# qope/starky-bn254

Measured on AMD Instinct MI355X. Metric: G1 scalar-mult proofs/sec at trace height 2^16, higher is better.
Workload: dtype u64

## Files before the change

### starky_bn254_amd/csrc/kernels.cuh

```cuda
#pragma once
#include "poseidon.cuh"
#include "air.cuh"

#include "kernels_ntt.cuh"

__global__ void pow_table_kernel(u64* out, size_t n, u64 base) {
  size_t i = (size_t)blockIdx.x * blockDim.x + threadIdx.x;
  if (i < n) out[i] = f_pow(F(base), i).v;
}
__global__ void shift_odd_table_kernel(u64* out, size_t n, const u64* __restrict__ shift, const u64* __restrict__ tw, u32 log_s) {
  size_t i = (size_t)blockIdx.x * blockDim.x + threadIdx.x;
  if (i < n) out[i] = (F(shift[i]) * F(tw[(i >> log_s) << log_s])).v;
}
__global__ void scale_pow_kernel(u64* v, size_t n, u64 base) {
  size_t i = (size_t)blockIdx.x * blockDim.x + threadIdx.x;
  if (i < n) v[i] = (F(v[i]) * f_pow(F(base), i)).v;
}

__global__ __launch_bounds__(256) __attribute__((amdgpu_waves_per_eu(4))) void leaf_hash_kernel(const u64* __restrict__ lde, size_t m, u32 lde_log, u32 ncols,
                                                        u64* __restrict__ digests) {
  size_t row = (size_t)blockIdx.x * blockDim.x + threadIdx.x;
  if (row >= m) return;
  F s[12];
#pragma unroll
  for (int i = 0; i < 12; i++) s[i] = F(0);
  size_t leaf = bitrev32((u32)row, lde_log);
  if (ncols <= 4) {
    for (u32 c = 0; c < 4; c++) digests[leaf * 4 + c] = c < ncols ? lde[(size_t)c * m + row] : 0;
    return;
  }
  for (u32 c = 0; c < ncols; c += 8) {
#pragma unroll
    for (u32 i = 0; i < 8; i++)
      if (c + i < ncols) s[i] = F(lde[(size_t)(c + i) * m + row]);
    poseidon_permute_keep(s, c + 8 >= ncols ? P_KEEP_DIGEST : (c + 16 <= ncols ? P_KEEP_CAPACITY : P_KEEP_ALL));
  }
#pragma unroll
  for (int i = 0; i < 4; i++) digests[leaf * 4 + i] = s[i].v;
}

__global__ __launch_bounds__(256) void merkle_level_kernel(const u64* __restrict__ child, u64* __restrict__ parent, size_t nparent) {
  size_t i = (size_t)blockIdx.x * blockDim.x + threadIdx.x;
  if (i >= nparent) return;
  F s[12];
#pragma unroll
  for (int k = 0; k < 8; k++) s[k] = F(child[i * 8 + k]);
#pragma unroll
  for (int k = 8; k < 12; k++) s[k] = F(0);
  poseidon_permute_keep(s, P_KEEP_DIGEST);
#pragma unroll
  for (int k = 0; k < 4; k++) parent[i * 4 + k] = s[k].v;
}

__global__ __launch_bounds__(256) __attribute__((amdgpu_waves_per_eu(4))) void leaf_absorb_kernel(const u64* __restrict__ lde_chunk, size_t m, u32 lde_log, u32 ncols_chunk,
                                                          u64* __restrict__ state, int first, int last, u64* __restrict__ digests, int next_full) {
  size_t row = (size_t)blockIdx.x * blockDim.x + threadIdx.x;
  if (row >= m) return;
  F s[12];
#pragma unroll
  for (int i = 0; i < 12; i++) s[i] = F(0);
  if (!first) {
#pragma unroll
    for (int i = 8; i < 12; i++) s[i] = F(state[(size_t)i * m + row]);
    if (ncols_chunk < 8) {
#pragma unroll
      for (int i = 0; i < 8; i++) s[i] = F(state[(size_t)i * m + row]);
    }
  }
  for (u32 c = 0; c < ncols_chunk; c += 8) {
#pragma unroll
    for (u32 i = 0; i < 8; i++)
      if (c + i < ncols_chunk) s[i] = F(lde_chunk[(size_t)(c + i) * m + row]);
    const bool end = c + 8 >= ncols_chunk;
    const int keep = end ? (last ? P_KEEP_DIGEST : (next_full ? P_KEEP_CAPACITY : P_KEEP_ALL)) : (c + 16 <= ncols_chunk ? P_KEEP_CAPACITY : P_KEEP_ALL);
    poseidon_permute_keep(s, keep);
  }
  u32 tid = threadIdx.x;
  asm volatile("" : "+v"(tid));
  const size_t row2 = (size_t)blockIdx.x * blockDim.x + tid;
  if (last) {
    size_t leaf = bitrev32((u32)row2, lde_log);
#pragma unroll
    for (int i = 0; i < 4; i++) digests[leaf * 4 + i] = s[i].v;
  } else {
#pragma unroll
    for (int i = 8; i < 12; i++) state[(size_t)i * m + row2] = s[i].v;
    if (!next_full) {
#pragma unroll
      for (int i = 0; i < 8; i++) state[(size_t)i * m + row2] = s[i].v;
    }
  }
}

static constexpr u32 MERKLE_SUBTREE_THREADS = 256;
__global__ __launch_bounds__(MERKLE_SUBTREE_THREADS) void merkle_subtree_kernel(u64* __restrict__ tree, size_t nleaf, u32 l0, u32 nlev, u32 nchild) {
  __shared__ u64 buf[2 * 256 * 4];
  const u32 tid = threadIdx.x, nt = blockDim.x;
  const u64* child = tree + (2 * nleaf - ((2 * nleaf) >> l0)) * 4;
  size_t base = (size_t)blockIdx.x * nchild;
  for (u32 e = tid; e < nchild * 4; e += nt) buf[e] = child[base * 4 + e];
  __syncthreads();
  u32 active = nchild / 2;
  const u32 groups = nt / 16, grp = tid / 16, lane = tid & 15;
  for (u32 lv = 1; lv <= nlev; lv++) {
    u64* out = tree + (2 * nleaf - ((2 * nleaf) >> (l0 + lv))) * 4;
    const size_t idx0 = ((size_t)blockIdx.x * nchild) >> lv;
    if (active > 4 * groups) {
      F s[12];
      if (tid < active) {
#pragma unroll
        for (int k = 0; k < 8; k++) s[k] = F(buf[tid * 8 + k]);
#pragma unroll
        for (int k = 8; k < 12; k++) s[k] = F(0);
        poseidon_permute_keep(s, P_KEEP_DIGEST);
      }
      __syncthreads();
      if (tid < active) {
#pragma unroll
        for (int k = 0; k < 4; k++) { buf[tid * 4 + k] = s[k].v; out[(idx0 + tid) * 4 + k] = s[k].v; }
      }
      __syncthreads();
    } else {
      u64 res[4];
      u32 nit = (active + groups - 1) / groups;
      for (u32 it = 0; it < nit; it++) {
        u32 parent = it * groups + grp;
        if (it * groups + (tid / 64) * 4 >= active) break;
        const u32 e = lane < 12 ? lane : lane - 12;
        u64 v = (parent < active && e < 8) ? buf[parent * 8 + e] : 0;
        res[it] = poseidon_permute_coop16(v, lane);
      }
      __syncthreads();
      for (u32 it = 0; it < nit; it++) {
        u32 parent = it * groups + grp;
        if (parent < active && lane < 4) { buf[parent * 4 + lane] = res[it]; out[(idx0 + parent) * 4 + lane] = res[it]; }
      }
      __syncthreads();
    }
    active >>= 1;
  }
}

__global__ __launch_bounds__(256) void merkle_level_thread_kernel(u64* __restrict__ tree, size_t nleaf, u32 l) {
  const size_t parents = nleaf >> (l + 1);
  const size_t i = (size_t)blockIdx.x * blockDim.x + threadIdx.x;
  if (i >= parents) return;
  const u64* child = tree + (2 * nleaf - ((2 * nleaf) >> l)) * 4;
  u64* out = tree + (2 * nleaf - ((2 * nleaf) >> (l + 1))) * 4;
  F s[12];
#pragma unroll
  for (int k = 0; k < 8; k++) s[k] = F(child[i * 8 + k]);
#pragma unroll
  for (int k = 8; k < 12; k++) s[k] = F(0);
  poseidon_permute_keep(s, P_KEEP_DIGEST);
#pragma unroll
  for (int k = 0; k < 4; k++) out[i * 4 + k] = s[k].v;
}
__global__ __launch_bounds__(256) void merkle_level_coop_kernel(u64* __restrict__ tree, size_t nleaf, u32 l) {
  const size_t parents = nleaf >> (l + 1);
  const size_t parent = ((size_t)blockIdx.x * blockDim.x + threadIdx.x) >> 4;
  const u32 lane = threadIdx.x & 15, e = lane < 12 ? lane : lane - 12;
  const u64* child = tree + (2 * nleaf - ((2 * nleaf) >> l)) * 4;
  u64* out = tree + (2 * nleaf - ((2 * nleaf) >> (l + 1))) * 4;
  const u64 v = (parent < parents && e < 8) ? child[parent * 8 + e] : 0;
  const u64 r = poseidon_permute_coop16(v, lane);
  if (parent < parents && lane < 4) out[parent * 4 + lane] = r;
}

__global__ __launch_bounds__(256) void fri_leaf_hash_kernel(const u64* __restrict__ va, const u64* __restrict__ vb, u32 log_m, u32 arity_bits,
                                                            u64* __restrict__ digests) {
  size_t leaf = (size_t)blockIdx.x * blockDim.x + threadIdx.x;
  size_t nleaf = (size_t)1 << (log_m - arity_bits);
  if (leaf >= nleaf) return;
  if (arity_bits == 1) {
    const u32 n0 = bitrev32((u32)(leaf * 2), log_m), n1 = bitrev32((u32)(leaf * 2 + 1), log_m);
    digests[leaf * 4 + 0] = va[n0]; digests[leaf * 4 + 1] = vb[n0]; digests[leaf * 4 + 2] = va[n1]; digests[leaf * 4 + 3] = vb[n1];
    return;
  }
  F s[12];
#pragma unroll
  for (int i = 0; i < 12; i++) s[i] = F(0);
  u32 arity = 1u << arity_bits;
  for (u32 t = 0; t < arity; t += 4) {
#pragma unroll
    for (u32 u = 0; u < 4; u++) {
      u32 nat = bitrev32((u32)(leaf * arity + t + u), log_m);
      s[2 * u] = F(va[nat]); s[2 * u + 1] = F(vb[nat]);
    }
    poseidon_permute_keep(s, t + 4 >= arity ? P_KEEP_DIGEST : P_KEEP_CAPACITY);
  }
#pragma unroll
  for (int i = 0; i < 4; i++) digests[leaf * 4 + i] = s[i].v;
}

__global__ __launch_bounds__(256) void fri_leaf_hash_coop_kernel(const u64* __restrict__ va, const u64* __restrict__ vb, u32 log_m, u32 arity_bits,
                                                                 u64* __restrict__ digests) {
  const size_t leaf = ((size_t)blockIdx.x * blockDim.x + threadIdx.x) >> 4;
  const size_t nleaf = (size_t)1 << (log_m - arity_bits);
  const u32 lane = threadIdx.x & 15, e = lane < 12 ? lane : lane - 12;
  const u32 arity = 1u << arity_bits;
  if (arity_bits == 1) {
    if (leaf < nleaf && lane < 4) {
      const u32 nat = bitrev32((u32)(leaf * 2 + (lane >> 1)), log_m);
      digests[leaf * 4 + lane] = (lane & 1) ? vb[nat] : va[nat];
    }
    return;
  }
  u64 st = 0;
  for (u32 t = 0; t < arity; t += 4) {
    if (leaf < nleaf && e < 8) {
      const u32 nat = bitrev32((u32)(leaf * arity + t + (e >> 1)), log_m);
      st = (e & 1) ? vb[nat] : va[nat];
    }
    st = poseidon_permute_coop16(st, lane);
  }
  if (leaf < nleaf && lane < 4) digests[leaf * 4 + lane] = st;
}

__global__ void field_mul_batch_kernel(const u64* a, const u64* b, u64* out, size_t count, int mode) {
  size_t i = (size_t)blockIdx.x * blockDim.x + threadIdx.x;
  if (i >= count) return;
#if defined(__HIP_DEVICE_COMPILE__)
  out[i] = mode ? nw::canon(nw::canon(nw::mul(a[i], b[i]))) : (F(a[i]) * F(b[i])).v;
#endif
}
__global__ void poseidon_batch_kernel(u64* states, size_t count) {
  size_t i = (size_t)blockIdx.x * blockDim.x + threadIdx.x;
  if (i >= count) return;
  F s[12];
  for (int k = 0; k < 12; k++) s[k] = F(states[i * 12 + k]);
  poseidon_permute(s);
  for (int k = 0; k < 12; k++) states[i * 12 + k] = s[k].v;
}

struct PairCols { int lhs, rhs; };

__device__ __forceinline__ F wave_scan_mul(F x, int lane) {
#pragma unroll
  for (int d = 1; d < 64; d <<= 1) {
    u64 o = __shfl_up((unsigned long long)x.v, d, 64);
    if (lane >= d) x = x * F(o);
  }
  return x;
}

template <int PZ_E>
__global__ __launch_bounds__(256) void permutation_z_kernel(const u64* __restrict__ trace, size_t n, const PairCols* __restrict__ pairs,
                                                            u64 gamma0, u64 gamma1, u64* __restrict__ zout) {
  __shared__ u64 wtot[4];
  __shared__ u64 carry_s;
  const int z = blockIdx.x;
  const u64* lhs = trace + (size_t)pairs[z].lhs * n;
  const u64* rhs = trace + (size_t)pairs[z].rhs * n;
  u64* zc = zout + (size_t)z * n;
  const int tid = threadIdx.x, lane = tid & 63, wv = tid >> 6;
  const F g0(gamma0), g1(gamma1);
  F carry(1), dprod(1);
  for (size_t base = 0; base < n; base += 256 * PZ_E) {
    const size_t i0 = base + (size_t)tid * PZ_E;
    u64 lv[PZ_E], rv[PZ_E];
#pragma unroll
    for (int e = 0; e < PZ_E; e++) { lv[e] = lhs[i0 + e]; rv[e] = rhs[i0 + e]; }
    F pr[PZ_E];
#pragma unroll
    for (int e = 0; e < PZ_E; e++) {
      const F l(lv[e]), r(rv[e]);
      const F num = (l + g0) * (l + g1);
      pr[e] = e ? pr[e - 1] * num : num;
      dprod = dprod * ((r + g0) * (r + g1));
    }
    F inc = wave_scan_mul(pr[PZ_E - 1], lane);
    if (lane == 63) wtot[wv] = inc.v;
    __syncthreads();
    F pre = carry;
    for (int w = 0; w < wv; w++) pre = pre * F(wtot[w]);
    const u64 prev = __shfl_up((unsigned long long)inc.v, 1, 64);
    const F excl = lane == 0 ? pre : pre * F(prev);
    zc[i0] = excl.v;
#pragma unroll
    for (int e = 1; e < PZ_E; e++) zc[i0 + e] = (excl * pr[e - 1]).v;
    carry = carry * F(wtot[0]) * F(wtot[1]) * F(wtot[2]) * F(wtot[3]);
    __syncthreads();
  }
  {
    F w = dprod;
#pragma unroll
    for (int d = 32; d >= 1; d >>= 1) w = w * F(__shfl_xor((unsigned long long)w.v, d, 64));
    if (lane == 0) wtot[wv] = w.v;
    __syncthreads();
    if (tid == 0) carry_s = f_inv(F(wtot[0]) * F(wtot[1]) * F(wtot[2]) * F(wtot[3])).v;
    __syncthreads();
  }
  carry = F(carry_s);
  __syncthreads();
  for (size_t base = n; base > 0; base -= 256 * PZ_E) {
    const size_t i0 = base - 1 - (size_t)tid * PZ_E;
    u64 rv[PZ_E], zv[PZ_E];
#pragma unroll
    for (int e = 0; e < PZ_E; e++) { rv[e] = rhs[i0 - e]; zv[e] = zc[i0 - e]; }
    F pr[PZ_E];
#pragma unroll
    for (int e = 0; e < PZ_E; e++) {
      const F r(rv[e]);
      const F den = (r + g0) * (r + g1);
      pr[e] = e ? pr[e - 1] * den : den;
    }
    F inc = wave_scan_mul(pr[PZ_E - 1], lane);
    if (lane == 63) wtot[wv] = inc.v;
    __syncthreads();
    F pre = carry;
    for (int w = 0; w < wv; w++) pre = pre * F(wtot[w]);
    const u64 prev = __shfl_up((unsigned long long)inc.v, 1, 64);
    const F excl = lane == 0 ? pre : pre * F(prev);
#pragma unroll
    for (int e = 0; e < PZ_E; e++) zc[i0 - e] = (F(zv[e]) * (excl * pr[e])).v;
    carry = carry * F(wtot[0]) * F(wtot[1]) * F(wtot[2]) * F(wtot[3]);
    __syncthreads();
  }
}

#include "kernels_quotient.cuh"
__global__ __launch_bounds__(256) void quotient_combine_kernel(QuotientParams p) {
  size_t i = (size_t)blockIdx.x * blockDim.x + threadIdx.x;
  if (i >= p.m) return;
  F dinv(p.zh_inv[((i << p.row_shift) | p.row_rho) & 1]);
#pragma unroll
  for (int j = 0; j < SBN_NCH; j++) {
    F acc(p.part[((size_t)(QSEG - 1) * SBN_NCH + j) * p.m + i]);
#pragma unroll
    for (u32 sgm = 0; sgm + 1 < QSEG; sgm++) acc += F(p.part[((size_t)sgm * SBN_NCH + j) * p.m + i]) * F(p.seg_shift[sgm][j]);
    p.qout[(size_t)j * p.m + i] = (acc * dinv).v;
  }
}

__global__ void domain_tables_kernel(u64* xs, u64* lag_first, u64* lag_last, size_t m, u32 lde_log, u32 degree_bits) {
  size_t i = (size_t)blockIdx.x * blockDim.x + threadIdx.x;
  if (i >= m) return;
  F w = f_root_of_unity(lde_log);
  F x = F(GL_GEN) * f_pow(w, i);
  F g = f_root_of_unity(degree_bits);
  F nn = F((u64)1 << degree_bits);
  F zx = f_exp_pow2(x, degree_bits) - F(1);
  xs[i] = x.v;
  lag_first[i] = (zx * f_inv(nn * (x - F(1)))).v;
  lag_last[i] = (zx * f_inv(nn * (g * x - F(1)))).v;
}

__device__ __forceinline__ F wave_scan_mul_rev(F x, int lane) {
#pragma unroll
  for (int d = 1; d < 64; d <<= 1) {
    u64 o = __shfl_down((unsigned long long)x.v, d, 64);
    if (lane + d < 64) x = x * F(o);
  }
  return x;
}
template <int PZ_E>
__global__ __launch_bounds__(256) void permz_chunk_products_kernel(const u64* __restrict__ trace, size_t n, const PairCols* __restrict__ pairs, u64 gamma0, u64 gamma1,
                                                                   u64* __restrict__ tot) {
  __shared__ u64 wn[4], wd[4];
  const int z = blockIdx.y;
  const size_t c = blockIdx.x, chunks = gridDim.x;
  const int tid = threadIdx.x, lane = tid & 63, wv = tid >> 6;
  const size_t i0 = c * 256 * PZ_E + (size_t)tid * PZ_E;
  const u64* lhs = trace + (size_t)pairs[z].lhs * n + i0;
  const u64* rhs = trace + (size_t)pairs[z].rhs * n + i0;
  const F g0(gamma0), g1(gamma1);
  u64 lv[PZ_E], rv[PZ_E];
#pragma unroll
  for (int e = 0; e < PZ_E; e++) { lv[e] = lhs[e]; rv[e] = rhs[e]; }
  F pn(1), pd(1);
#pragma unroll
  for (int e = 0; e < PZ_E; e++) { const F l(lv[e]), r(rv[e]); pn = pn * ((l + g0) * (l + g1)); pd = pd * ((r + g0) * (r + g1)); }
#pragma unroll
  for (int d = 32; d >= 1; d >>= 1) { pn = pn * F(__shfl_xor((unsigned long long)pn.v, d, 64)); pd = pd * F(__shfl_xor((unsigned long long)pd.v, d, 64)); }
  if (lane == 0) { wn[wv] = pn.v; wd[wv] = pd.v; }
  __syncthreads();
  if (tid == 0) {
    tot[((size_t)z * chunks + c) * 2] = (F(wn[0]) * F(wn[1]) * F(wn[2]) * F(wn[3])).v;
    tot[((size_t)z * chunks + c) * 2 + 1] = (F(wd[0]) * F(wd[1]) * F(wd[2]) * F(wd[3])).v;
  }
}
__global__ __launch_bounds__(64) void permz_chunk_scan_kernel(const u64* __restrict__ tot, u32 chunks, u64* __restrict__ pq) {
  const int z = blockIdx.x, lane = threadIdx.x;
  const u64* t = tot + (size_t)z * chunks * 2;
  u64* o = pq + (size_t)z * chunks * 2;
  F carry(1), all(1);
  for (u32 b = 0; b < chunks; b += 64) {
    const u32 idx = b + lane;
    const bool on = idx < chunks;
    const F inc = wave_scan_mul(on ? F(t[2 * idx]) : F(1), lane);
    const u64 pv = __shfl_up((unsigned long long)inc.v, 1, 64);
    if (on) o[2 * idx] = (lane == 0 ? carry : carry * F(pv)).v;
    carry = carry * F(__shfl((unsigned long long)inc.v, 63, 64));
    F d = on ? F(t[2 * idx + 1]) : F(1);
#pragma unroll
    for (int k = 32; k >= 1; k >>= 1) d = d * F(__shfl_xor((unsigned long long)d.v, k, 64));
    all = all * d;
  }
  F carry_s = f_inv(all);
  for (u32 b = ((chunks - 1) / 64) * 64;; b -= 64) {
    const u32 idx = b + lane;
    const bool on = idx < chunks;
    const F inc = wave_scan_mul_rev(on ? F(t[2 * idx + 1]) : F(1), lane);
    const u64 sv = __shfl_down((unsigned long long)inc.v, 1, 64);
    if (on) o[2 * idx + 1] = (lane == 63 ? carry_s : carry_s * F(sv)).v;
    carry_s = carry_s * F(__shfl((unsigned long long)inc.v, 0, 64));
    if (b == 0) break;
  }
}
template <int PZ_E>
__global__ __launch_bounds__(256) void permz_chunk_write_kernel(const u64* __restrict__ trace, size_t n, const PairCols* __restrict__ pairs, u64 gamma0, u64 gamma1,
                                                                const u64* __restrict__ pq, u64* __restrict__ zout) {
  __shared__ u64 wn[4], wd[4];
  const int z = blockIdx.y;
  const size_t c = blockIdx.x, chunks = gridDim.x;
  const int tid = threadIdx.x, lane = tid & 63, wv = tid >> 6;
  const size_t i0 = c * 256 * PZ_E + (size_t)tid * PZ_E;
  const u64* lhs = trace + (size_t)pairs[z].lhs * n + i0;
  const u64* rhs = trace + (size_t)pairs[z].rhs * n + i0;
  u64* zc = zout + (size_t)z * n + i0;
  const F g0(gamma0), g1(gamma1);
  u64 lv[PZ_E], rv[PZ_E];
#pragma unroll
  for (int e = 0; e < PZ_E; e++) { lv[e] = lhs[e]; rv[e] = rhs[e]; }
  F pn[PZ_E], sd[PZ_E];
#pragma unroll
  for (int e = 0; e < PZ_E; e++) { const F l(lv[e]); const F num = (l + g0) * (l + g1); pn[e] = e ? pn[e - 1] * num : num; }
#pragma unroll
  for (int e = PZ_E - 1; e >= 0; e--) { const F r(rv[e]); const F den = (r + g0) * (r + g1); sd[e] = e < PZ_E - 1 ? sd[e + 1] * den : den; }
  const F incn = wave_scan_mul(pn[PZ_E - 1], lane), incd = wave_scan_mul_rev(sd[0], lane);
  if (lane == 63) wn[wv] = incn.v;
  if (lane == 0) wd[wv] = incd.v;
  __syncthreads();
  F pre(pq[((size_t)z * chunks + c) * 2]), suf(pq[((size_t)z * chunks + c) * 2 + 1]);
  for (int w = 0; w < wv; w++) pre = pre * F(wn[w]);
  for (int w = 3; w > wv; w--) suf = suf * F(wd[w]);
  const u64 pv = __shfl_up((unsigned long long)incn.v, 1, 64), sv = __shfl_down((unsigned long long)incd.v, 1, 64);
  const F exn = lane == 0 ? pre : pre * F(pv);
  const F exd = lane == 63 ? suf : suf * F(sv);
  const F both = exn * exd;
  zc[0] = (both * sd[0]).v;
#pragma unroll
  for (int e = 1; e < PZ_E; e++) zc[e] = (both * pn[e - 1] * sd[e]).v;
}

__global__ void ext_pow_table_kernel(u64* pa, u64* pb, size_t n, u64 z0, u64 z1) {
  size_t i = (size_t)blockIdx.x * blockDim.x + threadIdx.x;
  if (i >= n) return;
  E2 r = e2_pow(E2(F(z0), F(z1)), i);
  pa[i] = r.a.v; pb[i] = r.b.v;
}
__device__ __forceinline__ F block_sum(F v, u64* sh) {
  const int lane = threadIdx.x & 63, wv = threadIdx.x >> 6;
#pragma unroll
  for (int d = 32; d >= 1; d >>= 1) v = v + F(__shfl_xor((unsigned long long)v.v, d, 64));
  __syncthreads();
  if (lane == 0) sh[wv] = v.v;
  __syncthreads();
  F t(0);
  for (unsigned w = 0; w < blockDim.x / 64; w++) t = t + F(sh[w]);
  return t;
}
template <u32 OPEN_UNROLL>
__global__ __launch_bounds__(256) void openings_kernel(const u64* __restrict__ coeffs, size_t n, const u64* __restrict__ pa0, const u64* __restrict__ pb0,
                                                       const u64* __restrict__ pa1, const u64* __restrict__ pb1, u64* __restrict__ out) {
  __shared__ u64 sh[4];
  const u64* c = coeffs + (size_t)blockIdx.x * n;
  Acc<F> s0, r0, s1, r1;
  s0.clear(); r0.clear(); s1.clear(); r1.clear();
  for (size_t i = threadIdx.x; i < n; i += 256 * OPEN_UNROLL) {
    u64 cv[OPEN_UNROLL], t0[OPEN_UNROLL], t1[OPEN_UNROLL], t2[OPEN_UNROLL], t3[OPEN_UNROLL];
#pragma unroll
    for (u32 k = 0; k < OPEN_UNROLL; k++) {
      const size_t ik = i + 256 * k;
      cv[k] = c[ik]; t0[k] = pa0[ik]; t1[k] = pb0[ik]; t2[k] = pa1[ik]; t3[k] = pb1[ik];
    }
    __builtin_amdgcn_sched_barrier(0);
#pragma unroll
    for (u32 k = 0; k < OPEN_UNROLL; k++) {
      const F v{cv[k]};
      s0.macv(v, F(t0[k])); r0.macv(v, F(t1[k]));
      s1.macv(v, F(t2[k])); r1.macv(v, F(t3[k]));
    }
  }
  const F a0 = block_sum(s0.value(), sh), b0 = block_sum(r0.value(), sh), a1 = block_sum(s1.value(), sh), b1 = block_sum(r1.value(), sh);
  if (threadIdx.x == 0) {
    u64* o = out + (size_t)blockIdx.x * 4;
    o[0] = a0.v; o[1] = b0.v; o[2] = a1.v; o[3] = b1.v;
  }
}

template <u32 OPEN_UNROLL>
__global__ __launch_bounds__(256) void openings1_kernel(const u64* __restrict__ coeffs, size_t n, const u64* __restrict__ pa, const u64* __restrict__ pb,
                                                        u64* __restrict__ out, u32 off) {
  __shared__ u64 sh[4];
  const u64* c = coeffs + (size_t)blockIdx.x * n;
  Acc<F> s0, r0;
  s0.clear(); r0.clear();
  for (size_t i = threadIdx.x; i < n; i += 256 * OPEN_UNROLL) {
    u64 cv[OPEN_UNROLL], t0[OPEN_UNROLL], t1[OPEN_UNROLL];
#pragma unroll
    for (u32 k = 0; k < OPEN_UNROLL; k++) {
      const size_t ik = i + 256 * k;
      cv[k] = c[ik]; t0[k] = pa[ik]; t1[k] = pb[ik];
    }
    __builtin_amdgcn_sched_barrier(0);
#pragma unroll
    for (u32 k = 0; k < OPEN_UNROLL; k++) {
      const F v{cv[k]};
      s0.macv(v, F(t0[k])); r0.macv(v, F(t1[k]));
    }
  }
  const F a0 = block_sum(s0.value(), sh), b0 = block_sum(r0.value(), sh);
  if (threadIdx.x == 0) {
    u64* o = out + (size_t)blockIdx.x * 4 + off;
    o[0] = a0.v; o[1] = b0.v;
  }
}

__global__ __launch_bounds__(256) void fri_combine_partial_kernel(const u64* __restrict__ coeffs, size_t n, u32 npoly, u32 group_size,
                                                                  const u64* __restrict__ pa, const u64* __restrict__ pb, u64* __restrict__ part_a,
                                                                  u64* __restrict__ part_b) {
  size_t i = (size_t)blockIdx.x * blockDim.x + threadIdx.x;
  if (i >= n) return;
  const u32 g = blockIdx.y;
  const u32 j0 = g * group_size, cnt = j0 + group_size < npoly ? group_size : npoly - j0;
  const u64* c = coeffs + (size_t)j0 * n + i;
  Acc<F> a, b;
  a.clear(); b.clear();
  u32 k = 0;
  for (; k + 8 <= cnt; k += 8) {
    u64 f[8];
#pragma unroll
    for (u32 u = 0; u < 8; u++) f[u] = c[(size_t)(k + u) * n];
#pragma unroll
    for (u32 u = 0; u < 8; u++) { const F v(f[u]); a.mac(v, F(pa[k + u])); b.mac(v, F(pb[k + u])); }
  }
  for (; k < cnt; k++) { const F v(c[(size_t)k * n]); a.mac(v, F(pa[k])); b.mac(v, F(pb[k])); }
  part_a[(size_t)g * n + i] = a.value().v; part_b[(size_t)g * n + i] = b.value().v;
}
__global__ void fri_combine_reduce_kernel(const u64* part_a, const u64* part_b, size_t n, u32 ngroups, const u64* w, u64* out_a, u64* out_b, int accumulate) {
  size_t i = (size_t)blockIdx.x * blockDim.x + threadIdx.x;
  if (i >= n) return;
  E2 acc = accumulate ? E2(F(out_a[i]), F(out_b[i])) : E2(F(0), F(0));
  for (u32 g = 0; g < ngroups; g++) acc += E2(F(part_a[(size_t)g * n + i]), F(part_b[(size_t)g * n + i])) * E2(F(w[2 * g]), F(w[2 * g + 1]));
  out_a[i] = acc.a.v; out_b[i] = acc.b.v;
}

static constexpr u32 DBL_CHUNK = 16;
__global__ __launch_bounds__(256) void divide_by_linear_pass1(const u64* __restrict__ ca, const u64* __restrict__ cb, size_t nchunks, u64 z0, u64 z1,
                                                              u64* __restrict__ ha, u64* __restrict__ hb) {
  const size_t t = (size_t)blockIdx.x * blockDim.x + threadIdx.x;
  if (t >= nchunks) return;
  const E2 z{F(z0), F(z1)};
  const size_t s = t * DBL_CHUNK;
  E2 h{F(0), F(0)};
  for (u32 k = DBL_CHUNK; k-- > 0;) h = h * z + E2(F(ca[s + k]), F(cb[s + k]));
  ha[t] = h.a.v; hb[t] = h.b.v;
}
template <u32 U> __device__ __forceinline__ void dbl_fold(const u64* ha, const u64* hb, size_t base, size_t per, const E2 zl, E2& g) {
  for (size_t j0 = per; j0 > 0; j0 -= U) {
    u64 va[U], vb[U];
#pragma unroll
    for (u32 k = 0; k < U; k++) { va[k] = ha[base + j0 - 1 - k]; vb[k] = hb[base + j0 - 1 - k]; }
#pragma unroll
    for (u32 k = 0; k < U; k++) g = E2(F(va[k]), F(vb[k])) + zl * g;
  }
}
template <u32 U> __device__ __forceinline__ void dbl_replay(u64* ha, u64* hb, size_t base, size_t per, const E2 zl, E2 carry) {
  for (size_t j0 = per; j0 > 0; j0 -= U) {
    u64 va[U], vb[U];
#pragma unroll
    for (u32 k = 0; k < U; k++) { va[k] = ha[base + j0 - 1 - k]; vb[k] = hb[base + j0 - 1 - k]; }
#pragma unroll
    for (u32 k = 0; k < U; k++) {
      ha[base + j0 - 1 - k] = carry.a.v; hb[base + j0 - 1 - k] = carry.b.v;
      carry = E2(F(va[k]), F(vb[k])) + zl * carry;
    }
  }
}
__global__ __launch_bounds__(256) void divide_by_linear_pass2(u64* __restrict__ ha, u64* __restrict__ hb, size_t nchunks, u64 z0, u64 z1) {
  __shared__ u64 sa[2][256], sb[2][256];
  const int tid = threadIdx.x;
  const int lanes = nchunks < 256 ? (int)nchunks : 256;
  const size_t per = nchunks / lanes, base = (size_t)tid * per;
  const bool live = tid < lanes;
  const E2 zl = e2_pow(E2{F(z0), F(z1)}, DBL_CHUNK);
  E2 g{F(0), F(0)};
  if (live) { if (per % 8 == 0) dbl_fold<8>(ha, hb, base, per, zl, g); else dbl_fold<1>(ha, hb, base, per, zl, g); }
  E2 m = e2_pow(zl, per);
  int cur = 0;
  sa[0][tid] = g.a.v; sb[0][tid] = g.b.v;
  __syncthreads();
  for (int d = 1; d < lanes; d <<= 1) {
    E2 v{F(sa[cur][tid]), F(sb[cur][tid])};
    if (tid + d < lanes) v = v + m * E2(F(sa[cur][tid + d]), F(sb[cur][tid + d]));
    sa[cur ^ 1][tid] = v.a.v; sb[cur ^ 1][tid] = v.b.v;
    m = m * m;
    cur ^= 1;
    __syncthreads();
  }
  E2 carry{F(0), F(0)};
  if (tid + 1 < lanes) carry = E2(F(sa[cur][tid + 1]), F(sb[cur][tid + 1]));
  if (live) { if (per % 8 == 0) dbl_replay<8>(ha, hb, base, per, zl, carry); else dbl_replay<1>(ha, hb, base, per, zl, carry); }
}
__global__ __launch_bounds__(256) void divide_by_linear_pass3(const u64* __restrict__ ca, const u64* __restrict__ cb, size_t nchunks, u64 z0, u64 z1,
                                                              const u64* __restrict__ ha, const u64* __restrict__ hb, u64 mul0, u64 mul1,
                                                              u64* __restrict__ oa, u64* __restrict__ ob, int accumulate, u32 times_x) {
  const size_t t = (size_t)blockIdx.x * blockDim.x + threadIdx.x;
  if (t >= nchunks) return;
  const E2 z{F(z0), F(z1)}, mul{F(mul0), F(mul1)};
  const size_t s = t * DBL_CHUNK, n = nchunks * DBL_CHUNK;
  E2 b{F(ha[t]), F(hb[t])};
  for (u32 k = DBL_CHUNK; k-- > 0;) {
    const size_t i = s + k;
    const E2 q = b;
    b = b * z + E2(F(ca[i]), F(cb[i]));
    const size_t j = i + times_x;
    if (j >= n) continue;
    const E2 o = accumulate ? E2(F(oa[j]), F(ob[j])) * mul + q : q;
    oa[j] = o.a.v; ob[j] = o.b.v;
  }
}

__global__ void fri_fold_kernel(const u64* ca, const u64* cb, size_t nout, u32 arity, u64 b0, u64 b1, u64* oa, u64* ob) {
  size_t i = (size_t)blockIdx.x * blockDim.x + threadIdx.x;
  if (i >= nout) return;
  E2 beta{F(b0), F(b1)}, acc(F(0), F(0));
  for (u32 t = arity; t-- > 0;) acc = acc * beta + E2(F(ca[i * arity + t]), F(cb[i * arity + t]));
  oa[i] = acc.a.v; ob[i] = acc.b.v;
}

struct PowParams { u64 state[12]; u32 wpos; u32 min_lz; u64 base; u64 count; u64* result; };
__global__ __launch_bounds__(256) void pow_kernel(PowParams p) {
  u64 gid = (u64)blockIdx.x * blockDim.x + threadIdx.x;
  if (gid >= p.count) return;
  F s[12];
#pragma unroll
  for (int i = 0; i < 12; i++) s[i] = F(p.state[i]);
  s[p.wpos] = F(p.base + gid);
  poseidon_permute(s);
  u64 resp = s[P_RATE - 1].v;
  u32 lz = resp ? (u32)__clzll((long long)resp) : 64;
  if (lz >= p.min_lz) atomicMin((unsigned long long*)p.result, (unsigned long long)(p.base + gid));
}

__global__ __launch_bounds__(256) void split_pack_kernel(const u64* __restrict__ lde, size_t m, u32 nc, u32 ob, u32 log_r, u32 me,
                                                         u64* __restrict__ send_l, u64* __restrict__ send_n, u64* __restrict__ self_l, u64* __restrict__ self_n) {
  const size_t i = (size_t)blockIdx.x * blockDim.x + threadIdx.x;
  const u32 c = blockIdx.y;
  if (i >= m || c >= nc) return;
  const u64 v = lde[(size_t)c * m + i];
  const size_t ml = m >> log_r, rmask = ((size_t)1 << log_r) - 1;
  const u32 s = bitrev32((u32)(i & rmask), log_r);
  if (s == me) self_l[(size_t)c * ml + (i >> log_r)] = v;
  else send_l[((size_t)s * ob + c) * ml + (i >> log_r)] = v;
  if (send_n) {
    const size_t p = (i + m - 2) & (m - 1);
    const u32 s2 = bitrev32((u32)(p & rmask), log_r);
    if (s2 == me) self_n[(size_t)c * ml + (p >> log_r)] = v;
    else send_n[((size_t)s2 * ob + c) * ml + (p >> log_r)] = v;
  }
}
__global__ void split_unpack_rows_kernel(const u64* __restrict__ in, size_t m, u32 nplanes, u32 log_r, u64* __restrict__ out) {
  const size_t i = (size_t)blockIdx.x * blockDim.x + threadIdx.x;
  if (i >= m) return;
  const size_t ml = m >> log_r;
  const u32 s = bitrev32((u32)(i & (((size_t)1 << log_r) - 1)), log_r);
  for (u32 p = 0; p < nplanes; p++) out[(size_t)p * m + i] = in[((size_t)s * nplanes + p) * ml + (i >> log_r)];
}
__global__ void split_modadd_kernel(const u64* __restrict__ in, size_t len, u32 nranks, u64* __restrict__ out) {
  const size_t k = (size_t)blockIdx.x * blockDim.x + threadIdx.x;
  if (k >= len) return;
  F acc(in[k]);
  for (u32 r = 1; r < nranks; r++) acc += F(in[(size_t)r * len + k]);
  out[k] = acc.v;
}

__global__ void gather_rows_kernel(const u64* mat, size_t m, u32 lde_log, u32 ncols, const u32* idx, u64* out, size_t qstride, size_t off) {
  u32 c = blockIdx.x * blockDim.x + threadIdx.x;
  u32 q = blockIdx.y;
  if (c >= ncols) return;
  size_t row = bitrev32(idx[q], lde_log);
  out[(size_t)q * qstride + off + c] = mat[(size_t)c * m + row];
}
__global__ void gather_siblings_kernel(const u64* tree, size_t nleaf, u32 nlevels, const u32* idx, u32 shift, u64* out, size_t qstride, size_t off) {
  u32 q = blockIdx.x;
  u32 e = threadIdx.x;
  if (e >= nlevels * 4) return;
  u32 l = e >> 2, k = e & 3;
  size_t x = idx[q] >> shift;
  size_t level_off = 2 * nleaf - ((2 * nleaf) >> l);
  size_t sib = (x >> l) ^ 1;
  out[(size_t)q * qstride + off + e] = tree[(level_off + sib) * 4 + k];
}
__global__ void gather_fri_leaf_kernel(const u64* va, const u64* vb, u32 log_m, u32 arity_bits, const u32* idx, u32 shift, u64* out, size_t qstride, size_t off) {
  u32 q = blockIdx.x;
  u32 e = threadIdx.x;
  u32 arity = 1u << arity_bits;
  if (e >= 2 * arity) return;
  size_t leaf = idx[q] >> shift;
  u32 nat = bitrev32((u32)(leaf * arity + (e >> 1)), log_m);
  out[(size_t)q * qstride + off + e] = (e & 1) ? vb[nat] : va[nat];
}

typedef unsigned long long u64x2_t __attribute__((ext_vector_type(2)));
__global__ __launch_bounds__(256) void first_non_canonical_kernel(const u64* __restrict__ w, size_t count, u64 base, unsigned long long* first_bad) {
  const size_t head = (((size_t)w & 8) && count) ? 1 : 0;
  const u64x2_t* __restrict__ v = reinterpret_cast<const u64x2_t*>(w + head);
  const size_t nvec = (count - head) >> 1;
  const size_t tid = (size_t)blockIdx.x * blockDim.x + threadIdx.x, stride = (size_t)gridDim.x * blockDim.x;
  u64 bad = ~(u64)0;
#pragma unroll 4
  for (size_t i = tid; i < nvec; i += stride) {
    const u64x2_t x = v[i];
    const bool b0 = x.x >= GLP, b1 = x.y >= GLP;
    if (b0 | b1) { const u64 j = head + 2 * i + (b0 ? 0 : 1); bad = bad < j ? bad : j; }
  }
  if (tid == 0) {
    const size_t last = head + 2 * nvec;
    if (last < count && w[last] >= GLP) bad = bad < last ? bad : last;
    if (head && w[0] >= GLP) bad = 0;
  }
  if (!__any(bad != ~(u64)0)) return;
  for (int d = 32; d >= 1; d >>= 1) { const u64 o = __shfl_xor((unsigned long long)bad, d, 64); bad = o < bad ? o : bad; }
  if ((threadIdx.x & 63) == 0) atomicMin(first_bad, (unsigned long long)(base + bad));
}
```

### starky_bn254_amd/csrc/kernels_ntt.cuh

```cuda
#pragma once
#include "gl.cuh"

struct NttPassParams {
  const u64* in; u64* out;
  size_t in_col_stride, out_col_stride;
  u32 log_r;
  u32 log_t;
  u32 log_n;
  size_t in_sr, in_st, out_sr, out_st;
  size_t n_in;
  u32 r_fast_load;
  u32 twiddle;
  const u64* tw;
  u32 tw_log;
  const u64* pre;
  const u64* post;
  u64 scale;
  const u64* pre2;
  u32 split;
  u32 xcd_order;
};

GL_HD F tw_lookup(const u64* tw, u32 tw_log, u64 e_of_order, u32 order_log) {
  u64 idx = (e_of_order << (tw_log - order_log)) & ((1ULL << tw_log) - 1);
  u64 half = 1ULL << (tw_log - 1);
  if (idx >= half) return -F(tw[idx - half]);
  return F(tw[idx]);
}

__device__ __forceinline__ u64 tw_full(const u64* __restrict__ tw, u32 tw_log, u32 e_of_order, u32 order_log) {
  return tw[(e_of_order << (tw_log - order_log)) & ((1u << tw_log) - 1u)];
}

static constexpr int NTT_THREADS = 256;

#ifdef SBN_NTT_KERNELS_HERE
__global__ __launch_bounds__(NTT_THREADS) void ntt_pass_kernel(NttPassParams p) {
  extern __shared__ u64 lds[];
  const u32 R = 1u << p.log_r, T = 1u << p.log_t;
  const u32 LDT = T + 1;
  const size_t col = blockIdx.y;
  const size_t t0 = (size_t)blockIdx.x << p.log_t;
  const u64* in = p.in + col * p.in_col_stride;
  u64* out = p.out + col * p.out_col_stride;
  const u32 total = R << p.log_t;
  for (u32 e = threadIdx.x; e < total; e += NTT_THREADS) {
    u32 r, t;
    if (p.r_fast_load) { r = e & (R - 1); t = e >> p.log_r; } else { t = e & (T - 1); r = e >> p.log_t; }
    size_t gi = (size_t)r * p.in_sr + (t0 + t) * p.in_st;
    u64 v = 0;
    if (gi < p.n_in) {
      v = in[gi];
      if (p.pre) v = (F(v) * F(p.pre[gi])).v;
    }
    lds[r * LDT + t] = v;
  }
  __syncthreads();
  for (u32 s = 0; s < p.log_r; s++) {
    u32 half = R >> (s + 1);
    u32 nb = total >> 1;
    for (u32 e = threadIdx.x; e < nb; e += NTT_THREADS) {
      u32 t = e & (T - 1), b = e >> p.log_t;
      u32 j = b & (half - 1), blk = b / half;
      u32 i0 = blk * 2 * half + j, i1 = i0 + half;
      F u{lds[i0 * LDT + t]}, v(lds[i1 * LDT + t]);
      F w = tw_lookup(p.tw, p.tw_log, (u64)j << s, p.log_r);
      lds[i0 * LDT + t] = (u + v).v;
      lds[i1 * LDT + t] = ((u - v) * w).v;
    }
    __syncthreads();
  }
  for (u32 e = threadIdx.x; e < total; e += NTT_THREADS) {
    u32 t = e & (T - 1), k = e >> p.log_t;
    u32 q = bitrev32(k, p.log_r);
    F v{lds[q * LDT + t]};
    if (p.twiddle) v = v * tw_lookup(p.tw, p.tw_log, (u64)k * (t0 + t), p.log_n);
    if (p.scale != 1) v = v * F(p.scale);
    size_t go = (size_t)k * p.out_sr + (t0 + t) * p.out_st;
    if (p.post) v = v * F(p.post[go]);
    out[go] = v.v;
  }
}
#else
__global__ void ntt_pass_kernel(NttPassParams p);
#endif

namespace nw {
#if !defined(SBN_NTT_CXX_ARITH)
using namespace gp;
__device__ __forceinline__ u64 repay_carry(u64 s, u64 k) { u64 k2, k3; u64 t = madm1(sel01(k), s, k2); return madm1(sel01(k2), t, k3); }
__device__ __forceinline__ u64 add(u64 a, u64 b) {
  u64 k1, k2; u32 lo = addco(lo32(a), lo32(b), k1); u32 hi = addc(hi32(a), hi32(b), k1, k2);
  return repay_carry(pack(lo, hi), k2);
}
__device__ __forceinline__ u64 sub(u64 a, u64 b) {
  u64 k1, k2, k3, k4, k5, k6;
  u32 lo = subco(lo32(a), lo32(b), k1); u32 hi = subb(hi32(a), hi32(b), k1, k2);
  u32 l2 = subco(lo, selm1(k2), k3); u32 h2 = subb0(hi, k3, k4);
  u32 l3 = subco(l2, selm1(k4), k5); u32 h3 = subb0(h2, k5, k6);
  return pack(l3, h3);
}
__device__ __forceinline__ u64 red32(u64 lo, u32 hi) { u64 k; u64 t = madm1(hi, lo, k); u64 k2; return madm1(sel01(k), t, k2); }
__device__ __forceinline__ u64 red(u64 lo, u64 hi) {
  u64 k1, k2, k3, k4, k5, k6;
  const u32 l = subco(lo32(lo), hi32(hi), k1), h = subb0(hi32(lo), k1, k2);
  const u32 t = subb0(lo32(hi), k2, k3);
  const u64 r = madm1(t, pack(l, h), k4);
  const u32 rl = addc(lo32(r), selm1(k4), k3, k5), rh = addc(hi32(r), 0u, k5, k6);
  return pack(rl, rh);
}
template <int E> __device__ __forceinline__ u64 mul_pow2(u64 x) {
  if constexpr (E == 0) return x;
  else if constexpr (E < 32) return red32(x << E, hi32(x) >> (32 - E));
  else if constexpr (E == 32) return red32(pack(0, lo32(x)), hi32(x));
  else if constexpr (E < 64) return red(pack(0, lo32(x) << (E - 32)), x >> (64 - E));
  else return mul_pow2<E - 48>(mul_pow2<48>(x));
}
__device__ __forceinline__ u64 mul(u64 a, u64 b) { return gl_mul_weak(a, b); }
__device__ __forceinline__ u64 canon(u64 x) { return gp::canon(x); }
#else
__device__ __forceinline__ u64 add(u64 a, u64 b) {
  u64 s = a + b;
  u64 c = s < a ? GLEPS : 0;
  s += c;
  if (s < c) s += GLEPS;
  return s;
}
__device__ __forceinline__ u64 sub(u64 a, u64 b) {
  u64 d = a - b;
  u64 c = a < b ? GLEPS : 0;
  u64 r = d - c;
  if (d < c) r -= GLEPS;
  return r;
}
__device__ __forceinline__ u64 red(u64 lo, u64 hi) {
  u32 hi_hi = (u32)(hi >> 32), hi_lo = (u32)hi;
  u64 t0 = lo - hi_hi;
  if (lo < hi_hi) t0 -= GLEPS;
  u64 t1 = ((u64)hi_lo << 32) - hi_lo;
  u64 r = t0 + t1;
  if (r < t1) r += GLEPS;
  return r;
}
template <int E> __device__ __forceinline__ u64 mul_pow2(u64 x) {
  if constexpr (E == 0) return x;
  else if constexpr (E < 64) return red(x << E, x >> (64 - E));
  else return mul_pow2<E - 48>(mul_pow2<48>(x));
}
__device__ __forceinline__ u64 mul(u64 a, u64 b) { return red(a * b, __umul64hi(a, b)); }
__device__ __forceinline__ u64 canon(u64 x) { return x >= GLP ? x - GLP : x; }
#endif

#define NW_BF(i, j, E) { u64 a_ = x[i], b_ = x[j]; x[i] = add(a_, b_); x[j] = mul_pow2<E>(sub(a_, b_)); }
__device__ __forceinline__ void dft16_rho(u64* x) {
  NW_BF(0, 8, 0) NW_BF(1, 9, 12) NW_BF(2, 10, 24) NW_BF(3, 11, 36) NW_BF(4, 12, 48) NW_BF(5, 13, 60) NW_BF(6, 14, 72) NW_BF(7, 15, 84)
  NW_BF(0, 4, 0) NW_BF(1, 5, 24) NW_BF(2, 6, 48) NW_BF(3, 7, 72) NW_BF(8, 12, 0) NW_BF(9, 13, 24) NW_BF(10, 14, 48) NW_BF(11, 15, 72)
  NW_BF(0, 2, 0) NW_BF(1, 3, 48) NW_BF(4, 6, 0) NW_BF(5, 7, 48) NW_BF(8, 10, 0) NW_BF(9, 11, 48) NW_BF(12, 14, 0) NW_BF(13, 15, 48)
  NW_BF(0, 1, 0) NW_BF(2, 3, 0) NW_BF(4, 5, 0) NW_BF(6, 7, 0) NW_BF(8, 9, 0) NW_BF(10, 11, 0) NW_BF(12, 13, 0) NW_BF(14, 15, 0)
}
#undef NW_BF
}

#ifdef SBN_NTT_KERNELS_HERE
template <int LOG_B>
__global__ __launch_bounds__(256) void ntt_fast_pass_kernel(NttPassParams p, u32 kperm) {
  extern __shared__ u64 lds[];
  constexpr u32 NB = 1u << LOG_B;
  constexpr u32 R = 256u << LOG_B;
  const size_t col = p.xcd_order ? blockIdx.x : blockIdx.y;
  const size_t t0 = (size_t)(p.xcd_order ? blockIdx.y : blockIdx.x) << 4;
  const u32 half = p.split ? blockIdx.z : 0u;
  const u64* __restrict__ pre = half ? p.pre2 : p.pre;
  const u64* in = p.in + col * p.in_col_stride;
  u64* out = p.out + col * p.out_col_stride;
  u32 g, t;
  if (p.r_fast_load) { g = threadIdx.x & 15; t = threadIdx.x >> 4; } else { t = threadIdx.x & 15; g = threadIdx.x >> 4; }
  const size_t tg = t0 + t;
  const u32 S1 = p.r_fast_load ? 257u : 272u;
  const u32 lane_off = p.r_fast_load ? (t * 16) : t;
  const u32 g_mul = p.r_fast_load ? 1u : 16u;
  u64 x[NB][16];
#pragma unroll
  for (u32 b = 0; b < NB; b++)
#pragma unroll
    for (u32 q = 0; q < 16; q++) {
      u32 r = g + 16 * q + 256 * b;
      size_t gi = (size_t)r * p.in_sr + tg * p.in_st;
      u64 v = 0;
      if (gi < p.n_in) {
        v = in[gi];
        if (pre) v = nw::mul(v, pre[gi]);
      }
      x[b][q] = v;
    }
  if (LOG_B == 1) {
    const bool upper_zero = p.in_st == 1 && (size_t)256 * p.in_sr >= p.n_in;
#pragma unroll
    for (u32 q = 0; q < 16; q++) {
      u32 r = g + 16 * q;
      u64 a = x[0][q], bb = x[NB - 1][q];
      u64 w = tw_full(p.tw, p.tw_log, r, 9);
      if (upper_zero) { x[NB - 1][q] = nw::mul(a, w); }
      else { x[0][q] = nw::add(a, bb); x[NB - 1][q] = nw::mul(nw::sub(a, bb), w); }
    }
  }
#pragma unroll
  for (u32 b = 0; b < NB; b++) {
    nw::dft16_rho(x[b]);
#pragma unroll
    for (u32 pidx = 0; pidx < 16; pidx++) {
      u32 m = __brev(pidx) >> 28;
      u32 k1 = (kperm * m) & 15;
      u64 v = x[b][pidx];
      if (g && k1) v = nw::mul(v, tw_full(p.tw, p.tw_log, (u32)(g * k1), 8));
      lds[(b * 16 + k1) * S1 + lane_off + g * g_mul] = v;
    }
  }
  __syncthreads();
  const u32 k1 = g;
#pragma unroll
  for (u32 b = 0; b < NB; b++) {
#pragma unroll
    for (u32 gp = 0; gp < 16; gp++) x[b][gp] = lds[(b * 16 + k1) * S1 + lane_off + gp * g_mul];
    nw::dft16_rho(x[b]);
#pragma unroll
    for (u32 pidx = 0; pidx < 16; pidx++) {
      u32 m = __brev(pidx) >> 28;
      u32 k2 = (kperm * m) & 15;
      u32 k256 = k1 + 16 * k2;
      u32 k = LOG_B == 0 ? k256 : (k256 * NB + b);
      if (LOG_B == 1) k = (k << p.split) + half;
      u64 v = x[b][pidx];
      if (p.twiddle) v = nw::mul(v, tw_full(p.tw, p.tw_log, (u32)(k * tg), p.log_n));
      if (p.scale != 1) v = nw::mul(v, p.scale);
      size_t go = (size_t)k * p.out_sr + tg * p.out_st;
      if (p.post) v = nw::mul(v, p.post[go]);
      out[go] = nw::canon(v);
    }
  }
  (void)R;
}
#else
template <int LOG_B> __global__ void ntt_fast_pass_kernel(NttPassParams p, u32 kperm);
#endif

struct NttFusedParams {
  const u64* in; size_t in_col_stride;
  u64* coef; size_t coef_col_stride;
  u64* out; size_t out_col_stride;
  size_t n1;
  u32 log_n;
  const u64* tw_i; const u64* tw_f; u32 tw_log;
  const u64* pre;
  u64 scale;
  const u64* pre2;
};
#ifdef SBN_NTT_KERNELS_HERE
__global__ __launch_bounds__(256) __attribute__((amdgpu_waves_per_eu(4))) void ntt_fused_inv_b_lde_a_kernel(NttFusedParams p) {
  extern __shared__ u64 lds[];
  const size_t col = blockIdx.x;
  const size_t t0 = (size_t)blockIdx.y << 4;
  const u64* in = p.in + col * p.in_col_stride;
  u64* coef = p.coef + col * p.coef_col_stride;
  u64* out = p.out + col * p.out_col_stride;
  const u32 g = threadIdx.x & 15, t = threadIdx.x >> 4;
  const size_t tg = t0 + t;
  u64 x[2][16];
#pragma unroll
  for (u32 q = 0; q < 16; q++) x[0][q] = in[(size_t)(g + 16 * q) + tg * 256];
  nw::dft16_rho(x[0]);
#pragma unroll
  for (u32 pidx = 0; pidx < 16; pidx++) {
    const u32 m = __brev(pidx) >> 28, k1 = (11u * m) & 15;
    u64 v = x[0][pidx];
    if (g && k1) v = nw::mul(v, tw_full(p.tw_i, p.tw_log, (u32)(g * k1), 8));
    lds[k1 * 257 + t * 16 + g] = v;
  }
  __syncthreads();
#pragma unroll
  for (u32 gp = 0; gp < 16; gp++) x[0][gp] = lds[g * 257 + t * 16 + gp];
  nw::dft16_rho(x[0]);
  u64 a[16];
#pragma unroll
  for (u32 pidx = 0; pidx < 16; pidx++) {
    const u32 m = __brev(pidx) >> 28, k2 = (11u * m) & 15;
    const u32 k = g + 16 * k2;
    const u64 v = nw::mul(x[0][pidx], p.scale);
    coef[(size_t)k * p.n1 + tg] = nw::canon(v);
    a[k2] = v;
  }
  __syncthreads();
#pragma unroll
  for (u32 q = 0; q < 16; q++) {
    const u32 r = g + 16 * q;
    const u64 v = nw::mul(a[q], p.pre[(size_t)r * p.n1 + tg]);
    x[0][q] = v;
    x[1][q] = nw::mul(v, tw_full(p.tw_f, p.tw_log, r, 9));
  }
#pragma unroll
  for (u32 b = 0; b < 2; b++) {
    nw::dft16_rho(x[b]);
#pragma unroll
    for (u32 pidx = 0; pidx < 16; pidx++) {
      const u32 m = __brev(pidx) >> 28, k1 = (5u * m) & 15;
      u64 v = x[b][pidx];
      if (g && k1) v = nw::mul(v, tw_full(p.tw_f, p.tw_log, (u32)(g * k1), 8));
      lds[(b * 16 + k1) * 272 + g * 17 + t] = v;
    }
  }
  __syncthreads();
  const u32 t2 = threadIdx.x & 15, k1o = threadIdx.x >> 4;
  const size_t tg2 = t0 + t2;
#pragma unroll
  for (u32 b = 0; b < 2; b++) {
#pragma unroll
    for (u32 gp = 0; gp < 16; gp++) x[b][gp] = lds[(b * 16 + k1o) * 272 + gp * 17 + t2];
    nw::dft16_rho(x[b]);
#pragma unroll
    for (u32 pidx = 0; pidx < 16; pidx++) {
      const u32 m = __brev(pidx) >> 28, k2 = (5u * m) & 15;
      const u32 k = (k1o + 16 * k2) * 2 + b;
      const u64 v = nw::mul(x[b][pidx], tw_full(p.tw_f, p.tw_log, (u32)(k * tg2), p.log_n + 1));
      out[(size_t)k * p.n1 + tg2] = nw::canon(v);
    }
  }
}
#else
__global__ void ntt_fused_inv_b_lde_a_kernel(NttFusedParams p);
#endif

#ifdef SBN_NTT_KERNELS_HERE
__global__ __launch_bounds__(256) __attribute__((amdgpu_waves_per_eu(4))) void ntt_fused512_inv_b_lde_a_kernel(NttFusedParams p) {
  extern __shared__ u64 lds[];
  const size_t col = blockIdx.x;
  const size_t t0 = (size_t)blockIdx.y << 4;
  const u64* in = p.in + col * p.in_col_stride;
  u64* coef = p.coef + col * p.coef_col_stride;
  u64* out = p.out + col * p.out_col_stride;
  const u32 g = threadIdx.x & 15, t = threadIdx.x >> 4;
  const size_t tg = t0 + t;
  u64 x[2][16];
#pragma unroll
  for (u32 q0 = 0; q0 < 16; q0 += 8) {
#pragma unroll
    for (u32 q = q0; q < q0 + 8; q++) {
      const u64 lo = in[(size_t)(g + 16 * q) + tg * 512], hi = in[(size_t)(g + 16 * q + 256) + tg * 512];
      x[0][q] = nw::add(lo, hi);
      x[1][q] = nw::mul(nw::sub(lo, hi), tw_full(p.tw_i, p.tw_log, g + 16 * q, 9));
    }
    asm volatile("" ::: "memory");
  }
#pragma unroll
  for (u32 b = 0; b < 2; b++) {
    nw::dft16_rho(x[b]);
#pragma unroll
    for (u32 pidx = 0; pidx < 16; pidx++) {
      const u32 m = __brev(pidx) >> 28, k1 = (11u * m) & 15;
      u64 v = x[b][pidx];
      if (g && k1) v = nw::mul(v, tw_full(p.tw_i, p.tw_log, (u32)(g * k1), 8));
      lds[(b * 16 + k1) * 257 + t * 16 + g] = v;
    }
  }
  __syncthreads();
#pragma unroll
  for (u32 b = 0; b < 2; b++) {
    u64 z[16];
#pragma unroll
    for (u32 gp = 0; gp < 16; gp++) z[gp] = lds[(b * 16 + g) * 257 + t * 16 + gp];
    nw::dft16_rho(z);
#pragma unroll
    for (u32 pidx = 0; pidx < 16; pidx++) {
      const u32 m = __brev(pidx) >> 28, k2 = (11u * m) & 15;
      const u64 v = nw::mul(z[pidx], p.scale);
      coef[(size_t)((g + 16 * k2) * 2 + b) * 512 + tg] = nw::canon(v);
      x[b][k2] = v;
    }
    asm volatile("" ::: "memory");
  }
  __syncthreads();
#pragma unroll 1
  for (u32 h = 0; h < 2; h++) {
    u32 t2 = threadIdx.x & 15, k1o = threadIdx.x >> 4;
    u32 gl = g, tl = t;
    asm volatile("" : "+v"(t2), "+v"(k1o), "+v"(gl), "+v"(tl));
    const size_t tg2 = t0 + t2, tgl = t0 + tl;
    const u64* __restrict__ pre = h ? p.pre2 : p.pre;
#pragma unroll
    for (u32 b = 0; b < 2; b++)
#pragma unroll
      for (u32 q0 = 0; q0 < 16; q0 += 8) {
#pragma unroll
        for (u32 q = q0; q < q0 + 8; q++) {
          const size_t ci = (size_t)(2 * (gl + 16 * q) + b) * 512 + tgl;
          u64 c = x[b][q];
          if (h) c = coef[ci];
          x[b][q] = nw::mul(c, pre[ci]);
        }
        asm volatile("" ::: "memory");
      }
#pragma unroll
    for (u32 b = 0; b < 2; b++) {
      nw::dft16_rho(x[b]);
#pragma unroll
      for (u32 pidx = 0; pidx < 16; pidx++) {
        const u32 m = __brev(pidx) >> 28, k1 = (5u * m) & 15;
        u64 v = x[b][pidx];
        if (gl && k1) v = nw::mul(v, tw_full(p.tw_f, p.tw_log, (u32)(gl * k1), 8));
        lds[(b * 16 + k1) * 272 + gl * 17 + tl] = v;
      }
    }
    __syncthreads();
#pragma unroll
    for (u32 b = 0; b < 2; b++) {
#pragma unroll
      for (u32 gp = 0; gp < 16; gp++) x[b][gp] = lds[(b * 16 + k1o) * 272 + gp * 17 + t2];
      nw::dft16_rho(x[b]);
    }
#pragma unroll
    for (u32 pidx = 0; pidx < 16; pidx++) {
      const u32 m = __brev(pidx) >> 28, k2 = (5u * m) & 15;
      const u32 j = k1o + 16 * k2;
      const u64 e = x[0][pidx], o = nw::mul(x[1][pidx], tw_full(p.tw_f, p.tw_log, j, 9));
      const u32 ka = 2 * j + h, kb = 2 * (j + 256) + h;
      out[(size_t)ka * 512 + tg2] = nw::canon(nw::mul(nw::add(e, o), tw_full(p.tw_f, p.tw_log, (u32)(ka * tg2), 19)));
      out[(size_t)kb * 512 + tg2] = nw::canon(nw::mul(nw::sub(e, o), tw_full(p.tw_f, p.tw_log, (u32)(kb * tg2), 19)));
    }
    __syncthreads();
  }
}
#else
__global__ void ntt_fused512_inv_b_lde_a_kernel(NttFusedParams p);
#endif
```

### starky_bn254_amd/csrc/ntt.hip

```cpp
#define SBN_NTT_KERNELS_HERE
#include "kernels_ntt.cuh"
template __global__ void ntt_fast_pass_kernel<0>(NttPassParams p, u32 kperm);
template __global__ void ntt_fast_pass_kernel<1>(NttPassParams p, u32 kperm);
```

### starky_bn254_amd/csrc/prover.hip

```cpp
#include "prover_ctx.hpp"
#include "kernels.cuh"
#include <algorithm>
#include <cstring>
#include <cstdlib>
#include <thread>
#include <atomic>
#include <chrono>
#include <functional>

namespace sbn { thread_local std::string g_last_error; }

static std::atomic<int> g_default_device{0};
static thread_local int t_device = -1;
static inline int cur_device() { return t_device >= 0 ? t_device : g_default_device.load(); }
#define g_device (cur_device())
namespace sbn {
int current_device() { return cur_device(); }
int use_current_device(const char* why) {
  int ndev = 0;
  if (hipGetDeviceCount(&ndev) != hipSuccess || ndev == 0) return fail(SBN_ERR_NO_DEVICE, "no HIP device available: %s", why);
  HIPC(hipSetDevice(g_device));
  return 0;
}
}

static const char* STAGE_NAMES[ST_COUNT + EX_COUNT] = {
  "trace_commit", "perm_z", "z_commit", "quotient_eval", "quotient_commit",
  "openings", "fri_combine", "fri_layers", "pow", "queries",
  "trace_absorb_kernels_ms", "trace_absorb_launches", "z_absorb_kernels_ms", "z_absorb_launches", "device_tracegen_ms",
  "split_exchange_ms"};

static int dmalloc(u64** p, size_t words, size_t* bytes = nullptr) {
  HIPC(hipMalloc((void**)p, words * sizeof(u64)));
  if (bytes) *bytes += words * sizeof(u64);
  return 0;
}

static u32 pick_log_t(u32 log_r, u32 log_s) {
  u32 lt = 4;
  while (lt > 0 && ((size_t)(1u << log_r) * ((1u << lt) + 1) * 8) > 48 * 1024) lt--;
  return std::min(lt, log_s);
}
static int ntt_columns(sbn_prover* P, const u64* in, size_t in_cs, u64* out, size_t out_cs, u64* tmp, size_t tmp_cs, size_t ncols,
                       u32 log_n, bool inverse, size_t n_in, const u64* pre, const u64* post, u64 scale, hipStream_t st = nullptr, int which = 3) {
  if (ncols == 0) return 0;
  if (!st) st = P->stream;
  u32 log_n1 = (log_n + 1) / 2, log_n2 = log_n - log_n1;
  size_t n1 = (size_t)1 << log_n1, n2 = (size_t)1 << log_n2;
  NttPassParams a{};
  a.in = in; a.out = tmp; a.in_col_stride = in_cs; a.out_col_stride = tmp_cs;
  a.log_r = log_n1; a.log_t = pick_log_t(log_n1, log_n2); a.log_n = log_n;
  a.in_sr = n2; a.in_st = 1; a.out_sr = n2; a.out_st = 1; a.n_in = n_in;
  a.r_fast_load = 0; a.twiddle = 1; a.tw = inverse ? P->d_tw_i : P->d_tw_f; a.tw_log = P->lde_log;
  a.pre = pre; a.post = nullptr; a.scale = 1;
  NttPassParams b{};
  b.in = tmp; b.out = out; b.in_col_stride = tmp_cs; b.out_col_stride = out_cs;
  b.log_r = log_n2; b.log_t = pick_log_t(log_n2, log_n1); b.log_n = log_n;
  b.in_sr = 1; b.in_st = n2; b.out_sr = n1; b.out_st = 1; b.n_in = (size_t)1 << log_n;
  b.r_fast_load = 1; b.twiddle = 0; b.tw = a.tw; b.tw_log = P->lde_log;
  b.pre = nullptr; b.post = post; b.scale = scale;
  for (size_t c0 = 0; c0 < ncols; c0 += 32768) {
    size_t nc = std::min<size_t>(32768, ncols - c0);
    NttPassParams pa = a, pb = b;
    pa.in = a.in + c0 * in_cs; pa.out = a.out + c0 * tmp_cs;
    pb.in = b.in + c0 * tmp_cs; pb.out = b.out + c0 * out_cs;
    dim3 ga((unsigned)(n2 >> pa.log_t), (unsigned)nc), gb((unsigned)(n1 >> pb.log_t), (unsigned)nc);
    size_t la = ((size_t)1 << pa.log_r) * ((1u << pa.log_t) + 1) * 8, lb = ((size_t)1 << pb.log_r) * ((1u << pb.log_t) + 1) * 8;
    const u32 kperm = inverse ? 11u : 5u;
    auto launch = [&](NttPassParams q, dim3 grid, size_t lds_bytes) {
      const bool fast = q.log_t == 4 && (q.log_r == 8 || q.log_r == 9);
      if (fast) { q.xcd_order = 1; std::swap(grid.x, grid.y); }
      if (fast && q.log_r == 8) hipLaunchKernelGGL(ntt_fast_pass_kernel<0>, grid, dim3(256), 16 * 272 * 8, st, q, kperm);
      else if (fast) hipLaunchKernelGGL(ntt_fast_pass_kernel<1>, grid, dim3(256), 32 * 272 * 8, st, q, kperm);
      else hipLaunchKernelGGL(ntt_pass_kernel, grid, dim3(NTT_THREADS), lds_bytes, st, q);
    };
    if (pa.log_r == 9 && log_n2 >= 4) pa.log_t = 4;
    if (pb.log_r == 9 && log_n1 >= 4) pb.log_t = 4;
    const bool split_a = !inverse && pa.log_r == 10 && log_n2 >= 4 && pa.in_st == 1 && n_in <= (size_t)512 * pa.in_sr && pre == P->d_shift && P->d_shift_odd;
    if (split_a) { pa.log_r = 9; pa.log_t = 4; pa.split = 1; pa.pre2 = P->d_shift_odd; }
    ga = dim3((unsigned)(n2 >> pa.log_t), (unsigned)nc, split_a ? 2u : 1u); gb = dim3((unsigned)(n1 >> pb.log_t), (unsigned)nc);
    la = ((size_t)1 << pa.log_r) * ((1u << pa.log_t) + 1) * 8; lb = ((size_t)1 << pb.log_r) * ((1u << pb.log_t) + 1) * 8;
    if (which & 1) launch(pa, ga, la);
    if (which & 2) launch(pb, gb, lb);
  }
  HIPC(hipGetLastError());
  return 0;
}

static u64 host_inv_pow2(u32 k) { return f_inv(F((u64)1 << k)).v; }
static int ntt_fast_setup() {
  static std::atomic<bool> done[SBN_MAX_DEVICES];
  const int d = g_device >= 0 && g_device < SBN_MAX_DEVICES ? g_device : 0;
  if (!done[d].load()) {
    HIPC(hipFuncSetAttribute((const void*)ntt_fast_pass_kernel<1>, hipFuncAttributeMaxDynamicSharedMemorySize, 32 * 272 * 8));
    HIPC(hipFuncSetAttribute((const void*)ntt_fused_inv_b_lde_a_kernel, hipFuncAttributeMaxDynamicSharedMemorySize, 32 * 272 * 8));
    HIPC(hipFuncSetAttribute((const void*)ntt_fused512_inv_b_lde_a_kernel, hipFuncAttributeMaxDynamicSharedMemorySize, 32 * 272 * 8));
    done[d].store(true);
  }
  return 0;
}
static void ntt_plan(sbn_prover* P) {
  P->ntt_fused = P->degree_bits == 16 || P->degree_bits == 17;
  P->ntt_fused512 = P->degree_bits == 18 && P->lde_log == 19;
}

static int intt_values(sbn_prover* P, const u64* vals, u64* coef, size_t ncols) {
  for (size_t c0 = 0; c0 < ncols; c0 += P->ntt_chunk) {
    size_t nc = std::min(P->ntt_chunk, ncols - c0);
    int rc = ntt_columns(P, vals + c0 * P->n, P->n, coef + c0 * P->n, P->n, P->d_tmp, P->m, nc, P->degree_bits, true, P->n, nullptr, nullptr,
                         host_inv_pow2(P->degree_bits));
    if (rc) return rc;
  }
  return 0;
}
static int lde_coeffs(sbn_prover* P, const u64* coef, u64* lde, size_t ncols) {
  for (size_t c0 = 0; c0 < ncols; c0 += P->ntt_chunk) {
    size_t nc = std::min(P->ntt_chunk, ncols - c0);
    int rc = ntt_columns(P, coef + c0 * P->n, P->n, lde + c0 * P->m, P->m, P->d_tmp, P->m, nc, P->lde_log, false, P->n, P->d_shift, nullptr, 1);
    if (rc) return rc;
  }
  return 0;
}
static int intt_then_lde(sbn_prover* P, const u64* vals, u64* coef, u64* lde, size_t ncols) {
  for (size_t c0 = 0; c0 < ncols; c0 += P->ntt_chunk) {
    size_t nc = std::min(P->ntt_chunk, ncols - c0);
    int rc = ntt_columns(P, vals + c0 * P->n, P->n, coef + c0 * P->n, P->n, P->d_tmp, P->m, nc, P->degree_bits, true, P->n, nullptr, nullptr,
                         host_inv_pow2(P->degree_bits));
    if (rc) return rc;
    rc = ntt_columns(P, coef + c0 * P->n, P->n, lde + c0 * P->m, P->m, P->d_tmp, P->m, nc, P->lde_log, false, P->n, P->d_shift, nullptr, 1);
    if (rc) return rc;
  }
  return 0;
}

static int intt_lde_cols_fused(sbn_prover* P, const u64* v, u64* cf, u64* lde_out, size_t nc, u64* tmp2, hipStream_t lde_stream, hipEvent_t handoff) {
  int rc = ntt_columns(P, v, P->n, cf, P->n, P->d_tmp, P->m, nc, P->degree_bits, true, P->n, nullptr, nullptr, host_inv_pow2(P->degree_bits), nullptr, 1);
  if (rc) return rc;
  NttFusedParams f{};
  const u32 log_n1 = (P->degree_bits + 1) / 2;
  f.in = P->d_tmp; f.in_col_stride = P->m; f.coef = cf; f.coef_col_stride = P->n; f.out = tmp2; f.out_col_stride = P->m;
  f.n1 = (size_t)1 << log_n1; f.log_n = P->degree_bits; f.tw_i = P->d_tw_i; f.tw_f = P->d_tw_f; f.tw_log = P->lde_log; f.pre = P->d_shift; f.pre2 = P->d_shift_odd;
  f.scale = host_inv_pow2(P->degree_bits);
  if (P->ntt_fused512) hipLaunchKernelGGL(ntt_fused512_inv_b_lde_a_kernel, dim3((unsigned)nc, 32u), dim3(256), 32 * 272 * 8, P->stream, f);
  else hipLaunchKernelGGL(ntt_fused_inv_b_lde_a_kernel, dim3((unsigned)nc, (unsigned)(f.n1 >> 4)), dim3(256), 32 * 272 * 8, P->stream, f);
  if (lde_stream != P->stream) {
    HIPC(hipEventRecord(handoff, P->stream));
    HIPC(hipStreamWaitEvent(lde_stream, handoff, 0));
  }
  return ntt_columns(P, cf, P->n, lde_out, P->m, tmp2, P->m, nc, P->lde_log, false, P->n, P->d_shift, nullptr, 1, lde_stream, 2);
}
static int intt_lde_cols(sbn_prover* P, const u64* v, u64* cf, u64* lde_out, size_t nc) {
  if ((P->ntt_fused || P->ntt_fused512) && P->d_tmp2) return intt_lde_cols_fused(P, v, cf, lde_out, nc, P->d_tmp2, P->stream, nullptr);
  int rc = ntt_columns(P, v, P->n, cf, P->n, P->d_tmp, P->m, nc, P->degree_bits, true, P->n, nullptr, nullptr, host_inv_pow2(P->degree_bits));
  if (rc) return rc;
  return ntt_columns(P, cf, P->n, lde_out, P->m, P->d_tmp, P->m, nc, P->lde_log, false, P->n, P->d_shift, nullptr, 1);
}

static int tree_alloc(DevTree& t, size_t nleaf, u32 cap_height, size_t* bytes = nullptr) {
  t.nleaf = nleaf;
  u32 lg = 0; while (((size_t)1 << lg) < nleaf) lg++;
  t.nlevels = lg - cap_height;
  return dmalloc(&t.d, 2 * nleaf * 4, bytes);
}
static int tree_build_inner(sbn_prover* P, DevTree& t, hipStream_t st) {
  u32 l0 = 0;
  while (l0 < t.nlevels) {
    const size_t parents = t.nleaf >> (l0 + 1);
    if (parents <= 8192 && parents >= 16 && ((t.nleaf >> l0) % 32) == 0) {
      const u32 nlev = std::min<u32>(t.nlevels - l0, 5);
      hipLaunchKernelGGL(merkle_subtree_kernel, dim3((unsigned)((t.nleaf >> l0) / 32)), dim3(MERKLE_SUBTREE_THREADS), 0, st, t.d, t.nleaf, l0, nlev, 32u);
      l0 += nlev;
      continue;
    }
    if (parents >= 16384) {
      hipLaunchKernelGGL(merkle_level_thread_kernel, dim3((unsigned)((parents + 255) / 256)), dim3(256), 0, st, t.d, t.nleaf, l0);
      l0++;
    } else if (parents > 16) {
      hipLaunchKernelGGL(merkle_level_coop_kernel, dim3((unsigned)((parents * 16 + 255) / 256)), dim3(256), 0, st, t.d, t.nleaf, l0);
      l0++;
    } else {
      const size_t nodes = t.nleaf >> l0;
      u32 nchild = (u32)std::min<size_t>(512, nodes);
      u32 lg = 0; while ((2u << lg) < nchild) lg++;
      u32 nlev = std::min(t.nlevels - l0, lg + 1);
      hipLaunchKernelGGL(merkle_subtree_kernel, dim3((unsigned)(nodes / nchild)), dim3(MERKLE_SUBTREE_THREADS), 0, st, t.d, t.nleaf, l0, nlev, nchild);
      l0 += nlev;
    }
  }
  HIPC(hipGetLastError());
  return 0;
}
static int tree_from_matrix(sbn_prover* P, DevTree& t, const u64* lde, size_t ncols) {
  hipLaunchKernelGGL(leaf_hash_kernel, dim3((unsigned)((P->m + 255) / 256)), dim3(256), 0, P->stream, lde, P->m, P->lde_log, (u32)ncols, t.d);
  return tree_build_inner(P, t, P->stream);
}
struct HostUpload { const u64* src; hipEvent_t* done; };
static int upload_setup(sbn_prover* P) {
  if (!P->ustream) HIPC(hipStreamCreate(&P->ustream));
  for (auto& e : P->upload_done) if (!e) HIPC(hipEventCreateWithFlags(&e, hipEventDisableTiming));
  for (auto& e : P->slot_copied) if (!e) HIPC(hipEventCreateWithFlags(&e, hipEventDisableTiming));
  if (!P->h_ring) HIPC(hipHostMalloc((void**)&P->h_ring, UPLOAD_SLOTS * UPLOAD_SLOT_WORDS * sizeof(u64), hipHostMallocDefault));
  if (!P->h_first_bad) HIPC(hipHostMalloc((void**)&P->h_first_bad, sizeof(unsigned long long), hipHostMallocDefault));
  if (!P->d_first_bad) { HIPC(hipMalloc((void**)&P->d_first_bad, sizeof(unsigned long long))); P->dev_bytes += sizeof(unsigned long long); }
  return 0;
}
static void launch_first_non_canonical(const u64* d_words, size_t count, u64 base, unsigned long long* d_first_bad, hipStream_t st) {
  const size_t blocks = std::min<size_t>(std::max<size_t>((count / 2 + 255) / 256, 1), 2048);
  hipLaunchKernelGGL(first_non_canonical_kernel, dim3((unsigned)blocks), dim3(256), 0, st, d_words, count, base, d_first_bad);
}
static int upload_chunk(sbn_prover* P, const HostUpload& up, size_t k, size_t c0, size_t nc) {
  const size_t w0 = c0 * P->n, w1 = w0 + nc * P->n;
  const size_t threads = std::min<size_t>(tracegen_host_threads(), 16);
  for (size_t a = w0; a < w1; a += UPLOAD_SLOT_WORDS) {
    const size_t len = std::min(UPLOAD_SLOT_WORDS, w1 - a);
    const unsigned s = P->slot_next; P->slot_next = (s + 1) % UPLOAD_SLOTS;
    if (P->slot_used[s]) HIPC(hipEventSynchronize(P->slot_copied[s]));
    u64* slot = P->h_ring + (size_t)s * UPLOAD_SLOT_WORDS;
    const u64* from = up.src + a;
    const size_t parts = std::max<size_t>(1, std::min(threads, len >> 15)), per = (len + parts - 1) / parts;
    host_parallel_for(parts, [&](size_t t) { const size_t b0 = t * per, b1 = std::min(len, b0 + per); if (b0 < b1) memcpy(slot + b0, from + b0, (b1 - b0) * sizeof(u64)); });
    HIPC(hipMemcpyAsync(P->d_trace + a, slot, len * sizeof(u64), hipMemcpyHostToDevice, P->ustream));
    HIPC(hipEventRecord(P->slot_copied[s], P->ustream));
    P->slot_used[s] = true;
  }
  launch_first_non_canonical(P->d_trace + w0, w1 - w0, (u64)w0, P->d_first_bad, P->ustream);
  HIPC(hipGetLastError());
  HIPC(hipEventRecord(up.done[k], P->ustream));
  return 0;
}

static int commit_pipeline(sbn_prover* P, const u64* vals, u64* coef, u64* lde, size_t ncols, DevTree& t, int ex_ms, int ex_launches, const HostUpload* up = nullptr) {
  size_t ch = P->ntt_chunk;
  size_t nchunks = (ncols + ch - 1) / ch;
  if (nchunks > (size_t)MAX_CHUNKS) return fail(SBN_ERR_UNSUPPORTED, "too many column chunks");
  if (ncols <= 4) {
    if (up) {
      int rc = upload_chunk(P, *up, 0, 0, ncols);
      if (rc) return rc;
      HIPC(hipStreamWaitEvent(P->stream, up->done[0], 0));
    }
    int rc = intt_then_lde(P, vals, coef, lde, ncols);
    if (rc) return rc;
    P->stage_ms[ST_COUNT + ex_launches] = 0;
    return tree_from_matrix(P, t, lde, ncols);
  }
  for (size_t k = 0; k < nchunks; k++) {
    size_t c0 = k * ch, nc = std::min(ch, ncols - c0);
    int rc;
    if (up) {
      if ((rc = upload_chunk(P, *up, k, c0, nc))) return rc;
      HIPC(hipStreamWaitEvent(P->stream, up->done[k], 0));
    }
    if (P->ntt_two_streams && (P->ntt_fused || P->ntt_fused512) && P->d_tmp3) {
      if (k >= 2) HIPC(hipStreamWaitEvent(P->stream, P->chunk_ready[k - 2], 0));
      rc = intt_lde_cols_fused(P, vals + c0 * P->n, coef + c0 * P->n, lde + c0 * P->m, nc, (k & 1) ? P->d_tmp3 : P->d_tmp2, P->nstream, P->intt_done[k]);
      if (rc) return rc;
      HIPC(hipEventRecord(P->chunk_ready[k], P->nstream));
    } else if (P->ntt_two_streams && !P->ntt_fused && !P->ntt_fused512) {
      rc = ntt_columns(P, vals + c0 * P->n, P->n, coef + c0 * P->n, P->n, P->d_tmp, P->m, nc, P->degree_bits, true, P->n, nullptr, nullptr, host_inv_pow2(P->degree_bits));
      if (rc) return rc;
      HIPC(hipEventRecord(P->intt_done[k], P->stream));
      HIPC(hipStreamWaitEvent(P->nstream, P->intt_done[k], 0));
      rc = ntt_columns(P, coef + c0 * P->n, P->n, lde + c0 * P->m, P->m, P->d_tmp2, P->m, nc, P->lde_log, false, P->n, P->d_shift, nullptr, 1, P->nstream);
      if (rc) return rc;
      HIPC(hipEventRecord(P->chunk_ready[k], P->nstream));
    } else {
      rc = intt_lde_cols(P, vals + c0 * P->n, coef + c0 * P->n, lde + c0 * P->m, nc);
      if (rc) return rc;
      HIPC(hipEventRecord(P->chunk_ready[k], P->stream));
    }
    HIPC(hipStreamWaitEvent(P->hstream, P->chunk_ready[k], 0));
    HIPC(hipEventRecord(P->abs_ev[2 * k], P->hstream));
    hipLaunchKernelGGL(leaf_absorb_kernel, dim3((unsigned)((P->m + 255) / 256)), dim3(256), 0, P->hstream, lde + c0 * P->m, P->m, P->lde_log, (u32)nc,
                       P->d_sponge, k == 0 ? 1 : 0, k + 1 == nchunks ? 1 : 0, t.d,
                       (k + 1 < nchunks && std::min(ch, ncols - (c0 + nc)) >= 8) ? 1 : 0);
    HIPC(hipEventRecord(P->abs_ev[2 * k + 1], P->hstream));
  }
  int rc = tree_build_inner(P, t, P->hstream);
  if (rc) return rc;
  HIPC(hipEventRecord(P->hash_done, P->hstream));
  HIPC(hipStreamWaitEvent(P->stream, P->hash_done, 0));
  P->stage_ms[ST_COUNT + ex_launches] = (float)nchunks;
  (void)ex_ms;
  return 0;
}
static thread_local double t_wait_deadline_s = 0;
static inline void poll_backoff(unsigned spins) {
  if (spins < 2000) std::this_thread::yield();
  else std::this_thread::sleep_for(std::chrono::microseconds(spins < 20000 ? 20 : 200));
}
static inline hipError_t stream_wait(hipStream_t st) {
  if (t_wait_deadline_s <= 0) return hipStreamSynchronize(st);
  const auto t0 = std::chrono::steady_clock::now();
  unsigned spins = 0;
  for (;;) {
    const hipError_t e = hipStreamQuery(st);
    if (e != hipErrorNotReady) return e;
    if (std::chrono::duration<double>(std::chrono::steady_clock::now() - t0).count() > t_wait_deadline_s) return hipErrorNotReady;
    poll_backoff(++spins);
  }
}
static inline hipError_t event_wait(hipEvent_t ev) {
  if (t_wait_deadline_s <= 0) return hipEventSynchronize(ev);
  const auto t0 = std::chrono::steady_clock::now();
  unsigned spins = 0;
  for (;;) {
    const hipError_t e = hipEventQuery(ev);
    if (e != hipErrorNotReady) return e;
    if (std::chrono::duration<double>(std::chrono::steady_clock::now() - t0).count() > t_wait_deadline_s) return hipErrorNotReady;
    poll_backoff(++spins);
  }
}
static int split_exchange(sbn_prover* P, hipStream_t st, const std::vector<uint64_t>& so, const std::vector<uint64_t>& sl, const std::vector<uint64_t>& ro,
                          const std::vector<uint64_t>& rl) {
  SplitCtx* S = P->sp;
  bool any = false;
  for (u32 r = 0; r < S->comm.world; r++) any = any || sl[r] || rl[r];
  if (!any) return 0;
  const bool timed = S->tev_used + 2 <= S->tev.size();
  if (timed) HIPC(hipEventRecord(S->tev[S->tev_used], st));
  const int rc = S->comm.all_to_all(S->comm.ctx, (void*)st, so.data(), sl.data(), ro.data(), rl.data());
  if (rc) return fail(SBN_ERR_HIP, "sbn_comm.all_to_all failed (%d)", rc);
  if (timed) { HIPC(hipEventRecord(S->tev[S->tev_used + 1], st)); S->tev_used += 2; }
  return 0;
}
static int split_all_gather_host(sbn_prover* P, const void* send, void* recv, size_t bytes) {
  SplitCtx* S = P->sp;
  const int rc = S->comm.all_gather_host(S->comm.ctx, send, recv, bytes);
  if (rc) return fail(SBN_ERR_HIP, "sbn_comm.all_gather_host failed (%d)", rc);
  return 0;
}
static int split_all_gather_device(sbn_prover* P, size_t words) {
  SplitCtx* S = P->sp;
  const u32 R = S->comm.world;
  if (words * R > S->scratch_words || words * sizeof(u64) > S->comm.send_bytes) return fail(SBN_ERR_HIP, "internal: split scratch too small");
  const uint64_t base = (uint64_t)((const char*)S->scratch - (const char*)S->comm.recv_buf);
  std::vector<uint64_t> so(R, 0), sl(R, words * sizeof(u64)), ro(R), rl(R, words * sizeof(u64));
  for (u32 r = 0; r < R; r++) ro[r] = base + (uint64_t)r * words * sizeof(u64);
  return split_exchange(P, P->stream, so, sl, ro, rl);
}
static int commit_split(sbn_prover* P, const ColShare& sh, const u64* vals, bool vals_global, u64* coef_own, u64* plane_l, u64* plane_n, DevTree& t) {
  SplitCtx* S = P->sp;
  const u32 R = S->comm.world, me = S->comm.rank;
  const size_t n = P->n, m = P->m, ml = S->ml, ob = sh.ob;
  const size_t steps = sh.steps();
  if (steps > (size_t)MAX_CHUNKS) return fail(SBN_ERR_UNSUPPORTED, "too many column blocks");
  const char* rbase = (const char*)S->comm.recv_buf;
  const char* sbase = (const char*)S->comm.send_buf;
  const u32 row_log = P->lde_log - S->log_r;
  for (size_t k = 0; k < steps; k++) {
    const size_t b = k * R + me, nc = sh.block_cols(b);
    hipStream_t tstream = P->stream;
    u64* const slot = (u64*)S->comm.send_buf + (k & 1) * S->slot_words;
    u64* const slot_n = S->planes == 2 ? slot + (size_t)R * ob * ml : nullptr;
    if (nc) {
      const u64* v = vals + (vals_global ? b : k) * ob * n;
      u64* cf = coef_own + k * ob * n;
      u64* lde_out = R == 1 ? plane_l + b * ob * m : S->d_ldechunk;
      const bool fused = P->ntt_fused || P->ntt_fused512;
      const bool two = P->ntt_two_streams && P->d_tmp2 && (!fused || P->d_tmp3);
      tstream = two ? P->nstream : P->stream;
      int rc;
      if (two && fused) {
        if (k >= 2) HIPC(hipStreamWaitEvent(P->stream, P->chunk_ready[k - 2], 0));
        rc = intt_lde_cols_fused(P, v, cf, lde_out, nc, (k & 1) ? P->d_tmp3 : P->d_tmp2, P->nstream, P->intt_done[k]);
      } else if (two) {
        rc = ntt_columns(P, v, n, cf, n, P->d_tmp, m, nc, P->degree_bits, true, n, nullptr, nullptr, host_inv_pow2(P->degree_bits));
        if (rc) return rc;
        HIPC(hipEventRecord(P->intt_done[k], P->stream));
        HIPC(hipStreamWaitEvent(P->nstream, P->intt_done[k], 0));
        rc = ntt_columns(P, cf, n, lde_out, m, P->d_tmp2, m, nc, P->lde_log, false, n, P->d_shift, nullptr, 1, P->nstream);
      } else rc = intt_lde_cols(P, v, cf, lde_out, nc);
      if (rc) return rc;
      if (R > 1 && k >= 2) HIPC(hipStreamWaitEvent(tstream, S->xchg_done[k - 2], 0));
      if (R > 1)
        hipLaunchKernelGGL(split_pack_kernel, dim3((unsigned)((m + 255) / 256), (unsigned)nc), dim3(256), 0, tstream, S->d_ldechunk, m, (u32)nc, (u32)ob, S->log_r, me,
                           slot, slot_n, plane_l + b * ob * ml, plane_n ? plane_n + b * ob * ml : nullptr);
      HIPC(hipGetLastError());
    }
    HIPC(hipEventRecord(P->chunk_ready[k], tstream));
    hipEvent_t arrived = P->chunk_ready[k];
    if (R > 1) {
      HIPC(hipStreamWaitEvent(S->cstream, P->chunk_ready[k], 0));
      for (u32 pl = 0; pl < S->planes; pl++) {
        const u64* dst = pl ? plane_n : plane_l;
        std::vector<uint64_t> so(R, 0), sl(R, 0), ro(R, 0), rl(R, 0);
        for (u32 r = 0; r < R; r++) {
          if (r == me) continue;
          so[r] = (uint64_t)((const char*)(slot + ((size_t)pl * R + r) * ob * ml) - sbase);
          sl[r] = (uint64_t)(nc * ml * sizeof(u64));
          const size_t br = k * R + r;
          ro[r] = (uint64_t)((const char*)(dst + br * ob * ml) - rbase);
          rl[r] = (uint64_t)(sh.block_cols(br) * ml * sizeof(u64));
        }
        int rc = split_exchange(P, S->cstream, so, sl, ro, rl);
        if (rc) return rc;
      }
      HIPC(hipEventRecord(S->xchg_done[k], S->cstream));
      arrived = S->xchg_done[k];
    }
    HIPC(hipStreamWaitEvent(P->hstream, arrived, 0));
    const size_t c_begin = k * R * ob, c_end = std::min(sh.total, (k + 1) * R * ob);
    for (size_t c0 = c_begin; c0 < c_end; c0 += ob) {
      const size_t ncs = std::min(ob, c_end - c0);
      hipLaunchKernelGGL(leaf_absorb_kernel, dim3((unsigned)((ml + 255) / 256)), dim3(256), 0, P->hstream, plane_l + c0 * ml, ml, row_log, (u32)ncs,
                         P->d_sponge, c0 == 0 ? 1 : 0, c0 + ncs == sh.total ? 1 : 0, t.d,
                         (c0 + ncs < sh.total && sh.total - (c0 + ncs) >= 8) ? 1 : 0);
    }
    HIPC(hipGetLastError());
  }
  int rc = tree_build_inner(P, t, P->hstream);
  if (rc) return rc;
  HIPC(hipEventRecord(P->hash_done, P->hstream));
  HIPC(hipStreamWaitEvent(P->stream, P->hash_done, 0));
  return 0;
}
static int split_cap_to_host(sbn_prover* P, const DevTree& t, std::vector<u64>& cap) {
  SplitCtx* S = P->sp;
  const size_t capn = (size_t)1 << P->cfg.cap_height, own = capn >> S->log_r;
  std::vector<u64> mine(own * 4);
  HIPC(hipMemcpyAsync(mine.data(), t.level(t.nlevels), own * 4 * sizeof(u64), hipMemcpyDeviceToHost, P->stream));
  HIPC(stream_wait(P->stream));
  cap.resize(capn * 4);
  return split_all_gather_host(P, mine.data(), cap.data(), own * 4 * sizeof(u64));
}
static int absorb_times(sbn_prover* P, size_t ncols, int ex_ms) {
  size_t nchunks = (ncols + P->ntt_chunk - 1) / P->ntt_chunk;
  float tot = 0;
  for (size_t k = 0; k < nchunks; k++) { float ms = 0; HIPC(hipEventElapsedTime(&ms, P->abs_ev[2 * k], P->abs_ev[2 * k + 1])); tot += ms; }
  P->stage_ms[ST_COUNT + ex_ms] = tot;
  return 0;
}
static int tree_cap_to_host(sbn_prover* P, const DevTree& t, std::vector<u64>& cap, bool first_bad = false) {
  size_t capn = (size_t)1 << P->cfg.cap_height;
  cap.resize(capn * 4);
  HIPC(hipMemcpyAsync(cap.data(), t.level(t.nlevels), capn * 4 * sizeof(u64), hipMemcpyDeviceToHost, P->stream));
  if (first_bad) HIPC(hipMemcpyAsync(P->h_first_bad, P->d_first_bad, sizeof(unsigned long long), hipMemcpyDeviceToHost, P->stream));
  HIPC(stream_wait(P->stream));
  return 0;
}

static constexpr size_t SPLIT_BLOCK = 64;
static int split_sizes(const AirShape& as, u32 degree_bits, u32 rate_bits, u32 world, size_t ob, uint64_t* send_bytes, uint64_t* recv_bytes, size_t* scratch_words,
                       size_t* slot_words) {
  const size_t n = (size_t)1 << degree_bits, m = n << rate_bits;
  const u32 planes = world >= 4 ? 2 : 1;
  const size_t sw = std::max<size_t>(2 * m, 2 * n * world);
  const size_t slot = world > 1 ? (size_t)planes * ob * m : 0;
  *send_bytes = (uint64_t)(std::max(std::max(2 * slot, 2 * (m / world)), 2 * n) * sizeof(u64));
  *recv_bytes = (uint64_t)(((as.ncols + as.nzs) * (m / world) * planes + sw) * sizeof(u64));
  *scratch_words = sw;
  if (slot_words) *slot_words = slot;
  return 0;
}
static int create_ctx(const sbn_air_desc* air, const sbn_config* cfg, uint32_t degree_bits, const sbn_comm* comm, sbn_prover** out);
extern "C" int sbn_prover_create(const sbn_air_desc* air, const sbn_config* cfg, uint32_t degree_bits, sbn_prover** out) {
  return create_ctx(air, cfg, degree_bits, nullptr, out);
}
static int create_ctx(const sbn_air_desc* air, const sbn_config* cfg, uint32_t degree_bits, const sbn_comm* comm, sbn_prover** out) {
  if (!air || !cfg || !out) return fail(SBN_ERR_BAD_ARG, "null argument");
  *out = nullptr;
  if (!config_supported(cfg)) return fail(SBN_ERR_UNSUPPORTED, "unsupported StarkConfig (need num_challenges=2, rate_bits=1)");
  AirShape as;
  if (!air_shape(air, cfg, as)) return fail(SBN_ERR_BAD_ARG, "unknown air kind / num_io");
  if (degree_bits < 9 || degree_bits > 22) return fail(SBN_ERR_UNSUPPORTED, "degree_bits out of range");
  if (as.kind == SBN_AIR_FLAGS && (512 * (size_t)as.num_io) != ((size_t)1 << degree_bits)) return fail(SBN_ERR_BAD_ARG, "FlagStark needs 512*num_io rows");
  if (as.kind == SBN_AIR_FLAGS_U64 && (128 * (size_t)as.num_io) != ((size_t)1 << degree_bits)) return fail(SBN_ERR_BAD_ARG, "the u64 FlagStark needs 128*num_io rows");
  if (is_exp_air(as.kind)) {
    if ((exp_rows_per_instance(as.kind) * as.num_io) != ((size_t)1 << degree_bits)) return fail(SBN_ERR_BAD_ARG, "the Exp tables need 512*num_io rows (FQ12_EXP_U64: 128*num_io)");
    if (as.kind != SBN_AIR_FQ12_EXP && as.kind != SBN_AIR_FQ12_EXP_U64 && degree_bits < 16)
      return fail(SBN_ERR_UNSUPPORTED, "G1_EXP / G2_EXP / FQ_EXP need >= 2^16 rows (u16 range check, range_check.rs:26)");
  }
  if (int rc = use_current_device("the prover path has no CPU fallback")) return rc;
  sbn_prover* P = new sbn_prover();
  P->air = as; P->cfg = *cfg; P->degree_bits = degree_bits; P->lde_log = degree_bits + cfg->rate_bits;
  P->n = (size_t)1 << degree_bits; P->m = (size_t)1 << P->lde_log;
  P->fri = fri_shape(*cfg, degree_bits);
  P->device = g_device;
  int rc = 0;
  auto acc = [&](int r) { if (!rc) rc = r; };
  auto hipc = [&](hipError_t e, const char* what) { if (e != hipSuccess && !rc) rc = fail(SBN_ERR_HIP, "%s failed: %s", what, hipGetErrorString(e)); };
  if (P->fri.total_arity() > degree_bits + cfg->rate_bits - cfg->cap_height) { sbn_prover_destroy(P); return fail(SBN_ERR_UNSUPPORTED, "FRI total reduction arity is too large"); }
  P->ntt_chunk = P->lde_log >= 18 ? 48 : 64;
  {
    std::string serr;
    if (!P->set.load(serr)) { sbn_prover_destroy(P); return fail(SBN_ERR_BAD_ARG, "%s", serr.c_str()); }
  }
  const Settings& set = P->set;
  if (set.ntt_chunk) P->ntt_chunk = (size_t)set.ntt_chunk;
  ntt_plan(P);
  if (P->ntt_fused512 && !set.ntt_chunk) P->ntt_chunk = 40;
  P->chain_mode = set.device_chain >= 0 ? set.device_chain : ((tracegen_host_chains_vectorized() || tracegen_host_threads() >= 8) ? 0 : 2);
  acc(ntt_fast_setup());
  hipc(hipStreamCreate(&P->stream), "hipStreamCreate");
  hipc(hipStreamCreate(&P->hstream), "hipStreamCreate");
  P->ntt_two_streams = P->lde_log >= 19;
  if (P->ntt_two_streams) {
    hipc(hipStreamCreate(&P->nstream), "hipStreamCreate");
    for (auto& e : P->intt_done) hipc(hipEventCreateWithFlags(&e, hipEventDisableTiming), "hipEventCreate");
  }
  for (auto& e : P->ev) hipc(hipEventCreate(&e), "hipEventCreate");
  for (auto& e : P->abs_ev) hipc(hipEventCreate(&e), "hipEventCreate");
  for (auto& e : P->chunk_ready) hipc(hipEventCreateWithFlags(&e, hipEventDisableTiming), "hipEventCreate");
  hipc(hipEventCreateWithFlags(&P->hash_done, hipEventDisableTiming), "hipEventCreate");
  for (auto& v : P->stage_ms) v = 0;
  if (rc) { sbn_prover_destroy(P); return rc; }
  const size_t n = P->n, m = P->m, C = as.ncols, Z = as.nzs;
  if (comm && (C <= 4 || Z == 0)) { sbn_prover_destroy(P); return fail(SBN_ERR_UNSUPPORTED, "the split prover covers the wide tables (this one has %zu columns and %zu permutation Zs)", C, Z); }
  if (comm) {
    const u32 R = comm->world;
    u32 lr = 0; while ((1u << lr) < R) lr++;
    uint64_t sb = 0, rb = 0; size_t sw = 0, slotw = 0;
    if (comm->struct_size != sizeof(sbn_comm)) { sbn_prover_destroy(P); return fail(SBN_ERR_BAD_ARG, "sbn_comm.struct_size does not match this library (ABI %d)", SBN_ABI_VERSION); }
    if (!set.ntt_chunk) P->ntt_chunk = SPLIT_BLOCK;
    if (P->ntt_chunk != SPLIT_BLOCK) { sbn_prover_destroy(P); return fail(SBN_ERR_UNSUPPORTED, "the split prover deals columns in blocks of %zu: unset SBN_NTT_CHUNK", SPLIT_BLOCK); }
    split_sizes(as, degree_bits, cfg->rate_bits, R, SPLIT_BLOCK, &sb, &rb, &sw, &slotw);
    if ((1u << lr) != R || lr > cfg->cap_height || comm->rank >= R || !comm->all_to_all || !comm->all_gather_host || !comm->send_buf || !comm->recv_buf ||
        comm->send_bytes < sb || comm->recv_bytes < rb) {
      sbn_prover_destroy(P);
      return fail(SBN_ERR_BAD_ARG, "bad sbn_comm (world must be a power of two <= 2^cap_height; staging buffers of sbn_split_exchange_bytes)");
    }
    for (const void* buf : {(const void*)comm->send_buf, (const void*)comm->recv_buf}) {
      hipPointerAttribute_t pa{};
      if (hipPointerGetAttributes(&pa, buf) != hipSuccess || pa.device != P->device) {
        (void)hipGetLastError();
        sbn_prover_destroy(P);
        return fail(SBN_ERR_BAD_ARG, "sbn_comm staging buffers do not live on this prover's device %d (call sbn_set_device before creating the transport)", g_device);
      }
    }
    SplitCtx* S = P->sp = new SplitCtx();
    for (auto& e : S->xchg_done) e = nullptr;
    S->comm = *comm; S->log_r = lr; S->rho = bitrev32(comm->rank, lr); S->ml = m >> lr; S->planes = R >= 4 ? 2 : 1;
    S->slot_words = slotw;
    S->cs.total = C; S->cs.ob = SPLIT_BLOCK; S->cs.R = R; S->cs.rank = comm->rank;
    S->zs = S->cs; S->zs.total = Z;
    S->cr = S->cs.own(); S->zr = S->zs.own();
    hipc(hipStreamCreate(&S->cstream), "hipStreamCreate");
    for (auto& e : S->xchg_done) hipc(hipEventCreateWithFlags(&e, hipEventDisableTiming), "hipEventCreate");
    S->tev.assign(2 * (2 * (S->cs.steps() + S->zs.steps()) + 8), nullptr);
    for (auto& e : S->tev) hipc(hipEventCreate(&e), "hipEventCreate");
    u64* rbuf = (u64*)comm->recv_buf;
    S->lde_l = rbuf; rbuf += C * S->ml;
    if (S->planes == 2) { S->lde_n = rbuf; rbuf += C * S->ml; }
    S->zlde_l = rbuf; rbuf += Z * S->ml;
    if (S->planes == 2) { S->zlde_n = rbuf; rbuf += Z * S->ml; }
    S->scratch = rbuf; S->scratch_words = sw;
    P->lde_scratch_words = (size_t)(rb / sizeof(u64));
    acc(dmalloc(&P->d_trace, C * n, &P->dev_bytes)); acc(dmalloc(&P->d_coef, std::max<size_t>(S->cr, 1) * n, &P->dev_bytes));
    acc(dmalloc(&P->d_zval, std::max<size_t>(S->zr, 1) * n, &P->dev_bytes)); acc(dmalloc(&P->d_zcoef, std::max<size_t>(S->zr, 1) * n, &P->dev_bytes));
    acc(dmalloc(&S->d_ldechunk, P->ntt_chunk * m, &P->dev_bytes));
    hipc(hipMalloc((void**)&S->d_idx_local, cfg->num_query_rounds * sizeof(u32)), "hipMalloc"); P->dev_bytes += cfg->num_query_rounds * sizeof(u32);
    acc(tree_alloc(P->tree_t, S->ml, cfg->cap_height - lr, &P->dev_bytes)); acc(tree_alloc(P->tree_z, S->ml, cfg->cap_height - lr, &P->dev_bytes));
  } else {
    P->lde_scratch_words = C * m;
    acc(dmalloc(&P->d_trace, C * n, &P->dev_bytes)); acc(dmalloc(&P->d_coef, C * n, &P->dev_bytes)); acc(dmalloc(&P->d_lde, C * m, &P->dev_bytes));
    acc(dmalloc(&P->d_zval, std::max<size_t>(Z, 1) * n, &P->dev_bytes)); acc(dmalloc(&P->d_zcoef, std::max<size_t>(Z, 1) * n, &P->dev_bytes)); acc(dmalloc(&P->d_zlde, std::max<size_t>(Z, 1) * m, &P->dev_bytes));
    acc(tree_alloc(P->tree_t, m, cfg->cap_height, &P->dev_bytes)); acc(tree_alloc(P->tree_z, m, cfg->cap_height, &P->dev_bytes));
  }
  acc(dmalloc(&P->d_tmp, std::max(P->ntt_chunk, (size_t)4) * m, &P->dev_bytes));
  if (P->ntt_fused || P->ntt_fused512 || P->ntt_two_streams) acc(dmalloc(&P->d_tmp2, std::max(P->ntt_chunk, (size_t)4) * m, &P->dev_bytes));
  if ((P->ntt_fused || P->ntt_fused512) && P->ntt_two_streams) acc(dmalloc(&P->d_tmp3, std::max(P->ntt_chunk, (size_t)4) * m, &P->dev_bytes));
  acc(dmalloc(&P->d_q, 2 * m, &P->dev_bytes)); acc(dmalloc(&P->d_qlde, 4 * m, &P->dev_bytes));
  acc(tree_alloc(P->tree_q, m, cfg->cap_height, &P->dev_bytes));
  acc(dmalloc(&P->d_tw_f, m, &P->dev_bytes)); acc(dmalloc(&P->d_tw_i, m, &P->dev_bytes)); acc(dmalloc(&P->d_shift, m, &P->dev_bytes)); acc(dmalloc(&P->d_shift_inv, m, &P->dev_bytes));
  if (P->ntt_fused512) acc(dmalloc(&P->d_shift_odd, n, &P->dev_bytes));
  acc(dmalloc(&P->d_xs, m, &P->dev_bytes)); acc(dmalloc(&P->d_lag_first, m, &P->dev_bytes)); acc(dmalloc(&P->d_lag_last, m, &P->dev_bytes));
  P->apow_n = apow_len(as.nconstraints, as.nzs);
  acc(dmalloc(&P->d_apow, (size_t)SBN_NCH * P->apow_n, &P->dev_bytes));
  acc(dmalloc(&P->d_zpow, 4 * n, &P->dev_bytes)); acc(dmalloc(&P->d_open, (C + Z + 4) * 4, &P->dev_bytes));
  hipc(hipHostMalloc((void**)&P->h_open, (C + Z + 4) * 4 * sizeof(u64), hipHostMallocDefault), "hipHostMalloc");
  hipc(hipHostMalloc((void**)&P->h_open2, (C + Z) * 4 * sizeof(u64), hipHostMallocDefault), "hipHostMalloc");
  acc(dmalloc(&P->d_part, 2 * 32 * n, &P->dev_bytes)); acc(dmalloc(&P->d_w, 4096, &P->dev_bytes)); acc(dmalloc(&P->d_sponge, 12 * m, &P->dev_bytes));
  acc(dmalloc(&P->d_fa, 4 * n, &P->dev_bytes)); acc(dmalloc(&P->d_fcoef, 2 * m, &P->dev_bytes)); acc(dmalloc(&P->d_fcoef2, 2 * m, &P->dev_bytes));
  acc(dmalloc(&P->d_pow, 1, &P->dev_bytes));
  if (rc) { sbn_prover_destroy(P); return rc; }
  P->d_fb = P->d_fa + 2 * n;
  hipc(hipMalloc((void**)&P->d_pic, sizeof(ExpPiConsts<F>)), "hipMalloc"); P->dev_bytes += sizeof(ExpPiConsts<F>);
  hipc(hipMalloc((void**)&P->d_idx, cfg->num_query_rounds * sizeof(u32)), "hipMalloc"); P->dev_bytes += cfg->num_query_rounds * sizeof(u32);
  {
    u32 bits = P->lde_log;
    for (u32 ab : P->fri.arity_bits) {
      u64* v = nullptr; acc(dmalloc(&v, 2 * ((size_t)1 << bits), &P->dev_bytes)); P->fri_vals.push_back(v);
      DevTree t; acc(tree_alloc(t, (size_t)1 << (bits - ab), cfg->cap_height, &P->dev_bytes)); P->fri_trees.push_back(t);
      bits -= ab;
    }
    if (rc) { sbn_prover_destroy(P); return rc; }
  }
  {
    size_t sib = (size_t)(P->lde_log - cfg->cap_height) * 4;
    size_t s = C + sib + (Z ? Z + sib : 0) + 4 + sib;
    u32 bits = P->lde_log;
    for (u32 ab : P->fri.arity_bits) { bits -= ab; s += 2 * ((size_t)1 << ab) + (size_t)(bits - cfg->cap_height) * 4; }
    P->qstride = s;
    acc(dmalloc(&P->d_qbuf, s * cfg->num_query_rounds, &P->dev_bytes));
    if (rc) { sbn_prover_destroy(P); return rc; }
  }
  auto blocks = [](size_t k) { return dim3((unsigned)((k + 255) / 256)); };
  F w = f_root_of_unity(P->lde_log);
  hipLaunchKernelGGL(pow_table_kernel, blocks(m), dim3(256), 0, P->stream, P->d_tw_f, m, w.v);
  hipLaunchKernelGGL(pow_table_kernel, blocks(m), dim3(256), 0, P->stream, P->d_tw_i, m, f_inv(w).v);
  hipLaunchKernelGGL(pow_table_kernel, blocks(m), dim3(256), 0, P->stream, P->d_shift, m, (u64)GL_GEN);
  hipLaunchKernelGGL(pow_table_kernel, blocks(m), dim3(256), 0, P->stream, P->d_shift_inv, m, f_inv(F(GL_GEN)).v);
  hipLaunchKernelGGL(domain_tables_kernel, blocks(m), dim3(256), 0, P->stream, P->d_xs, P->d_lag_first, P->d_lag_last, m, P->lde_log, degree_bits);
  if (P->d_shift_odd) hipLaunchKernelGGL(shift_odd_table_kernel, blocks(n), dim3(256), 0, P->stream, P->d_shift_odd, n, P->d_shift, P->d_tw_f, 9u);
  {
    std::vector<PairCols> pairs(Z);
    for (size_t z = 0; z < Z; z++) {
      int l, r;
      if (as.kind == SBN_AIR_G1_OP) G1OpShape::pair((int)z, l, r);
      else if (as.kind == SBN_AIR_LOOKUP) LookupShape().pair((int)z, l, r);
      else if (is_op_air(as.kind)) OpShape(as.kind).pair((int)z, l, r);
      else exp_shape(as).pair((int)z, l, r);
      pairs[z].lhs = l; pairs[z].rhs = r;
    }
    hipc(hipMalloc((void**)&P->d_pairs, std::max<size_t>(Z, 1) * sizeof(PairCols)), "hipMalloc"); P->dev_bytes += std::max<size_t>(Z, 1) * sizeof(PairCols);
    if (!rc && Z) hipc(hipMemcpy(P->d_pairs, pairs.data(), Z * sizeof(PairCols), hipMemcpyHostToDevice), "hipMemcpy");
    if (P->sp && P->sp->zr) {
      SplitCtx* S = P->sp;
      std::vector<PairCols> own(S->zr);
      for (size_t l = 0; l < S->zr; l++) own[l] = pairs[S->zs.global_col(S->zs.rank, l)];
      hipc(hipMalloc((void**)&S->d_pairs_own, S->zr * sizeof(PairCols)), "hipMalloc"); P->dev_bytes += S->zr * sizeof(PairCols);
      if (!rc) hipc(hipMemcpy(S->d_pairs_own, own.data(), S->zr * sizeof(PairCols), hipMemcpyHostToDevice), "hipMemcpy");
    }
  }
  hipc(hipStreamSynchronize(P->stream), "hipStreamSynchronize");
  hipc(hipGetLastError(), "table kernels");
  if (rc) { sbn_prover_destroy(P); return rc; }
  *out = P;
  return SBN_OK;
}

namespace sbn { size_t prover_device_bytes(const sbn_prover* P) { return P ? P->dev_bytes : 0; } }
extern "C" void sbn_prover_destroy(sbn_prover* P) {
  if (!P) return;
  (void)hipSetDevice(P->device);
  u64* bufs[] = {P->d_trace, P->d_coef, P->d_lde, P->d_tmp, P->d_tmp2, P->d_tmp3, P->d_zval, P->d_zcoef, P->d_zlde, P->d_q, P->d_qlde, P->tree_t.d, P->tree_z.d,
                 P->tree_q.d, P->d_tw_f, P->d_tw_i, P->d_shift, P->d_shift_inv, P->d_xs, P->d_lag_first, P->d_lag_last, P->d_apow, P->d_zpow,
                 P->d_open, P->d_part, P->d_w, P->d_fa, P->d_fcoef, P->d_fcoef2, P->d_pow, P->d_qbuf, P->d_shift_odd};
  for (u64* b : bufs) if (b) (void)hipFree(b);
  for (u64* b : P->fri_vals) if (b) (void)hipFree(b);
  for (auto& t : P->fri_trees) if (t.d) (void)hipFree(t.d);
  if (P->sp) {
    if (P->sp->d_ldechunk) (void)hipFree(P->sp->d_ldechunk);
    if (P->sp->d_idx_local) (void)hipFree(P->sp->d_idx_local);
    if (P->sp->d_pairs_own) (void)hipFree(P->sp->d_pairs_own);
    for (auto& e : P->sp->xchg_done) if (e) (void)hipEventDestroy(e);
    for (auto& e : P->sp->tev) if (e) (void)hipEventDestroy(e);
    if (P->sp->cstream) (void)hipStreamDestroy(P->sp->cstream);
    delete P->sp;
  }
  if (P->d_pic) (void)hipFree(P->d_pic);
  if (P->d_idx) (void)hipFree(P->d_idx);
  if (P->d_pairs) (void)hipFree(P->d_pairs);
  for (auto& e : P->ev) if (e) (void)hipEventDestroy(e);
  for (auto& e : P->abs_ev) if (e) (void)hipEventDestroy(e);
  for (auto& e : P->chunk_ready) if (e) (void)hipEventDestroy(e);
  if (P->hash_done) (void)hipEventDestroy(P->hash_done);
  if (P->d_sponge) (void)hipFree(P->d_sponge);
  if (P->h_chain) (void)hipHostFree(P->h_chain);
  if (P->h_io) (void)hipHostFree(P->h_io);
  if (P->h_open) (void)hipHostFree(P->h_open);
  if (P->h_open2) (void)hipHostFree(P->h_open2);
  if (P->ustream) (void)hipStreamSynchronize(P->ustream);
  for (auto& e : P->upload_done) if (e) (void)hipEventDestroy(e);
  for (auto& e : P->slot_copied) if (e) (void)hipEventDestroy(e);
  if (P->h_ring) (void)hipHostFree(P->h_ring);
  if (P->h_first_bad) (void)hipHostFree(P->h_first_bad);
  if (P->d_first_bad) (void)hipFree(P->d_first_bad);
  if (P->ustream) (void)hipStreamDestroy(P->ustream);
  if (P->hstream) (void)hipStreamDestroy(P->hstream);
  if (P->nstream) { (void)hipStreamDestroy(P->nstream); for (auto& e : P->intt_done) if (e) (void)hipEventDestroy(e); }
  if (P->stream) (void)hipStreamDestroy(P->stream);
  delete P;
}

static int check_pi(sbn_prover* P, const uint64_t* pi, size_t n_pi) {
  if (n_pi != P->air.npi) return fail(SBN_ERR_BAD_ARG, "expected %zu public inputs, got %zu", P->air.npi, n_pi);
  if (n_pi && !pi) return fail(SBN_ERR_BAD_ARG, "null public inputs");
  for (size_t i = 0; i < n_pi; i++) if (pi[i] >= GLP) return fail(SBN_ERR_NON_CANONICAL, "public input %zu is not canonical", i);
  P->pi.assign(pi, pi + n_pi);
  return 0;
}
extern "C" int sbn_prover_load_trace(sbn_prover* P, const uint64_t* trace, const uint64_t* pi, size_t n_pi) {
  if (!P || !trace) return fail(SBN_ERR_BAD_ARG, "null argument");
  int rc = check_pi(P, pi, n_pi); if (rc) return rc;
  size_t words = P->air.ncols * P->n;
  {
    unsigned nt = tracegen_host_threads(); if (nt == 0) nt = 1; if (nt > 16) nt = 16;
    std::atomic<size_t> bad(words);
    std::vector<std::thread> th;
    size_t per = (words + nt - 1) / nt;
    for (unsigned t = 0; t < nt; t++)
      th.emplace_back([&, t] {
        size_t a = t * per, b = std::min(words, a + per);
        for (size_t i = a; i < b; i++) if (trace[i] >= GLP) { size_t cur = bad.load(); while (i < cur && !bad.compare_exchange_weak(cur, i)) {} break; }
      });
    for (auto& x : th) x.join();
    if (bad.load() < words) return fail(SBN_ERR_NON_CANONICAL, "trace word %zu is not canonical", bad.load());
  }
  HIPC(hipSetDevice(P->device));
  HIPC(hipMemcpy(P->d_trace, trace, words * sizeof(u64), hipMemcpyHostToDevice));
  P->loaded = true;
  return SBN_OK;
}
extern "C" int sbn_prover_load_trace_device(sbn_prover* P, const uint64_t* d_trace, const uint64_t* pi, size_t n_pi) {
  if (!P || !d_trace) return fail(SBN_ERR_BAD_ARG, "null argument");
  int rc = check_pi(P, pi, n_pi); if (rc) return rc;
  HIPC(hipSetDevice(P->device));
  if (d_trace != P->d_trace) HIPC(hipMemcpy(P->d_trace, d_trace, P->air.ncols * P->n * sizeof(u64), hipMemcpyDeviceToDevice));
  P->loaded = true;
  return SBN_OK;
}

extern "C" int sbn_prover_read_trace(sbn_prover* P, uint64_t* out) {
  if (!P || !out) return fail(SBN_ERR_BAD_ARG, "null argument");
  if (!P->loaded) return fail(SBN_ERR_BAD_ARG, "no trace loaded");
  HIPC(hipSetDevice(P->device));
  HIPC(hipMemcpy(out, P->d_trace, P->air.ncols * P->n * sizeof(u64), hipMemcpyDeviceToHost));
  return SBN_OK;
}
extern "C" uint64_t* sbn_prover_trace_device_ptr(sbn_prover* P) {
  if (!P) return nullptr;
  (void)hipSetDevice(P->device);
  return P->d_trace;
}

extern "C" int sbn_prover_stage_times(const sbn_prover* P, float* ms, int cap) {
  if (!P || !ms) return 0;
  int k = std::min(cap, (int)(ST_COUNT + EX_COUNT));
  for (int i = 0; i < k; i++) ms[i] = P->stage_ms[i];
  return k;
}
extern "C" const char* sbn_prover_stage_name(int i) { return (i >= 0 && i < ST_COUNT + EX_COUNT) ? STAGE_NAMES[i] : ""; }

template <int KIND>
static void launch_quotient_kind(sbn_prover* P, const QuotientParams& qp, size_t qblocks) {
  const dim3 g1((unsigned)qblocks, 1), g2((unsigned)qblocks, 2);
  if (qp.seg_mask & 12u) hipLaunchKernelGGL((quotient_kernel<KIND, 2>), g2, dim3(256), 0, P->hstream, qp, qp.apow[0], qp.apow[1], qp.pic);
  if (qp.seg_mask & 1u) hipLaunchKernelGGL((quotient_kernel<KIND, 0>), g1, dim3(256), 0, P->stream, qp, qp.apow[0], qp.apow[1], qp.pic);
  if (qp.seg_mask & 2u) hipLaunchKernelGGL((quotient_kernel<KIND, 1>), g1, dim3(256), 0, P->stream, qp, qp.apow[0], qp.apow[1], qp.pic);
}
static int launch_quotient_parts(sbn_prover* P, const QuotientParams& qp, size_t qblocks) {
  switch (P->air.kind) {
    case SBN_AIR_G1_OP: launch_quotient_kind<1>(P, qp, qblocks); break;
    case SBN_AIR_G1_EXP: launch_quotient_kind<2>(P, qp, qblocks); break;
    case SBN_AIR_G2_EXP: launch_quotient_kind<3>(P, qp, qblocks); break;
    case SBN_AIR_FQ_EXP: launch_quotient_kind<5>(P, qp, qblocks); break;
    case SBN_AIR_FQ12_EXP_U64: launch_quotient_kind<6>(P, qp, qblocks); break;
    case SBN_AIR_MODULAR: launch_quotient_kind<7>(P, qp, qblocks); break;
    case SBN_AIR_FQ12_MUL: launch_quotient_kind<8>(P, qp, qblocks); break;
    case SBN_AIR_LOOKUP: launch_quotient_kind<9>(P, qp, qblocks); break;
    case SBN_AIR_FLAGS: launch_quotient_kind<10>(P, qp, qblocks); break;
    case SBN_AIR_FLAGS_U64: launch_quotient_kind<11>(P, qp, qblocks); break;
    default: launch_quotient_kind<4>(P, qp, qblocks); break;
  }
  HIPC(hipGetLastError());
  return 0;
}

static int prove_impl(sbn_prover* P, sbn_proof** out, const HostUpload* up) {
  if (!P || !out) return fail(SBN_ERR_BAD_ARG, "null argument");
  *out = nullptr;
  if (!up && !P->loaded && !(P->sp && P->sp->comm.world > 1)) return fail(SBN_ERR_BAD_ARG, "no trace loaded");
  HIPC(hipSetDevice(P->device));
  hipStream_t st = P->stream;
  const size_t n = P->n, m = P->m, C = P->air.ncols, Z = P->air.nzs;
  const sbn_config& cfg = P->cfg;
  const size_t capw = ((size_t)1 << cfg.cap_height) * 4;
  auto blocks = [](size_t k) { return dim3((unsigned)((k + 255) / 256)); };
  int rc;
  Challenger ch;
  std::vector<u64> trace_cap, z_cap, q_cap;

  HIPC(hipEventRecord(P->ev[ST_TRACE_COMMIT], st));
  SplitCtx* const S = P->sp;
  struct DeadlineScope { ~DeadlineScope() { t_wait_deadline_s = 0; } } deadline_scope;
  if (S && S->comm.world > 1) {
    t_wait_deadline_s = P->set.comm_timeout_s;
    std::vector<uint32_t> st_all(S->comm.world, 0);
    const uint32_t mine = P->loaded ? 1u : 0u;
    if ((rc = split_all_gather_host(P, &mine, st_all.data(), sizeof(uint32_t)))) return rc;
    for (u32 r = 0; r < S->comm.world; r++) if (!st_all[r]) return fail(SBN_ERR_BAD_ARG, "split proof abandoned: rank %u has no trace loaded", r);
  }
  if (!up && !P->loaded) return fail(SBN_ERR_BAD_ARG, "no trace loaded");
  if (up) HIPC(hipMemsetAsync(P->d_first_bad, 0xff, sizeof(unsigned long long), P->ustream));
  if (S) {
    S->tev_used = 0;
    if ((rc = commit_split(P, S->cs, P->d_trace, true, P->d_coef, S->lde_l, S->lde_n, P->tree_t))) return rc;
  } else if ((rc = commit_pipeline(P, P->d_trace, P->d_coef, P->d_lde, C, P->tree_t, EX_TRACE_ABSORB_MS, EX_TRACE_ABSORB_LAUNCHES, up))) return rc;
  HIPC(hipEventRecord(P->ev[ST_PERM_Z], st));
  if ((rc = S ? split_cap_to_host(P, P->tree_t, trace_cap) : tree_cap_to_host(P, P->tree_t, trace_cap, up != nullptr))) return rc;
  if (up && *P->h_first_bad != ~0ull) return fail(SBN_ERR_NON_CANONICAL, "trace word %zu is not canonical", (size_t)*P->h_first_bad);
  ch.observe_words(trace_cap.data(), capw);

  F gam[2][2] = {};
  if (Z) for (int s = 0; s < 2; s++) for (int c = 0; c < (int)cfg.num_challenges; c++) { (void)ch.challenge(); gam[s][c] = ch.challenge(); }
  const F gamma0 = gam[0][0], gamma1 = gam[1][1];
  {
    const size_t zn = S ? S->zr : Z;
    const PairCols* pairs = S ? S->d_pairs_own : P->d_pairs;
    auto launch_z = [&](size_t z0, size_t cnt, hipStream_t s) {
      if (cnt == 0) return;
      const PairCols* pp = pairs + z0; u64* out = P->d_zval + z0 * n;
      const size_t chunks = n / 2048;
      if (n >= 8192 && n % 2048 == 0 && cnt <= 65535 && cnt * chunks * 4 <= 2 * 32 * n) {
        u64* tot = P->d_part; u64* pq = P->d_part + cnt * chunks * 2;
        hipLaunchKernelGGL(permz_chunk_products_kernel<8>, dim3((unsigned)chunks, (unsigned)cnt), dim3(256), 0, s, P->d_trace, n, pp, gamma0.v, gamma1.v, tot);
        hipLaunchKernelGGL(permz_chunk_scan_kernel, dim3((unsigned)cnt), dim3(64), 0, s, tot, (u32)chunks, pq);
        hipLaunchKernelGGL(permz_chunk_write_kernel<8>, dim3((unsigned)chunks, (unsigned)cnt), dim3(256), 0, s, P->d_trace, n, pp, gamma0.v, gamma1.v, pq, out);
        return;
      }
      if (n % 2048 == 0) hipLaunchKernelGGL(permutation_z_kernel<8>, dim3((unsigned)cnt), dim3(256), 0, s, P->d_trace, n, pp, gamma0.v, gamma1.v, out);
      else if (n % 1024 == 0) hipLaunchKernelGGL(permutation_z_kernel<4>, dim3((unsigned)cnt), dim3(256), 0, s, P->d_trace, n, pp, gamma0.v, gamma1.v, out);
      else hipLaunchKernelGGL(permutation_z_kernel<2>, dim3((unsigned)cnt), dim3(256), 0, s, P->d_trace, n, pp, gamma0.v, gamma1.v, out);
    };
    launch_z(0, zn, st);
  }
  HIPC(hipGetLastError());
  HIPC(hipEventRecord(P->ev[ST_Z_COMMIT], st));
  if (S) {
    if ((rc = commit_split(P, S->zs, P->d_zval, false, P->d_zcoef, S->zlde_l, S->zlde_n, P->tree_z))) return rc;
  } else {
    if (C > 4) if ((rc = absorb_times(P, C, EX_TRACE_ABSORB_MS))) return rc;
    if (Z) if ((rc = commit_pipeline(P, P->d_zval, P->d_zcoef, P->d_zlde, Z, P->tree_z, EX_Z_ABSORB_MS, EX_Z_ABSORB_LAUNCHES))) return rc;
  }
  HIPC(hipEventRecord(P->ev[ST_QUOTIENT_EVAL], st));
  if (Z) {
    if ((rc = S ? split_cap_to_host(P, P->tree_z, z_cap) : tree_cap_to_host(P, P->tree_z, z_cap))) return rc;
    ch.observe_words(z_cap.data(), capw);
  }

  F alphas[SBN_NCH];
  for (int j = 0; j < SBN_NCH; j++) alphas[j] = ch.challenge();
  {
    const size_t APN = P->apow_n;
    std::vector<u64> apow((size_t)SBN_NCH * APN);
    std::vector<F> ap[SBN_NCH];
    for (int j = 0; j < SBN_NCH; j++) {
      ap[j].resize(APN);
      F a(1);
      for (size_t k = 0; k < APN; k++) { ap[j][k] = a; apow[(size_t)j * APN + k] = a.v; a = a * alphas[j]; }
    }
    HIPC(hipMemcpyAsync(P->d_apow, apow.data(), apow.size() * sizeof(u64), hipMemcpyHostToDevice, st));
    if (is_exp_air(P->air.kind)) {
      static thread_local ExpPiConsts<F> pic;
      const F* app[SBN_NCH] = {ap[0].data(), ap[1].data()};
      std::vector<F> pif(P->pi.size());
      for (size_t i = 0; i < pif.size(); i++) pif[i] = F(P->pi[i]);
      exp_pi_consts<F>(exp_shape(P->air), app, pif.data(), pic);
      HIPC(hipMemcpyAsync(P->d_pic, &pic, sizeof(pic), hipMemcpyHostToDevice, st));
    }
    HIPC(stream_wait(st));
  }
  {
    QuotientParams qp{};
    qp.lde = P->d_lde; qp.zlde = P->d_zlde; qp.m = m; qp.next_step = 2;
    qp.lde_next = qp.lde; qp.zlde_next = qp.zlde; qp.row_shift = 0; qp.row_rho = 0;
    if (S) {
      qp.lde = S->lde_l; qp.zlde = S->zlde_l; qp.m = S->ml; qp.row_shift = S->log_r; qp.row_rho = S->rho;
      qp.lde_next = S->planes == 2 ? S->lde_n : S->lde_l; qp.zlde_next = S->planes == 2 ? S->zlde_n : S->zlde_l;
      qp.next_step = S->comm.world == 1 ? 2 : (S->comm.world == 2 ? 1 : 0);
    }
    qp.xs = P->d_xs; qp.lag_first = P->d_lag_first; qp.lag_last = P->d_lag_last;
    F gn = f_exp_pow2(F(GL_GEN), P->degree_bits);
    qp.zh_inv[0] = f_inv(gn - F(1)).v; qp.zh_inv[1] = f_inv(-gn - F(1)).v;
    qp.last = f_inv(f_root_of_unity(P->degree_bits)).v;
    for (int j = 0; j < SBN_NCH; j++) { qp.alpha[j] = alphas[j].v; qp.apow[j] = P->d_apow + (size_t)j * P->apow_n; }
    qp.gamma0 = gamma0.v; qp.gamma1 = gamma1.v; qp.num_zs = (int)Z; qp.num_io = (int)P->air.num_io; qp.pic = P->d_pic; qp.qout = P->d_q;
    if (S) qp.qout = (u64*)S->comm.send_buf;
    qp.part = P->d_part;
    {
      qp.zsplit = (int)(Z / 2);
      qp.lookups_in_perm = P->set.quotient_lookups == 1;
      const u64 n_tail = is_exp_air(P->air.kind) ? (u64)ExpShape(exp_e(P->air.kind), (int)P->air.num_io).num_tail_constraints() : 0;
      const u64 after[4] = {n_tail + 2 * (u64)Z, 2 * (u64)Z, 0, 0};
      qp.seg_count[0] = (int)(P->air.nconstraints - n_tail); qp.seg_count[1] = (int)n_tail;
      qp.seg_count[2] = qp.seg_count[3] = 2 * (int)Z;
      for (int sgm = 0; sgm < 4; sgm++) for (int j = 0; j < SBN_NCH; j++) qp.seg_shift[sgm][j] = f_pow(alphas[j], after[sgm]).v;
    }
    const size_t qblocks = (qp.m + 255) / 256;
    qp.seg_mask = 0xfu;
#ifdef SBN_DIAG
    { const char* e = std::getenv("SBN_DIAG_QUOTIENT_SEGMASK"); if (e) qp.seg_mask = (u32)atoi(e) & 0xfu; }
    if (qp.seg_mask != 0xfu) HIPC(hipMemsetAsync(qp.part, 0, (size_t)QSEG * SBN_NCH * qp.m * sizeof(u64), st));
#endif
    HIPC(hipEventRecord(P->chunk_ready[3], st));
    HIPC(hipStreamWaitEvent(P->hstream, P->chunk_ready[3], 0));
    if ((rc = launch_quotient_parts(P, qp, qblocks))) return rc;
    HIPC(hipEventRecord(P->hash_done, P->hstream));
    HIPC(hipStreamWaitEvent(st, P->hash_done, 0));
    hipLaunchKernelGGL(quotient_combine_kernel, blocks(qp.m), dim3(256), 0, st, qp);
    HIPC(hipGetLastError());
    if (S) {
      if ((rc = split_all_gather_device(P, 2 * S->ml))) return rc;
      hipLaunchKernelGGL(split_unpack_rows_kernel, blocks(m), dim3(256), 0, st, S->scratch, m, 2u, S->log_r, P->d_q);
      HIPC(hipGetLastError());
    } else if (Z > 4) { if ((rc = absorb_times(P, Z, EX_Z_ABSORB_MS))) return rc; }
  }
  HIPC(hipEventRecord(P->ev[ST_QUOTIENT_COMMIT], st));
  if ((rc = ntt_columns(P, P->d_q, m, P->d_q, m, P->d_tmp, m, 2, P->lde_log, true, m, nullptr, P->d_shift_inv, host_inv_pow2(P->lde_log)))) return rc;
  if ((rc = lde_coeffs(P, P->d_q, P->d_qlde, 4))) return rc;
  if ((rc = tree_from_matrix(P, P->tree_q, P->d_qlde, 4))) return rc;
  HIPC(hipEventRecord(P->ev[ST_OPENINGS], st));
  if ((rc = tree_cap_to_host(P, P->tree_q, q_cap))) return rc;
  ch.observe_words(q_cap.data(), capw);

  E2 zeta = ch.ext_challenge();
  F g = f_root_of_unity(P->degree_bits);
  if (e2_exp_pow2(zeta, P->degree_bits) == E2(F(1), F(0))) return fail(SBN_ERR_HIP, "opening point is in the subgroup");
  E2 zeta_next = zeta * g;
  hipLaunchKernelGGL(ext_pow_table_kernel, blocks(n), dim3(256), 0, st, P->d_zpow, P->d_zpow + n, n, zeta.a.v, zeta.b.v);
  hipLaunchKernelGGL(ext_pow_table_kernel, blocks(n), dim3(256), 0, st, P->d_zpow + 2 * n, P->d_zpow + 3 * n, n, zeta_next.a.v, zeta_next.b.v);
  const u64* open = P->h_open;
  const u64* open2 = P->h_open2;
  if (S && S->comm.world > 1) {
    const u64 *zp0 = P->d_zpow, *zp1 = P->d_zpow + n, *zp2 = P->d_zpow + 2 * n, *zp3 = P->d_zpow + 3 * n;
    auto open_k = n % 1024 == 0 ? openings_kernel<4> : openings_kernel<1>;
    if (S->cr) hipLaunchKernelGGL(open_k, dim3((unsigned)S->cr), dim3(256), 0, st, P->d_coef, n, zp0, zp1, zp2, zp3, P->d_open);
    if (S->zr) hipLaunchKernelGGL(open_k, dim3((unsigned)S->zr), dim3(256), 0, st, P->d_zcoef, n, zp0, zp1, zp2, zp3, P->d_open + C * 4);
    hipLaunchKernelGGL(open_k, dim3(4), dim3(256), 0, st, P->d_q, n, zp0, zp1, zp2, zp3, P->d_open + (C + Z) * 4);
    HIPC(hipGetLastError());
    HIPC(hipMemcpyAsync(P->h_open, P->d_open, (C + Z + 4) * 4 * sizeof(u64), hipMemcpyDeviceToHost, st));
    HIPC(hipEventRecord(P->ev[ST_FRI_COMBINE], st));
    HIPC(stream_wait(st));
    const u32 R = S->comm.world;
    const size_t cmax = S->cs.max_own(), zmax = S->zs.max_own(), per = (cmax + zmax) * 4;
    std::vector<u64> mine(per, 0), all((size_t)R * per);
    memcpy(mine.data(), P->h_open, S->cr * 4 * sizeof(u64));
    memcpy(mine.data() + cmax * 4, P->h_open + C * 4, S->zr * 4 * sizeof(u64));
    if ((rc = split_all_gather_host(P, mine.data(), all.data(), per * sizeof(u64)))) return rc;
    for (u32 r = 0; r < R; r++) {
      const u64* src = all.data() + (size_t)r * per;
      for (size_t l = 0, cnt = S->cs.own_cols(r); l < cnt; l++) memcpy(P->h_open + S->cs.global_col(r, l) * 4, src + l * 4, 4 * sizeof(u64));
      for (size_t l = 0, cnt = S->zs.own_cols(r); l < cnt; l++) memcpy(P->h_open + (C + S->zs.global_col(r, l)) * 4, src + (cmax + l) * 4, 4 * sizeof(u64));
    }
    open2 = open;
    for (size_t p = 0; p < C + Z + 4; p++) { ch.observe(F(open[4 * p])); ch.observe(F(open[4 * p + 1])); }
    for (size_t p = 0; p < C + Z; p++) { ch.observe(F(open[4 * p + 2])); ch.observe(F(open[4 * p + 3])); }
  } else {
    const bool u4 = n % 1024 == 0;
    auto open1_k = u4 ? openings1_kernel<4> : openings1_kernel<1>;
    const u64 *zp0 = P->d_zpow, *zp1 = P->d_zpow + n, *zp2 = P->d_zpow + 2 * n, *zp3 = P->d_zpow + 3 * n;
    size_t sl[5] = {0, C / 16, C / 16 + C / 8, C / 16 + C / 8 + C / 4, C};
    for (int k = 0; k < 4; k++) {
      const size_t a = sl[k], cnt = sl[k + 1] - sl[k];
      if (cnt) {
        hipLaunchKernelGGL(open1_k, dim3((unsigned)cnt), dim3(256), 0, st, P->d_coef + a * n, n, zp0, zp1, P->d_open + a * 4, 0u);
        HIPC(hipMemcpyAsync(P->h_open + a * 4, P->d_open + a * 4, cnt * 4 * sizeof(u64), hipMemcpyDeviceToHost, st));
      }
      HIPC(hipEventRecord(P->chunk_ready[8 + k], st));
    }
    if (Z) hipLaunchKernelGGL(open1_k, dim3((unsigned)Z), dim3(256), 0, st, P->d_zcoef, n, zp0, zp1, P->d_open + C * 4, 0u);
    hipLaunchKernelGGL(open1_k, dim3(4), dim3(256), 0, st, P->d_q, n, zp0, zp1, P->d_open + (C + Z) * 4, 0u);
    HIPC(hipMemcpyAsync(P->h_open + C * 4, P->d_open + C * 4, (Z + 4) * 4 * sizeof(u64), hipMemcpyDeviceToHost, st));
    HIPC(hipEventRecord(P->chunk_ready[1], st));
    size_t sn[5] = {0, C / 4, C / 2, C / 2 + C / 4, C};
    for (int k = 0; k < 4; k++) {
      const size_t a = sn[k], cnt = sn[k + 1] - sn[k];
      if (cnt) {
        hipLaunchKernelGGL(open1_k, dim3((unsigned)cnt), dim3(256), 0, st, P->d_coef + a * n, n, zp2, zp3, P->d_open + a * 4, 2u);
        HIPC(hipMemcpyAsync(P->h_open2 + a * 4, P->d_open + a * 4, cnt * 4 * sizeof(u64), hipMemcpyDeviceToHost, st));
      }
      HIPC(hipEventRecord(P->chunk_ready[12 + k], st));
    }
    if (Z) hipLaunchKernelGGL(open1_k, dim3((unsigned)Z), dim3(256), 0, st, P->d_zcoef, n, zp2, zp3, P->d_open + C * 4, 2u);
    HIPC(hipGetLastError());
    HIPC(hipMemcpyAsync(P->h_open2 + C * 4, P->d_open + C * 4, Z * 4 * sizeof(u64), hipMemcpyDeviceToHost, st));
    HIPC(hipEventRecord(P->ev[ST_FRI_COMBINE], st));
    for (int k = 0; k < 4; k++) {
      HIPC(event_wait(P->chunk_ready[8 + k]));
      for (size_t p = sl[k]; p < sl[k + 1]; p++) { ch.observe(F(open[4 * p])); ch.observe(F(open[4 * p + 1])); }
    }
    HIPC(event_wait(P->chunk_ready[1]));
    for (size_t p = C; p < C + Z + 4; p++) { ch.observe(F(open[4 * p])); ch.observe(F(open[4 * p + 1])); }
    for (int k = 0; k < 4; k++) {
      HIPC(event_wait(P->chunk_ready[12 + k]));
      for (size_t p = sn[k]; p < sn[k + 1]; p++) { ch.observe(F(open2[4 * p + 2])); ch.observe(F(open2[4 * p + 3])); }
    }
    HIPC(stream_wait(st));
    for (size_t p = C; p < C + Z; p++) { ch.observe(F(open2[4 * p + 2])); ch.observe(F(open2[4 * p + 3])); }
  }

  E2 fri_alpha = ch.ext_challenge();
  {
    const u32 RW = S ? S->comm.world : 1;
    const u32 GS = RW > 1 ? (u32)SPLIT_BLOCK : 128;
    std::vector<u64> wall;
    auto plan = [&](u32 npoly, E2 weight0, u64 stride) { size_t off = wall.size(); u32 ng = (npoly + GS - 1) / GS; E2 ag = e2_pow(fri_alpha, stride), cur = weight0;
                                                         for (u32 k = 0; k < ng; k++) { wall.push_back(cur.a.v); wall.push_back(cur.b.v); cur = cur * ag; } return off; };
    const size_t tc0 = S ? (size_t)S->comm.rank * GS : 0, tcn = S ? S->cr : C, tzn = S ? S->zr : Z;
    const u64 gstride = (u64)GS * RW;
    size_t w_t = tcn ? plan((u32)tcn, e2_pow(fri_alpha, RW > 1 ? tc0 : 0), gstride) : 0, w_z = tzn ? plan((u32)tzn, e2_pow(fri_alpha, C + (RW > 1 ? tc0 : 0)), gstride) : 0,
           w_q = plan(4, e2_pow(fri_alpha, C + Z), GS);
    if (wall.size() > 4096) return fail(SBN_ERR_UNSUPPORTED, "too many FRI combine groups");
    HIPC(hipMemcpyAsync(P->d_w, wall.data(), wall.size() * sizeof(u64), hipMemcpyHostToDevice, st));
    hipLaunchKernelGGL(ext_pow_table_kernel, dim3(1), dim3(GS), 0, st, P->d_apow, P->d_apow + GS, (size_t)GS, fri_alpha.a.v, fri_alpha.b.v);
    auto combine = [&](const u64* coeffs, u32 npoly, size_t woff, u64* oa, u64* ob, int accumulate) -> int {
      u32 ng = (npoly + GS - 1) / GS;
      for (u32 g0 = 0; g0 < ng; g0 += 32) {
        u32 gc = std::min<u32>(32, ng - g0);
        hipLaunchKernelGGL(fri_combine_partial_kernel, dim3((unsigned)((n + 255) / 256), gc), dim3(256), 0, st, coeffs + (size_t)g0 * GS * n, n,
                           npoly - g0 * GS, GS, P->d_apow, P->d_apow + GS, P->d_part, P->d_part + 32 * n);
        hipLaunchKernelGGL(fri_combine_reduce_kernel, blocks(n), dim3(256), 0, st, P->d_part, P->d_part + 32 * n, n, gc, P->d_w + woff + 2 * g0, oa, ob,
                           (accumulate || g0 > 0) ? 1 : 0);
      }
      HIPC(hipGetLastError());
      return 0;
    };
    u64 *f1a = P->d_fb, *f1b = P->d_fb + n, *f0a = P->d_fa, *f0b = P->d_fa + n;
    if (!tcn) HIPC(hipMemsetAsync(f1a, 0, 2 * n * sizeof(u64), st));
    if (tcn) if ((rc = combine(P->d_coef, (u32)tcn, w_t, f1a, f1b, 0))) return rc;
    if (tzn) if ((rc = combine(P->d_zcoef, (u32)tzn, w_z, f1a, f1b, 1))) return rc;
    if (S) {
      HIPC(hipMemcpyAsync(S->comm.send_buf, f1a, 2 * n * sizeof(u64), hipMemcpyDeviceToDevice, st));
      if ((rc = split_all_gather_device(P, 2 * n))) return rc;
      hipLaunchKernelGGL(split_modadd_kernel, blocks(2 * n), dim3(256), 0, st, S->scratch, 2 * n, S->comm.world, f1a);
      HIPC(hipGetLastError());
    }
    HIPC(hipMemcpyAsync(f0a, f1a, 2 * n * sizeof(u64), hipMemcpyDeviceToDevice, st));
    if ((rc = combine(P->d_q, 4, w_q, f0a, f0b, 1))) return rc;
    HIPC(stream_wait(st));
    HIPC(hipMemsetAsync(P->d_fcoef, 0, 2 * m * sizeof(u64), st));
    E2 shift2 = e2_pow(fri_alpha, C + Z);
    auto divide = [&](const u64* ca, const u64* cb, E2 z, E2 mul, int accumulate) {
      const size_t nch = n / DBL_CHUNK;
      u64 *ha = P->d_part, *hb = P->d_part + nch;
      hipLaunchKernelGGL(divide_by_linear_pass1, blocks(nch), dim3(256), 0, st, ca, cb, nch, z.a.v, z.b.v, ha, hb);
      hipLaunchKernelGGL(divide_by_linear_pass2, dim3(1), dim3(256), 0, st, ha, hb, nch, z.a.v, z.b.v);
      hipLaunchKernelGGL(divide_by_linear_pass3, blocks(nch), dim3(256), 0, st, ca, cb, nch, z.a.v, z.b.v, ha, hb, mul.a.v, mul.b.v, P->d_fcoef, P->d_fcoef + m, accumulate, fri_times_x(cfg));
    };
    divide(f0a, f0b, zeta, E2{F(0), F(0)}, 0);
    divide(f1a, f1b, zeta_next, shift2, 1);
    HIPC(hipGetLastError());
  }
  HIPC(hipEventRecord(P->ev[ST_FRI_LAYERS], st));
  std::vector<std::vector<u64>> fri_caps;
  std::vector<u64> final_poly;
  {
    u32 bits = P->lde_log;
    u64* coef = P->d_fcoef; u64* coef_alt = P->d_fcoef2;
    size_t clen = m;
    F shift(GL_GEN);
    for (size_t li = 0; li < P->fri.arity_bits.size(); li++) {
      u32 ab = P->fri.arity_bits[li];
      u64* va = P->fri_vals[li]; u64* vb = va + clen;
      HIPC(hipMemcpyAsync(va, coef, 2 * clen * sizeof(u64), hipMemcpyDeviceToDevice, st));
      hipLaunchKernelGGL(scale_pow_kernel, blocks(clen), dim3(256), 0, st, va, clen, shift.v);
      hipLaunchKernelGGL(scale_pow_kernel, blocks(clen), dim3(256), 0, st, vb, clen, shift.v);
      if ((rc = ntt_columns(P, va, clen, va, clen, P->d_tmp, m, 2, bits, false, clen, nullptr, nullptr, 1))) return rc;
      DevTree& t = P->fri_trees[li];
      if (t.nleaf <= 16384) hipLaunchKernelGGL(fri_leaf_hash_coop_kernel, blocks(t.nleaf * 16), dim3(256), 0, st, va, vb, bits, ab, t.d);
      else hipLaunchKernelGGL(fri_leaf_hash_kernel, blocks(t.nleaf), dim3(256), 0, st, va, vb, bits, ab, t.d);
      if ((rc = tree_build_inner(P, t, st))) return rc;
      std::vector<u64> cap;
      if ((rc = tree_cap_to_host(P, t, cap))) return rc;
      ch.observe_words(cap.data(), capw);
      fri_caps.push_back(cap);
      E2 beta = ch.ext_challenge();
      size_t nout = clen >> ab;
      hipLaunchKernelGGL(fri_fold_kernel, blocks(nout), dim3(256), 0, st, coef, coef + clen, nout, 1u << ab, beta.a.v, beta.b.v, coef_alt, coef_alt + nout);
      HIPC(hipGetLastError());
      std::swap(coef, coef_alt);
      clen = nout; bits -= ab;
      shift = f_pow(shift, (u64)1 << ab);
    }
    size_t fl = clen >> cfg.rate_bits;
    final_poly.resize(2 * fl);
    std::vector<u64> fa(fl), fb(fl);
    HIPC(hipMemcpyAsync(fa.data(), coef, fl * sizeof(u64), hipMemcpyDeviceToHost, st));
    HIPC(hipMemcpyAsync(fb.data(), coef + clen, fl * sizeof(u64), hipMemcpyDeviceToHost, st));
    HIPC(stream_wait(st));
    for (size_t i = 0; i < fl; i++) { final_poly[2 * i] = fa[i]; final_poly[2 * i + 1] = fb[i]; ch.observe(F(fa[i])); ch.observe(F(fb[i])); }
  }
  HIPC(hipEventRecord(P->ev[ST_POW], st));
  u64 pow_witness = ~0ULL;
  {
    PowParams pp{};
    for (int i = 0; i < 12; i++) pp.state[i] = ch.st[i].v;
    for (size_t i = 0; i < ch.in.size(); i++) pp.state[i] = ch.in[i].v;
    pp.wpos = (u32)ch.in.size(); pp.min_lz = cfg.proof_of_work_bits; pp.result = P->d_pow;
    u64 base = 0;
    for (int round = 0; pow_witness == ~0ULL; round++) {
      const u64 BATCH = round == 0 ? (1ULL << 17) : (1ULL << 20);
      if (base >= GLP - BATCH) return fail(SBN_ERR_HIP, "proof of work failed");
      u64 init = ~0ULL;
      HIPC(hipMemcpyAsync(P->d_pow, &init, sizeof(u64), hipMemcpyHostToDevice, st));
      pp.base = base; pp.count = BATCH;
      hipLaunchKernelGGL(pow_kernel, blocks(BATCH), dim3(256), 0, st, pp);
      HIPC(hipMemcpyAsync(&pow_witness, P->d_pow, sizeof(u64), hipMemcpyDeviceToHost, st));
      HIPC(stream_wait(st));
      base += BATCH;
    }
    ch.observe(F(pow_witness));
    F resp = ch.challenge();
    u32 lz = resp.v ? (u32)__builtin_clzll(resp.v) : 64;
    if (lz < cfg.proof_of_work_bits) return fail(SBN_ERR_HIP, "proof-of-work witness check failed");
  }
  HIPC(hipEventRecord(P->ev[ST_QUERIES], st));
  const u32 nq = cfg.num_query_rounds;
  std::vector<u64> qwords(P->qstride * nq);
  std::vector<u32> idx(nq), idx_local(nq);
  size_t split_section = 0;
  {
    for (u32 q = 0; q < nq; q++) idx[q] = (u32)(ch.challenge().v % m);
    HIPC(hipMemcpyAsync(P->d_idx, idx.data(), nq * sizeof(u32), hipMemcpyHostToDevice, st));
    size_t off = 0;
    const u32 nsib = P->lde_log - cfg.cap_height;
    auto initial = [&](const u64* mat, size_t ncols, const DevTree& t, size_t rows, u32 log_rows, const u32* d_index) {
      hipLaunchKernelGGL(gather_rows_kernel, dim3((unsigned)((ncols + 255) / 256), nq), dim3(256), 0, st, mat, rows, log_rows, (u32)ncols, d_index, P->d_qbuf, P->qstride, off);
      off += ncols;
      hipLaunchKernelGGL(gather_siblings_kernel, dim3(nq), dim3(128), 0, st, t.d, t.nleaf, nsib, d_index, 0u, P->d_qbuf, P->qstride, off);
      off += (size_t)nsib * 4;
    };
    if (S) {
      for (u32 q = 0; q < nq; q++) idx_local[q] = idx[q] & (u32)(S->ml - 1);
      HIPC(hipMemcpyAsync(S->d_idx_local, idx_local.data(), nq * sizeof(u32), hipMemcpyHostToDevice, st));
      initial(S->lde_l, C, P->tree_t, S->ml, P->lde_log - S->log_r, S->d_idx_local);
      if (Z) initial(S->zlde_l, Z, P->tree_z, S->ml, P->lde_log - S->log_r, S->d_idx_local);
      split_section = off;
    } else {
      initial(P->d_lde, C, P->tree_t, m, P->lde_log, P->d_idx);
      if (Z) initial(P->d_zlde, Z, P->tree_z, m, P->lde_log, P->d_idx);
    }
    initial(P->d_qlde, 4, P->tree_q, m, P->lde_log, P->d_idx);
    u32 bits = P->lde_log, shift = 0;
    for (size_t li = 0; li < P->fri.arity_bits.size(); li++) {
      u32 ab = P->fri.arity_bits[li];
      shift += ab;
      size_t len = (size_t)1 << bits;
      hipLaunchKernelGGL(gather_fri_leaf_kernel, dim3(nq), dim3(64), 0, st, P->fri_vals[li], P->fri_vals[li] + len, bits, ab, P->d_idx, shift, P->d_qbuf, P->qstride, off);
      off += 2 * ((size_t)1 << ab);
      const DevTree& t = P->fri_trees[li];
      hipLaunchKernelGGL(gather_siblings_kernel, dim3(nq), dim3(128), 0, st, t.d, t.nleaf, t.nlevels, P->d_idx, shift, P->d_qbuf, P->qstride, off);
      off += (size_t)t.nlevels * 4;
      bits -= ab;
    }
    HIPC(hipGetLastError());
    if (off != P->qstride) return fail(SBN_ERR_HIP, "internal: query layout mismatch (%zu vs %zu)", off, P->qstride);
    HIPC(hipMemcpyAsync(qwords.data(), P->d_qbuf, qwords.size() * sizeof(u64), hipMemcpyDeviceToHost, st));
  }
  HIPC(hipEventRecord(P->ev[ST_COUNT], st));
  HIPC(stream_wait(st));
  for (int i = 0; i < ST_COUNT; i++) HIPC(hipEventElapsedTime(&P->stage_ms[i], P->ev[i], P->ev[i + 1]));
  if (S) {
    const u32 R = S->comm.world;
    std::vector<u64> mine((size_t)nq * split_section), all((size_t)R * nq * split_section);
    for (u32 q = 0; q < nq; q++) memcpy(mine.data() + (size_t)q * split_section, qwords.data() + (size_t)q * P->qstride, split_section * sizeof(u64));
    if ((rc = split_all_gather_host(P, mine.data(), all.data(), mine.size() * sizeof(u64)))) return rc;
    for (u32 q = 0; q < nq; q++) {
      const u32 owner = idx[q] >> (P->lde_log - S->log_r);
      memcpy(qwords.data() + (size_t)q * P->qstride, all.data() + ((size_t)owner * nq + q) * split_section, split_section * sizeof(u64));
    }
    float xms = 0;
    for (size_t i = 0; i + 1 < S->tev_used; i += 2) { float t = 0; HIPC(hipEventElapsedTime(&t, S->tev[i], S->tev[i + 1])); xms += t; }
    P->stage_ms[ST_COUNT + EX_COMM_MS] = xms;
  }

  sbn_proof* pr = new sbn_proof();
  pr->degree_bits = P->degree_bits;
  std::vector<u64>& w = pr->words;
  w.reserve(12 + 3 * capw + (C + Z + 4) * 4 + fri_caps.size() * capw + qwords.size() + final_poly.size() + 1 + P->pi.size());
  u64 hdr[12] = {PROOF_MAGIC, P->degree_bits, C, Z, 4, P->pi.size(), cfg.cap_height, cfg.rate_bits, fri_caps.size(), cfg.fri_arity_bits,
                 final_poly.size() / 2, nq};
  w.insert(w.end(), hdr, hdr + 12);
  w.insert(w.end(), trace_cap.begin(), trace_cap.end());
  if (Z) w.insert(w.end(), z_cap.begin(), z_cap.end());
  w.insert(w.end(), q_cap.begin(), q_cap.end());
  for (size_t p = 0; p < C; p++) { w.push_back(open[4 * p]); w.push_back(open[4 * p + 1]); }
  for (size_t p = 0; p < C; p++) { w.push_back(open2[4 * p + 2]); w.push_back(open2[4 * p + 3]); }
  for (size_t p = C; p < C + Z; p++) { w.push_back(open[4 * p]); w.push_back(open[4 * p + 1]); }
  for (size_t p = C; p < C + Z; p++) { w.push_back(open2[4 * p + 2]); w.push_back(open2[4 * p + 3]); }
  for (size_t p = C + Z; p < C + Z + 4; p++) { w.push_back(open[4 * p]); w.push_back(open[4 * p + 1]); }
  for (auto& cap : fri_caps) w.insert(w.end(), cap.begin(), cap.end());
  w.insert(w.end(), qwords.begin(), qwords.end());
  w.insert(w.end(), final_poly.begin(), final_poly.end());
  w.push_back(pow_witness);
  w.insert(w.end(), P->pi.begin(), P->pi.end());
  *out = pr;
  return SBN_OK;
}
extern "C" int sbn_prover_prove(sbn_prover* P, sbn_proof** out) { return prove_impl(P, out, nullptr); }

extern "C" int sbn_prover_prove_host_trace(sbn_prover* P, const uint64_t* trace, const uint64_t* pi, size_t n_pi, sbn_proof** out) {
  if (!P || !out) return fail(SBN_ERR_BAD_ARG, "null argument");
  *out = nullptr;
  P->loaded = false;
  if (!trace) return fail(SBN_ERR_BAD_ARG, "null argument");
  if (P->sp) return fail(SBN_ERR_UNSUPPORTED, "sbn_prover_prove_host_trace covers single-GPU provers");
  int rc = check_pi(P, pi, n_pi); if (rc) return rc;
  HIPC(hipSetDevice(P->device));
  if ((rc = upload_setup(P))) return rc;
  const HostUpload up{trace, P->upload_done};
  if ((rc = prove_impl(P, out, &up))) {
    for (hipStream_t s : {P->ustream, P->stream, P->hstream, P->nstream}) if (s) (void)hipStreamSynchronize(s);
    return rc;
  }
  P->loaded = true;
  return SBN_OK;
}

extern "C" int sbn_commit_values(const uint64_t* cols, size_t ncols, size_t n, uint32_t rate_bits, uint32_t cap_height, uint64_t* cap_out,
                                 uint64_t* coeffs_out, uint64_t* lde_out) {
  if (!cols || !cap_out || ncols == 0) return fail(SBN_ERR_BAD_ARG, "null argument");
  if (rate_bits != 1 || n < 512 || (n & (n - 1))) return fail(SBN_ERR_UNSUPPORTED, "need rate_bits=1 and n a power of two >= 512");
  u32 lg = 0; while (((size_t)1 << lg) < n) lg++;
  if (cap_height < 1 || cap_height > 8) return fail(SBN_ERR_UNSUPPORTED, "cap_height must be 1..8");
  sbn_prover P{};
  sbn_standard_fast_config(&P.cfg); P.cfg.cap_height = cap_height;
  P.degree_bits = lg; P.lde_log = lg + 1; P.n = n; P.m = 2 * n; P.ntt_chunk = 64; P.device = g_device;
  if (int rc = use_current_device("no CPU fallback")) return rc;
  { int rc0 = ntt_fast_setup(); if (rc0) return rc0; }
  { std::string serr; if (!P.set.load(serr)) return fail(SBN_ERR_BAD_ARG, "%s", serr.c_str()); }
  ntt_plan(&P);
  HIPC(hipStreamCreate(&P.stream));
  u64 *d_vals = nullptr, *d_coef = nullptr, *d_lde = nullptr;
  int rc = 0;
  rc |= dmalloc(&d_vals, ncols * n); rc |= dmalloc(&d_coef, ncols * n); rc |= dmalloc(&d_lde, ncols * P.m); rc |= dmalloc(&P.d_tmp, 64 * P.m);
  if (P.ntt_fused || P.ntt_fused512) rc |= dmalloc(&P.d_tmp2, 64 * P.m);
  if (P.ntt_fused512) rc |= dmalloc(&P.d_shift_odd, n);
  rc |= dmalloc(&P.d_tw_f, P.m); rc |= dmalloc(&P.d_tw_i, P.m); rc |= dmalloc(&P.d_shift, P.m);
  rc |= tree_alloc(P.tree_t, P.m, cap_height);
  if (!rc) {
    auto blocks = [](size_t k) { return dim3((unsigned)((k + 255) / 256)); };
    F w = f_root_of_unity(P.lde_log);
    hipLaunchKernelGGL(pow_table_kernel, blocks(P.m), dim3(256), 0, P.stream, P.d_tw_f, P.m, w.v);
    hipLaunchKernelGGL(pow_table_kernel, blocks(P.m), dim3(256), 0, P.stream, P.d_tw_i, P.m, f_inv(w).v);
    hipLaunchKernelGGL(pow_table_kernel, blocks(P.m), dim3(256), 0, P.stream, P.d_shift, P.m, (u64)GL_GEN);
    if (P.d_shift_odd) hipLaunchKernelGGL(shift_odd_table_kernel, blocks(n), dim3(256), 0, P.stream, P.d_shift_odd, n, P.d_shift, P.d_tw_f, 9u);
    if (hipMemcpy(d_vals, cols, ncols * n * sizeof(u64), hipMemcpyHostToDevice) != hipSuccess) rc = fail(SBN_ERR_HIP, "H2D failed");
  }
  for (size_t c0 = 0; !rc && c0 < ncols; c0 += P.ntt_chunk) rc = intt_lde_cols(&P, d_vals + c0 * n, d_coef + c0 * n, d_lde + c0 * P.m, std::min(P.ntt_chunk, ncols - c0));
  if (!rc && ncols <= 4) rc = tree_from_matrix(&P, P.tree_t, d_lde, ncols);
  if (!rc && ncols > 4) {
    rc = dmalloc(&P.d_sponge, 12 * P.m);
    for (size_t c0 = 0; !rc && c0 < ncols; c0 += 64) {
      size_t nc = std::min<size_t>(64, ncols - c0);
      hipLaunchKernelGGL(leaf_absorb_kernel, dim3((unsigned)((P.m + 255) / 256)), dim3(256), 0, P.stream, d_lde + c0 * P.m, P.m, P.lde_log, (u32)nc, P.d_sponge,
                         c0 == 0 ? 1 : 0, c0 + 64 >= ncols ? 1 : 0, P.tree_t.d, (c0 + 64 < ncols && ncols - (c0 + 64) >= 8) ? 1 : 0);
    }
    if (!rc) rc = tree_build_inner(&P, P.tree_t, P.stream);
  }
  std::vector<u64> cap;
  if (!rc) rc = tree_cap_to_host(&P, P.tree_t, cap);
  if (!rc) memcpy(cap_out, cap.data(), cap.size() * sizeof(u64));
  if (!rc && coeffs_out && hipMemcpy(coeffs_out, d_coef, ncols * n * sizeof(u64), hipMemcpyDeviceToHost) != hipSuccess) rc = fail(SBN_ERR_HIP, "D2H failed");
  if (!rc && lde_out && hipMemcpy(lde_out, d_lde, ncols * P.m * sizeof(u64), hipMemcpyDeviceToHost) != hipSuccess) rc = fail(SBN_ERR_HIP, "D2H failed");
  for (u64* b : {d_vals, d_coef, d_lde, P.d_tmp, P.d_tmp2, P.d_shift_odd, P.d_tw_f, P.d_tw_i, P.d_shift, P.tree_t.d, P.d_sponge}) if (b) (void)hipFree(b);
  (void)hipStreamDestroy(P.stream);
  return rc;
}

extern "C" int sbn_poseidon_permute_batch(uint64_t* states, size_t count) {
  if (!states) return fail(SBN_ERR_BAD_ARG, "null argument");
  if (int rc = use_current_device("no CPU fallback")) return rc;
  for (size_t i = 0; i < count * 12; i++) if (states[i] >= GLP) return fail(SBN_ERR_NON_CANONICAL, "state word %zu is not canonical", i);
  u64* d = nullptr;
  HIPC(hipMalloc((void**)&d, count * 12 * sizeof(u64)));
  HIPC(hipMemcpy(d, states, count * 12 * sizeof(u64), hipMemcpyHostToDevice));
  hipLaunchKernelGGL(poseidon_batch_kernel, dim3((unsigned)((count + 255) / 256)), dim3(256), 0, 0, d, count);
  HIPC(hipMemcpy(states, d, count * 12 * sizeof(u64), hipMemcpyDeviceToHost));
  (void)hipFree(d);
  return SBN_OK;
}

extern "C" int sbn_field_mul_batch(const uint64_t* a, const uint64_t* b, uint64_t* out, size_t count, int mode) {
  if (!a || !b || !out) return fail(SBN_ERR_BAD_ARG, "null argument");
  if (int rc = use_current_device("no CPU fallback")) return rc;
  if (count == 0) return SBN_OK;
  u64* d = nullptr;
  HIPC(hipMalloc((void**)&d, 3 * count * sizeof(u64)));
  hipError_t e = hipMemcpy(d, a, count * sizeof(u64), hipMemcpyHostToDevice);
  if (e == hipSuccess) e = hipMemcpy(d + count, b, count * sizeof(u64), hipMemcpyHostToDevice);
  if (e == hipSuccess) {
    hipLaunchKernelGGL(field_mul_batch_kernel, dim3((unsigned)((count + 255) / 256)), dim3(256), 0, 0, d, d + count, d + 2 * count, count, mode);
    e = hipMemcpy(out, d + 2 * count, count * sizeof(u64), hipMemcpyDeviceToHost);
  }
  (void)hipFree(d);
  if (e != hipSuccess) return fail(SBN_ERR_HIP, "sbn_field_mul_batch: %s", hipGetErrorString(e));
  return SBN_OK;
}


extern "C" int sbn_first_non_canonical(const uint64_t* words, size_t count, int on_device, uint64_t* index_out) {
  if (!index_out || (!words && count)) return fail(SBN_ERR_BAD_ARG, "null argument");
  *index_out = count;
  if (!on_device) {
    for (size_t i = 0; i < count; i++) if (words[i] >= GLP) { *index_out = i; break; }
    return SBN_OK;
  }
  if (int rc = use_current_device("no CPU fallback")) return rc;
  if (count == 0) return SBN_OK;
  const size_t off = ((size_t)words & 8) ? 1 : 0;
  u64* d = nullptr;
  HIPC(hipMalloc((void**)&d, (2 + off + count) * sizeof(u64)));
  unsigned long long first = ~0ull;
  hipError_t e = hipMemset(d, 0xff, sizeof(u64));
  if (e == hipSuccess) e = hipMemcpy(d + 2 + off, words, count * sizeof(u64), hipMemcpyHostToDevice);
  if (e == hipSuccess) {
    launch_first_non_canonical(d + 2 + off, count, 0, (unsigned long long*)d, 0);
    e = hipGetLastError();
    if (e == hipSuccess) e = hipMemcpy(&first, d, sizeof first, hipMemcpyDeviceToHost);
  }
  (void)hipFree(d);
  if (e != hipSuccess) return fail(SBN_ERR_HIP, "sbn_first_non_canonical: %s", hipGetErrorString(e));
  if (first != ~0ull) *index_out = first;
  return SBN_OK;
}

extern "C" int sbn_poseidon_permute_host(uint64_t* states, size_t count, int use_definition) {
  if (!states) return fail(SBN_ERR_BAD_ARG, "null argument");
  for (size_t i = 0; i < count * 12; i++) if (states[i] >= GLP) return fail(SBN_ERR_NON_CANONICAL, "state word %zu is not canonical", i);
  for (size_t k = 0; k < count; k++) {
    F st[12];
    for (int i = 0; i < 12; i++) st[i] = F(states[12 * k + i]);
    if (use_definition) poseidon_permute_generic(st); else poseidon_permute(st);
    for (int i = 0; i < 12; i++) states[12 * k + i] = st[i].v;
  }
  return SBN_OK;
}

extern "C" int sbn_set_device(int device) {
  int ndev = 0;
  if (hipGetDeviceCount(&ndev) != hipSuccess || device < 0 || device >= ndev) return fail(SBN_ERR_NO_DEVICE, "device %d not available", device);
  HIPC(hipSetDevice(device));
  t_device = device; g_default_device.store(device);
  return SBN_OK;
}
extern "C" int sbn_set_thread_device(int device) {
  int ndev = 0;
  if (hipGetDeviceCount(&ndev) != hipSuccess || device < 0 || device >= ndev) return fail(SBN_ERR_NO_DEVICE, "device %d not available", device);
  HIPC(hipSetDevice(device));
  t_device = device;
  return SBN_OK;
}
extern "C" int sbn_prover_describe(const sbn_prover* P, char* out, size_t cap) {
  if (!P || !out || cap == 0) return fail(SBN_ERR_BAD_ARG, "null argument");
  const Settings& s = P->set;
  static const char* const CH[] = {"host_pool", "device_lane", "device_wave"};
  const char* chain = P->chain_mode == 0 && tracegen_host_chains_vectorized() ? "host_pool_ifma_x8" : CH[P->chain_mode < 0 || P->chain_mode > 2 ? 0 : P->chain_mode];
  char buf[1024];
  snprintf(buf, sizeof buf,
           "abi=%d device=%d ntt_chunk=%zu ntt_fused=%d ntt_streams=%d ntt_split1024=%d "
           "curve_chains=%s host_threads=%u fq12_host_chain=%d fq12_row_kernel=%d range_check=%d quotient_lookups=%d comm_timeout_s=%g experimental=%d ignored=[%s]",
           SBN_ABI_VERSION, P->device, P->ntt_chunk, (int)(P->ntt_fused || P->ntt_fused512), P->ntt_two_streams ? 2 : 1, P->d_shift_odd ? 1 : 0,
           chain, tracegen_host_threads(), (int)s.fq12_host_chain,
           (int)s.fq12_row_kernel, s.range_check, s.quotient_lookups, s.comm_timeout_s, (int)s.experimental, s.ignored.c_str());
  snprintf(out, cap, "%s", buf);
  return SBN_OK;
}
extern "C" int sbn_device_count(void) { int n = 0; return hipGetDeviceCount(&n) == hipSuccess ? n : 0; }

struct sbn_split_prover { sbn_prover* P; };
extern "C" int sbn_split_exchange_bytes(const sbn_air_desc* air, const sbn_config* cfg, uint32_t degree_bits, uint32_t world, uint64_t* send_bytes,
                                        uint64_t* recv_bytes) {
  if (!air || !cfg || !send_bytes || !recv_bytes || world == 0) return fail(SBN_ERR_BAD_ARG, "null argument");
  AirShape as;
  if (!air_shape(air, cfg, as)) return fail(SBN_ERR_BAD_ARG, "unknown air kind / num_io");
  size_t sw;
  return split_sizes(as, degree_bits, cfg->rate_bits, world, SPLIT_BLOCK, send_bytes, recv_bytes, &sw, nullptr);
}
extern "C" int sbn_split_prover_create(const sbn_air_desc* air, const sbn_config* cfg, uint32_t degree_bits, const sbn_comm* comm, sbn_split_prover** out) {
  if (!out || !comm) return fail(SBN_ERR_BAD_ARG, "null argument");
  *out = nullptr;
  sbn_prover* P = nullptr;
  int rc = create_ctx(air, cfg, degree_bits, comm, &P);
  if (rc) return rc;
  *out = new sbn_split_prover{P};
  return SBN_OK;
}
extern "C" void sbn_split_prover_destroy(sbn_split_prover* sp) {
  if (!sp) return;
  sbn_prover_destroy(sp->P);
  delete sp;
}
extern "C" int sbn_split_prover_generate_trace(sbn_split_prover* sp, const uint32_t* ios, size_t num_io, uint64_t* pi_out) {
  if (!sp) return fail(SBN_ERR_BAD_ARG, "null argument");
  return sbn_prover_generate_trace(sp->P, ios, num_io, pi_out);
}
extern "C" int sbn_split_prover_load_trace(sbn_split_prover* sp, const uint64_t* trace, const uint64_t* pi, size_t n_pi) {
  if (!sp) return fail(SBN_ERR_BAD_ARG, "null argument");
  return sbn_prover_load_trace(sp->P, trace, pi, n_pi);
}
extern "C" int sbn_split_prover_prove(sbn_split_prover* sp, sbn_proof** out) {
  if (!sp) return fail(SBN_ERR_BAD_ARG, "null argument");
  return sbn_prover_prove(sp->P, out);
}
extern "C" int sbn_split_prover_stage_times(const sbn_split_prover* sp, float* ms_out, int cap) {
  if (!sp) return 0;
  return sbn_prover_stage_times(sp->P, ms_out, cap);
}
```

### starky_bn254_amd/csrc/prover_ctx.hpp

```cpp
#pragma once
#include "host_common.hpp"
#include "settings.hpp"
#include <algorithm>

using namespace sbn;
struct PairCols;

#define HIPC(expr)                                                                                   \
  do {                                                                                               \
    hipError_t e_ = (expr);                                                                          \
    if (e_ != hipSuccess) return fail(SBN_ERR_HIP, "%s failed: %s (%s:%d)", #expr, hipGetErrorString(e_), __FILE__, __LINE__); \
  } while (0)

enum Stage {
  ST_TRACE_COMMIT, ST_PERM_Z, ST_Z_COMMIT, ST_QUOTIENT_EVAL, ST_QUOTIENT_COMMIT,
  ST_OPENINGS, ST_FRI_COMBINE, ST_FRI_LAYERS, ST_POW, ST_QUERIES, ST_COUNT
};
enum Extra { EX_TRACE_ABSORB_MS, EX_TRACE_ABSORB_LAUNCHES, EX_Z_ABSORB_MS, EX_Z_ABSORB_LAUNCHES, EX_TRACEGEN_MS, EX_COMM_MS, EX_COUNT };
static constexpr int MAX_CHUNKS = 512;
static constexpr int UPLOAD_SLOTS = 4;
static constexpr size_t UPLOAD_SLOT_WORDS = (size_t)2 << 20;
static constexpr int SBN_MAX_DEVICES = 64;

struct DevTree {
  u64* d = nullptr; size_t nleaf = 0; u32 nlevels = 0;
  u64* level(u32 l) const { return d + (2 * nleaf - ((2 * nleaf) >> l)) * 4; }
};

struct ColShare {
  size_t total = 0, ob = 64; u32 R = 1, rank = 0;
  size_t nblocks() const { return (total + ob - 1) / ob; }
  size_t steps() const { return (nblocks() + R - 1) / R; }
  size_t block_cols(size_t b) const { return b < nblocks() ? std::min(ob, total - b * ob) : 0; }
  size_t own_cols(u32 r) const { size_t s = 0; for (size_t b = r; b < nblocks(); b += R) s += block_cols(b); return s; }
  size_t own() const { return own_cols(rank); }
  size_t max_own() const { size_t s = 0; for (u32 r = 0; r < R; r++) s = std::max(s, own_cols(r)); return s; }
  size_t global_col(u32 r, size_t local) const { return ((local / ob) * R + r) * ob + local % ob; }
};
struct SplitCtx {
  sbn_comm comm;
  u32 log_r = 0, rho = 0;
  size_t ml = 0;
  ColShare cs, zs;
  size_t cr = 0, zr = 0;
  u32 planes = 1;
  u64 *lde_l = nullptr, *lde_n = nullptr, *zlde_l = nullptr, *zlde_n = nullptr, *scratch = nullptr;
  size_t scratch_words = 0;
  size_t slot_words = 0;
  u64* d_ldechunk = nullptr;
  u32* d_idx_local = nullptr;
  PairCols* d_pairs_own = nullptr;
  hipStream_t cstream = nullptr;
  hipEvent_t xchg_done[MAX_CHUNKS];
  std::vector<hipEvent_t> tev;
  size_t tev_used = 0;
};

struct sbn_prover {
  AirShape air; sbn_config cfg; FriShape fri;
  SplitCtx* sp = nullptr;
  size_t lde_scratch_words = 0;
  u32 degree_bits, lde_log; size_t n, m;
  int device; hipStream_t stream;
  u64 *d_trace = nullptr, *d_coef = nullptr, *d_lde = nullptr, *d_tmp = nullptr;
  u64 *d_zval = nullptr, *d_zcoef = nullptr, *d_zlde = nullptr;
  u64 *d_q = nullptr, *d_qlde = nullptr;
  DevTree tree_t, tree_z, tree_q;
  std::vector<DevTree> fri_trees;
  u64 *d_tw_f = nullptr, *d_tw_i = nullptr, *d_shift = nullptr, *d_shift_inv = nullptr;
  u64 *d_shift_odd = nullptr;
  u64 *d_xs = nullptr, *d_lag_first = nullptr, *d_lag_last = nullptr;
  u64 *d_apow = nullptr;
  size_t apow_n = 0;
  void* d_pic = nullptr;
  PairCols* d_pairs = nullptr;
  u64 *d_zpow = nullptr;
  u64 *d_open = nullptr;
  u64 *d_part = nullptr;
  u64 *d_w = nullptr;
  u64 *d_fa = nullptr, *d_fb = nullptr;
  u64 *d_fcoef = nullptr;
  u64 *d_fcoef2 = nullptr;
  std::vector<u64*> fri_vals;
  u64 *d_pow = nullptr;
  u32 *d_idx = nullptr;
  u64 *d_qbuf = nullptr; size_t qstride = 0;
  std::vector<u64> pi;
  bool loaded = false;
  hipEvent_t ev[ST_COUNT + 1];
  float stage_ms[ST_COUNT + EX_COUNT];
  size_t ntt_chunk;
  bool ntt_fused = false;
  u64* d_tmp2 = nullptr;
  u64* d_tmp3 = nullptr;
  bool ntt_fused512 = false;
  hipStream_t hstream = nullptr;
  hipStream_t nstream = nullptr;
  hipEvent_t intt_done[MAX_CHUNKS];
  bool ntt_two_streams = false;
  Settings set;
  int chain_mode = 0;
  hipEvent_t chunk_ready[MAX_CHUNKS];
  hipEvent_t abs_ev[2 * MAX_CHUNKS];
  hipEvent_t hash_done;
  u64* d_sponge = nullptr;
  u64* h_chain = nullptr;
  size_t h_chain_words = 0;
  u64* h_io = nullptr;
  size_t h_io_words = 0;
  u64* h_open = nullptr;
  u64* h_open2 = nullptr;
  size_t dev_bytes = 0;
  hipStream_t ustream = nullptr;
  hipEvent_t upload_done[MAX_CHUNKS];
  hipEvent_t slot_copied[UPLOAD_SLOTS];
  bool slot_used[UPLOAD_SLOTS] = {};
  unsigned slot_next = 0;
  u64* h_ring = nullptr;
  unsigned long long* d_first_bad = nullptr;
  unsigned long long* h_first_bad = nullptr;
};
```

Baseline: 44.13.

## Fold inverse-NTT scale into twiddles and use lighter butterflies on canonical inputs

Precomputes an inverse root table pre-multiplied by 1/n so the inverse NTT's first pass applies the scale through its twiddles, removing the separate per-element scale multiply in the second pass and in the fused kernels. Adds add1/sub1 butterflies that do a single carry correction, used in a new canonical-input template path of the fast NTT pass and in the first DFT-16 stage. Also rewrites mul_pow2 for exponents above 64 as one reduction instead of two. The lighter butterflies assume canonical inputs, so a host-side canonicity check over the input columns is added, which costs a host loop per call.

After: 44.34, median of 2. Within noise of the previous version (+0.5%).

```diff
diff --git a/starky_bn254_amd/csrc/kernels.cuh b/starky_bn254_amd/csrc/kernels.cuh
--- a/starky_bn254_amd/csrc/kernels.cuh
+++ b/starky_bn254_amd/csrc/kernels.cuh
@@ -7,6 +7,10 @@
 __global__ void pow_table_kernel(u64* out, size_t n, u64 base) {
   size_t i = (size_t)blockIdx.x * blockDim.x + threadIdx.x;
   if (i < n) out[i] = f_pow(F(base), i).v;
+}
+__global__ void pow_table_scaled_kernel(u64* out, size_t n, u64 base, u64 scale) {
+  size_t i = (size_t)blockIdx.x * blockDim.x + threadIdx.x;
+  if (i < n) out[i] = (F(scale) * f_pow(F(base), i)).v;
 }
 __global__ void shift_odd_table_kernel(u64* out, size_t n, const u64* __restrict__ shift, const u64* __restrict__ tw, u32 log_s) {
   size_t i = (size_t)blockIdx.x * blockDim.x + threadIdx.x;
@@ -221,7 +225,15 @@
   size_t i = (size_t)blockIdx.x * blockDim.x + threadIdx.x;
   if (i >= count) return;
 #if defined(__HIP_DEVICE_COMPILE__)
-  out[i] = mode ? nw::canon(nw::canon(nw::mul(a[i], b[i]))) : (F(a[i]) * F(b[i])).v;
+  const u64 x = a[i], y = b[i];
+  switch (mode) {
+    case 0: out[i] = (F(x) * F(y)).v; break;
+    case 2: out[i] = nw::canon(nw::add1(x, y)); break;
+    case 3: out[i] = nw::canon(nw::sub1(x, y)); break;
+    case 4: out[i] = nw::canon(nw::mul_pow2<72>(x)); break;
+    case 5: out[i] = nw::canon(nw::mul_pow2<84>(x)); break;
+    default: out[i] = nw::canon(nw::canon(nw::mul(x, y))); break;
+  }
 #endif
 }
 __global__ void poseidon_batch_kernel(u64* states, size_t count) {
diff --git a/starky_bn254_amd/csrc/kernels_ntt.cuh b/starky_bn254_amd/csrc/kernels_ntt.cuh
--- a/starky_bn254_amd/csrc/kernels_ntt.cuh
+++ b/starky_bn254_amd/csrc/kernels_ntt.cuh
@@ -13,6 +13,7 @@
   u32 twiddle;
   const u64* tw;
   u32 tw_log;
+  const u64* tw_ab;
   const u64* pre;
   const u64* post;
   u64 scale;
@@ -100,6 +101,16 @@
   u32 l3 = subco(l2, selm1(k4), k5); u32 h3 = subb0(h2, k5, k6);
   return pack(l3, h3);
 }
+__device__ __forceinline__ u64 add1(u64 a, u64 b) {
+  u64 k1, k2, k3; u32 lo = addco(lo32(a), lo32(b), k1); u32 hi = addc(hi32(a), hi32(b), k1, k2);
+  return madm1(sel01(k2), pack(lo, hi), k3);
+}
+__device__ __forceinline__ u64 sub1(u64 a, u64 b) {
+  u64 k1, k2, k3, k4;
+  u32 lo = subco(lo32(a), lo32(b), k1); u32 hi = subb(hi32(a), hi32(b), k1, k2);
+  u32 l2 = subco(lo, selm1(k2), k3); u32 h2 = subb0(hi, k3, k4);
+  return pack(l2, h2);
+}
 __device__ __forceinline__ u64 red32(u64 lo, u32 hi) { u64 k; u64 t = madm1(hi, lo, k); u64 k2; return madm1(sel01(k), t, k2); }
 __device__ __forceinline__ u64 red(u64 lo, u64 hi) {
   u64 k1, k2, k3, k4, k5, k6;
@@ -114,26 +125,37 @@
   else if constexpr (E < 32) return red32(x << E, hi32(x) >> (32 - E));
   else if constexpr (E == 32) return red32(pack(0, lo32(x)), hi32(x));
   else if constexpr (E < 64) return red(pack(0, lo32(x) << (E - 32)), x >> (64 - E));
-  else return mul_pow2<E - 48>(mul_pow2<48>(x));
+  else {
+    static_assert(E > 64 && E < 96, "2^64 itself is not used by the DFT-16");
+    constexpr int e = E - 64;
+    const u64 T = x >> (32 - e);
+    u64 k1, k2, k3, k4; u32 nl, nh;
+    asm("v_sub_co_u32_e64 %0, %1, 1, %2" : "=v"(nl), "=s"(k1) : "v"(lo32(T)));
+    asm("v_subb_co_u32_e64 %0, %1, -1, %2, %3" : "=v"(nh), "=s"(k2) : "v"(hi32(T)), "s"(k1));
+    const u64 r = madm1(lo32(x) << e, pack(nl, nh), k3);
+    return madm1(sel01(k3), r, k4);
+  }
 }
 __device__ __forceinline__ u64 mul(u64 a, u64 b) { return gl_mul_weak(a, b); }
 __device__ __forceinline__ u64 canon(u64 x) { return gp::canon(x); }
 #else
-__device__ __forceinline__ u64 add(u64 a, u64 b) {
+GL_HD u64 add(u64 a, u64 b) {
   u64 s = a + b;
   u64 c = s < a ? GLEPS : 0;
   s += c;
   if (s < c) s += GLEPS;
   return s;
 }
-__device__ __forceinline__ u64 sub(u64 a, u64 b) {
+GL_HD u64 sub(u64 a, u64 b) {
   u64 d = a - b;
   u64 c = a < b ? GLEPS : 0;
   u64 r = d - c;
   if (d < c) r -= GLEPS;
   return r;
 }
-__device__ __forceinline__ u64 red(u64 lo, u64 hi) {
+GL_HD u64 add1(u64 a, u64 b) { u64 s = a + b; return s + (s < a ? GLEPS : 0); }
+GL_HD u64 sub1(u64 a, u64 b) { u64 d = a - b; return d - (a < b ? GLEPS : 0); }
+GL_HD u64 red(u64 lo, u64 hi) {
   u32 hi_hi = (u32)(hi >> 32), hi_lo = (u32)hi;
   u64 t0 = lo - hi_hi;
   if (lo < hi_hi) t0 -= GLEPS;
@@ -142,27 +164,45 @@
   if (r < t1) r += GLEPS;
   return r;
 }
-template <int E> __device__ __forceinline__ u64 mul_pow2(u64 x) {
+template <int E> GL_HD u64 mul_pow2(u64 x) {
   if constexpr (E == 0) return x;
   else if constexpr (E < 64) return red(x << E, x >> (64 - E));
-  else return mul_pow2<E - 48>(mul_pow2<48>(x));
-}
-__device__ __forceinline__ u64 mul(u64 a, u64 b) { return red(a * b, __umul64hi(a, b)); }
-__device__ __forceinline__ u64 canon(u64 x) { return x >= GLP ? x - GLP : x; }
-#endif
-
+  else {
+    const u64 a = (u64)(u32)((u32)x << (E - 64)) * GLEPS, b = GLP - (x >> (96 - E));
+    const u64 s = a + b;
+    return s + (s < a ? GLEPS : 0);
+  }
+}
+GL_HD u64 mul(u64 a, u64 b) { return red(a * b, gl_mulhi(a, b)); }
+GL_HD u64 canon(u64 x) { return x >= GLP ? x - GLP : x; }
+#endif
+
+#if defined(SBN_NTT_CXX_ARITH)
+#define NW_FN GL_HD
+#else
+#define NW_FN __device__ __forceinline__
+#endif
 #define NW_BF(i, j, E) { u64 a_ = x[i], b_ = x[j]; x[i] = add(a_, b_); x[j] = mul_pow2<E>(sub(a_, b_)); }
-__device__ __forceinline__ void dft16_rho(u64* x) {
+NW_FN void dft16_rho(u64* x) {
   NW_BF(0, 8, 0) NW_BF(1, 9, 12) NW_BF(2, 10, 24) NW_BF(3, 11, 36) NW_BF(4, 12, 48) NW_BF(5, 13, 60) NW_BF(6, 14, 72) NW_BF(7, 15, 84)
   NW_BF(0, 4, 0) NW_BF(1, 5, 24) NW_BF(2, 6, 48) NW_BF(3, 7, 72) NW_BF(8, 12, 0) NW_BF(9, 13, 24) NW_BF(10, 14, 48) NW_BF(11, 15, 72)
   NW_BF(0, 2, 0) NW_BF(1, 3, 48) NW_BF(4, 6, 0) NW_BF(5, 7, 48) NW_BF(8, 10, 0) NW_BF(9, 11, 48) NW_BF(12, 14, 0) NW_BF(13, 15, 48)
   NW_BF(0, 1, 0) NW_BF(2, 3, 0) NW_BF(4, 5, 0) NW_BF(6, 7, 0) NW_BF(8, 9, 0) NW_BF(10, 11, 0) NW_BF(12, 13, 0) NW_BF(14, 15, 0)
 }
+#define NW_BF1(i, j, E) { u64 a_ = x[i], b_ = x[j]; x[i] = add1(a_, b_); x[j] = mul_pow2<E>(sub1(a_, b_)); }
+NW_FN void dft16_rho_canon_in(u64* x) {
+  NW_BF1(0, 8, 0) NW_BF1(1, 9, 12) NW_BF1(2, 10, 24) NW_BF1(3, 11, 36) NW_BF1(4, 12, 48) NW_BF1(5, 13, 60) NW_BF1(6, 14, 72) NW_BF1(7, 15, 84)
+  NW_BF(0, 4, 0) NW_BF(1, 5, 24) NW_BF(2, 6, 48) NW_BF(3, 7, 72) NW_BF(8, 12, 0) NW_BF(9, 13, 24) NW_BF(10, 14, 48) NW_BF(11, 15, 72)
+  NW_BF(0, 2, 0) NW_BF(1, 3, 48) NW_BF(4, 6, 0) NW_BF(5, 7, 48) NW_BF(8, 10, 0) NW_BF(9, 11, 48) NW_BF(12, 14, 0) NW_BF(13, 15, 48)
+  NW_BF(0, 1, 0) NW_BF(2, 3, 0) NW_BF(4, 5, 0) NW_BF(6, 7, 0) NW_BF(8, 9, 0) NW_BF(10, 11, 0) NW_BF(12, 13, 0) NW_BF(14, 15, 0)
+}
+#undef NW_BF1
 #undef NW_BF
+#undef NW_FN
 }
 
 #ifdef SBN_NTT_KERNELS_HERE
-template <int LOG_B>
+template <int LOG_B, bool CANON_IN>
 __global__ __launch_bounds__(256) void ntt_fast_pass_kernel(NttPassParams p, u32 kperm) {
   extern __shared__ u64 lds[];
   constexpr u32 NB = 1u << LOG_B;
@@ -170,7 +210,7 @@
   const size_t col = p.xcd_order ? blockIdx.x : blockIdx.y;
   const size_t t0 = (size_t)(p.xcd_order ? blockIdx.y : blockIdx.x) << 4;
   const u32 half = p.split ? blockIdx.z : 0u;
-  const u64* __restrict__ pre = half ? p.pre2 : p.pre;
+  const u64* __restrict__ pre = CANON_IN ? nullptr : (half ? p.pre2 : p.pre);
   const u64* in = p.in + col * p.in_col_stride;
   u64* out = p.out + col * p.out_col_stride;
   u32 g, t;
@@ -201,12 +241,14 @@
       u64 a = x[0][q], bb = x[NB - 1][q];
       u64 w = tw_full(p.tw, p.tw_log, r, 9);
       if (upper_zero) { x[NB - 1][q] = nw::mul(a, w); }
+      else if (CANON_IN) { x[0][q] = nw::add1(a, bb); x[NB - 1][q] = nw::mul(nw::sub1(a, bb), w); }
       else { x[0][q] = nw::add(a, bb); x[NB - 1][q] = nw::mul(nw::sub(a, bb), w); }
     }
   }
 #pragma unroll
   for (u32 b = 0; b < NB; b++) {
-    nw::dft16_rho(x[b]);
+    if (LOG_B == 0 && CANON_IN) nw::dft16_rho_canon_in(x[b]);
+    else nw::dft16_rho(x[b]);
 #pragma unroll
     for (u32 pidx = 0; pidx < 16; pidx++) {
       u32 m = __brev(pidx) >> 28;
@@ -231,7 +273,7 @@
       u32 k = LOG_B == 0 ? k256 : (k256 * NB + b);
       if (LOG_B == 1) k = (k << p.split) + half;
       u64 v = x[b][pidx];
-      if (p.twiddle) v = nw::mul(v, tw_full(p.tw, p.tw_log, (u32)(k * tg), p.log_n));
+      if (p.twiddle) v = nw::mul(v, tw_full(p.tw_ab ? p.tw_ab : p.tw, p.tw_log, (u32)(k * tg), p.log_n));
       if (p.scale != 1) v = nw::mul(v, p.scale);
       size_t go = (size_t)k * p.out_sr + tg * p.out_st;
       if (p.post) v = nw::mul(v, p.post[go]);
@@ -241,7 +283,7 @@
   (void)R;
 }
 #else
-template <int LOG_B> __global__ void ntt_fast_pass_kernel(NttPassParams p, u32 kperm);
+template <int LOG_B, bool CANON_IN> __global__ void ntt_fast_pass_kernel(NttPassParams p, u32 kperm);
 #endif
 
 struct NttFusedParams {
@@ -252,7 +294,6 @@
   u32 log_n;
   const u64* tw_i; const u64* tw_f; u32 tw_log;
   const u64* pre;
-  u64 scale;
   const u64* pre2;
 };
 #ifdef SBN_NTT_KERNELS_HERE
@@ -268,7 +309,7 @@
   u64 x[2][16];
 #pragma unroll
   for (u32 q = 0; q < 16; q++) x[0][q] = in[(size_t)(g + 16 * q) + tg * 256];
-  nw::dft16_rho(x[0]);
+  nw::dft16_rho_canon_in(x[0]);
 #pragma unroll
   for (u32 pidx = 0; pidx < 16; pidx++) {
     const u32 m = __brev(pidx) >> 28, k1 = (11u * m) & 15;
@@ -285,7 +326,7 @@
   for (u32 pidx = 0; pidx < 16; pidx++) {
     const u32 m = __brev(pidx) >> 28, k2 = (11u * m) & 15;
     const u32 k = g + 16 * k2;
-    const u64 v = nw::mul(x[0][pidx], p.scale);
+    const u64 v = x[0][pidx];
     coef[(size_t)k * p.n1 + tg] = nw::canon(v);
     a[k2] = v;
   }
@@ -345,8 +386,8 @@
 #pragma unroll
     for (u32 q = q0; q < q0 + 8; q++) {
       const u64 lo = in[(size_t)(g + 16 * q) + tg * 512], hi = in[(size_t)(g + 16 * q + 256) + tg * 512];
-      x[0][q] = nw::add(lo, hi);
-      x[1][q] = nw::mul(nw::sub(lo, hi), tw_full(p.tw_i, p.tw_log, g + 16 * q, 9));
+      x[0][q] = nw::add1(lo, hi);
+      x[1][q] = nw::mul(nw::sub1(lo, hi), tw_full(p.tw_i, p.tw_log, g + 16 * q, 9));
     }
     asm volatile("" ::: "memory");
   }
@@ -371,7 +412,7 @@
 #pragma unroll
     for (u32 pidx = 0; pidx < 16; pidx++) {
       const u32 m = __brev(pidx) >> 28, k2 = (11u * m) & 15;
-      const u64 v = nw::mul(z[pidx], p.scale);
+      const u64 v = z[pidx];
       coef[(size_t)((g + 16 * k2) * 2 + b) * 512 + tg] = nw::canon(v);
       x[b][k2] = v;
     }
diff --git a/starky_bn254_amd/csrc/ntt.hip b/starky_bn254_amd/csrc/ntt.hip
--- a/starky_bn254_amd/csrc/ntt.hip
+++ b/starky_bn254_amd/csrc/ntt.hip
@@ -1,4 +1,6 @@
 #define SBN_NTT_KERNELS_HERE
 #include "kernels_ntt.cuh"
-template __global__ void ntt_fast_pass_kernel<0>(NttPassParams p, u32 kperm);
-template __global__ void ntt_fast_pass_kernel<1>(NttPassParams p, u32 kperm);
+template __global__ void ntt_fast_pass_kernel<0, false>(NttPassParams p, u32 kperm);
+template __global__ void ntt_fast_pass_kernel<0, true>(NttPassParams p, u32 kperm);
+template __global__ void ntt_fast_pass_kernel<1, false>(NttPassParams p, u32 kperm);
+template __global__ void ntt_fast_pass_kernel<1, true>(NttPassParams p, u32 kperm);
diff --git a/starky_bn254_amd/csrc/prover.hip b/starky_bn254_amd/csrc/prover.hip
--- a/starky_bn254_amd/csrc/prover.hip
+++ b/starky_bn254_amd/csrc/prover.hip
@@ -36,6 +36,7 @@
   return 0;
 }
 
+static u64 host_inv_pow2(u32 k) { return f_inv(F((u64)1 << k)).v; }
 static u32 pick_log_t(u32 log_r, u32 log_s) {
   u32 lt = 4;
   while (lt > 0 && ((size_t)(1u << log_r) * ((1u << lt) + 1) * 8) > 48 * 1024) lt--;
@@ -59,6 +60,10 @@
   b.in_sr = 1; b.in_st = n2; b.out_sr = n1; b.out_st = 1; b.n_in = (size_t)1 << log_n;
   b.r_fast_load = 1; b.twiddle = 0; b.tw = a.tw; b.tw_log = P->lde_log;
   b.pre = nullptr; b.post = post; b.scale = scale;
+  const bool fast_a = log_n2 >= 4 && ((a.log_r == 8 && a.log_t == 4) || a.log_r == 9);
+  if (inverse && fast_a && P->d_tw_i_n && log_n == P->degree_bits && scale == host_inv_pow2(log_n)) {
+    a.tw_ab = P->d_tw_i_n; b.scale = 1;
+  }
   for (size_t c0 = 0; c0 < ncols; c0 += 32768) {
     size_t nc = std::min<size_t>(32768, ncols - c0);
     NttPassParams pa = a, pb = b;
@@ -70,8 +75,11 @@
     auto launch = [&](NttPassParams q, dim3 grid, size_t lds_bytes) {
       const bool fast = q.log_t == 4 && (q.log_r == 8 || q.log_r == 9);
       if (fast) { q.xcd_order = 1; std::swap(grid.x, grid.y); }
-      if (fast && q.log_r == 8) hipLaunchKernelGGL(ntt_fast_pass_kernel<0>, grid, dim3(256), 16 * 272 * 8, st, q, kperm);
-      else if (fast) hipLaunchKernelGGL(ntt_fast_pass_kernel<1>, grid, dim3(256), 32 * 272 * 8, st, q, kperm);
+      const bool canon_in = !q.pre;
+      if (fast && q.log_r == 8 && canon_in) hipLaunchKernelGGL((ntt_fast_pass_kernel<0, true>), grid, dim3(256), 16 * 272 * 8, st, q, kperm);
+      else if (fast && q.log_r == 8) hipLaunchKernelGGL((ntt_fast_pass_kernel<0, false>), grid, dim3(256), 16 * 272 * 8, st, q, kperm);
+      else if (fast && canon_in) hipLaunchKernelGGL((ntt_fast_pass_kernel<1, true>), grid, dim3(256), 32 * 272 * 8, st, q, kperm);
+      else if (fast) hipLaunchKernelGGL((ntt_fast_pass_kernel<1, false>), grid, dim3(256), 32 * 272 * 8, st, q, kperm);
       else hipLaunchKernelGGL(ntt_pass_kernel, grid, dim3(NTT_THREADS), lds_bytes, st, q);
     };
     if (pa.log_r == 9 && log_n2 >= 4) pa.log_t = 4;
@@ -87,12 +95,12 @@
   return 0;
 }
 
-static u64 host_inv_pow2(u32 k) { return f_inv(F((u64)1 << k)).v; }
 static int ntt_fast_setup() {
   static std::atomic<bool> done[SBN_MAX_DEVICES];
   const int d = g_device >= 0 && g_device < SBN_MAX_DEVICES ? g_device : 0;
   if (!done[d].load()) {
-    HIPC(hipFuncSetAttribute((const void*)ntt_fast_pass_kernel<1>, hipFuncAttributeMaxDynamicSharedMemorySize, 32 * 272 * 8));
+    HIPC(hipFuncSetAttribute((const void*)ntt_fast_pass_kernel<1, false>, hipFuncAttributeMaxDynamicSharedMemorySize, 32 * 272 * 8));
+    HIPC(hipFuncSetAttribute((const void*)ntt_fast_pass_kernel<1, true>, hipFuncAttributeMaxDynamicSharedMemorySize, 32 * 272 * 8));
     HIPC(hipFuncSetAttribute((const void*)ntt_fused_inv_b_lde_a_kernel, hipFuncAttributeMaxDynamicSharedMemorySize, 32 * 272 * 8));
     HIPC(hipFuncSetAttribute((const void*)ntt_fused512_inv_b_lde_a_kernel, hipFuncAttributeMaxDynamicSharedMemorySize, 32 * 272 * 8));
     done[d].store(true);
@@ -134,13 +142,13 @@
 }
 
 static int intt_lde_cols_fused(sbn_prover* P, const u64* v, u64* cf, u64* lde_out, size_t nc, u64* tmp2, hipStream_t lde_stream, hipEvent_t handoff) {
+  if (!P->d_tw_i_n) return fail(SBN_ERR_UNSUPPORTED, "the fused transform pass needs the scaled inverse root table");
   int rc = ntt_columns(P, v, P->n, cf, P->n, P->d_tmp, P->m, nc, P->degree_bits, true, P->n, nullptr, nullptr, host_inv_pow2(P->degree_bits), nullptr, 1);
   if (rc) return rc;
   NttFusedParams f{};
   const u32 log_n1 = (P->degree_bits + 1) / 2;
   f.in = P->d_tmp; f.in_col_stride = P->m; f.coef = cf; f.coef_col_stride = P->n; f.out = tmp2; f.out_col_stride = P->m;
   f.n1 = (size_t)1 << log_n1; f.log_n = P->degree_bits; f.tw_i = P->d_tw_i; f.tw_f = P->d_tw_f; f.tw_log = P->lde_log; f.pre = P->d_shift; f.pre2 = P->d_shift_odd;
-  f.scale = host_inv_pow2(P->degree_bits);
   if (P->ntt_fused512) hipLaunchKernelGGL(ntt_fused512_inv_b_lde_a_kernel, dim3((unsigned)nc, 32u), dim3(256), 32 * 272 * 8, P->stream, f);
   else hipLaunchKernelGGL(ntt_fused_inv_b_lde_a_kernel, dim3((unsigned)nc, (unsigned)(f.n1 >> 4)), dim3(256), 32 * 272 * 8, P->stream, f);
   if (lde_stream != P->stream) {
@@ -563,6 +571,7 @@
   acc(dmalloc(&P->d_q, 2 * m, &P->dev_bytes)); acc(dmalloc(&P->d_qlde, 4 * m, &P->dev_bytes));
   acc(tree_alloc(P->tree_q, m, cfg->cap_height, &P->dev_bytes));
   acc(dmalloc(&P->d_tw_f, m, &P->dev_bytes)); acc(dmalloc(&P->d_tw_i, m, &P->dev_bytes)); acc(dmalloc(&P->d_shift, m, &P->dev_bytes)); acc(dmalloc(&P->d_shift_inv, m, &P->dev_bytes));
+  acc(dmalloc(&P->d_tw_i_n, m, &P->dev_bytes));
   if (P->ntt_fused512) acc(dmalloc(&P->d_shift_odd, n, &P->dev_bytes));
   acc(dmalloc(&P->d_xs, m, &P->dev_bytes)); acc(dmalloc(&P->d_lag_first, m, &P->dev_bytes)); acc(dmalloc(&P->d_lag_last, m, &P->dev_bytes));
   P->apow_n = apow_len(as.nconstraints, as.nzs);
@@ -599,6 +608,7 @@
   F w = f_root_of_unity(P->lde_log);
   hipLaunchKernelGGL(pow_table_kernel, blocks(m), dim3(256), 0, P->stream, P->d_tw_f, m, w.v);
   hipLaunchKernelGGL(pow_table_kernel, blocks(m), dim3(256), 0, P->stream, P->d_tw_i, m, f_inv(w).v);
+  hipLaunchKernelGGL(pow_table_scaled_kernel, blocks(m), dim3(256), 0, P->stream, P->d_tw_i_n, m, f_inv(w).v, host_inv_pow2(degree_bits));
   hipLaunchKernelGGL(pow_table_kernel, blocks(m), dim3(256), 0, P->stream, P->d_shift, m, (u64)GL_GEN);
   hipLaunchKernelGGL(pow_table_kernel, blocks(m), dim3(256), 0, P->stream, P->d_shift_inv, m, f_inv(F(GL_GEN)).v);
   hipLaunchKernelGGL(domain_tables_kernel, blocks(m), dim3(256), 0, P->stream, P->d_xs, P->d_lag_first, P->d_lag_last, m, P->lde_log, degree_bits);
@@ -635,7 +645,7 @@
   if (!P) return;
   (void)hipSetDevice(P->device);
   u64* bufs[] = {P->d_trace, P->d_coef, P->d_lde, P->d_tmp, P->d_tmp2, P->d_tmp3, P->d_zval, P->d_zcoef, P->d_zlde, P->d_q, P->d_qlde, P->tree_t.d, P->tree_z.d,
-                 P->tree_q.d, P->d_tw_f, P->d_tw_i, P->d_shift, P->d_shift_inv, P->d_xs, P->d_lag_first, P->d_lag_last, P->d_apow, P->d_zpow,
+                 P->tree_q.d, P->d_tw_f, P->d_tw_i, P->d_tw_i_n, P->d_shift, P->d_shift_inv, P->d_xs, P->d_lag_first, P->d_lag_last, P->d_apow, P->d_zpow,
                  P->d_open, P->d_part, P->d_w, P->d_fa, P->d_fcoef, P->d_fcoef2, P->d_pow, P->d_qbuf, P->d_shift_odd};
   for (u64* b : bufs) if (b) (void)hipFree(b);
   for (u64* b : P->fri_vals) if (b) (void)hipFree(b);
@@ -1205,6 +1215,7 @@
   if (rate_bits != 1 || n < 512 || (n & (n - 1))) return fail(SBN_ERR_UNSUPPORTED, "need rate_bits=1 and n a power of two >= 512");
   u32 lg = 0; while (((size_t)1 << lg) < n) lg++;
   if (cap_height < 1 || cap_height > 8) return fail(SBN_ERR_UNSUPPORTED, "cap_height must be 1..8");
+  for (size_t i = 0; i < ncols * n; i++) if (cols[i] >= GLP) return fail(SBN_ERR_NON_CANONICAL, "value %zu is not canonical", i);
   sbn_prover P{};
   sbn_standard_fast_config(&P.cfg); P.cfg.cap_height = cap_height;
   P.degree_bits = lg; P.lde_log = lg + 1; P.n = n; P.m = 2 * n; P.ntt_chunk = 64; P.device = g_device;
@@ -1218,13 +1229,14 @@
   rc |= dmalloc(&d_vals, ncols * n); rc |= dmalloc(&d_coef, ncols * n); rc |= dmalloc(&d_lde, ncols * P.m); rc |= dmalloc(&P.d_tmp, 64 * P.m);
   if (P.ntt_fused || P.ntt_fused512) rc |= dmalloc(&P.d_tmp2, 64 * P.m);
   if (P.ntt_fused512) rc |= dmalloc(&P.d_shift_odd, n);
-  rc |= dmalloc(&P.d_tw_f, P.m); rc |= dmalloc(&P.d_tw_i, P.m); rc |= dmalloc(&P.d_shift, P.m);
+  rc |= dmalloc(&P.d_tw_f, P.m); rc |= dmalloc(&P.d_tw_i, P.m); rc |= dmalloc(&P.d_tw_i_n, P.m); rc |= dmalloc(&P.d_shift, P.m);
   rc |= tree_alloc(P.tree_t, P.m, cap_height);
   if (!rc) {
     auto blocks = [](size_t k) { return dim3((unsigned)((k + 255) / 256)); };
     F w = f_root_of_unity(P.lde_log);
     hipLaunchKernelGGL(pow_table_kernel, blocks(P.m), dim3(256), 0, P.stream, P.d_tw_f, P.m, w.v);
     hipLaunchKernelGGL(pow_table_kernel, blocks(P.m), dim3(256), 0, P.stream, P.d_tw_i, P.m, f_inv(w).v);
+    hipLaunchKernelGGL(pow_table_scaled_kernel, blocks(P.m), dim3(256), 0, P.stream, P.d_tw_i_n, P.m, f_inv(w).v, host_inv_pow2(lg));
     hipLaunchKernelGGL(pow_table_kernel, blocks(P.m), dim3(256), 0, P.stream, P.d_shift, P.m, (u64)GL_GEN);
     if (P.d_shift_odd) hipLaunchKernelGGL(shift_odd_table_kernel, blocks(n), dim3(256), 0, P.stream, P.d_shift_odd, n, P.d_shift, P.d_tw_f, 9u);
     if (hipMemcpy(d_vals, cols, ncols * n * sizeof(u64), hipMemcpyHostToDevice) != hipSuccess) rc = fail(SBN_ERR_HIP, "H2D failed");
@@ -1245,7 +1257,7 @@
   if (!rc) memcpy(cap_out, cap.data(), cap.size() * sizeof(u64));
   if (!rc && coeffs_out && hipMemcpy(coeffs_out, d_coef, ncols * n * sizeof(u64), hipMemcpyDeviceToHost) != hipSuccess) rc = fail(SBN_ERR_HIP, "D2H failed");
   if (!rc && lde_out && hipMemcpy(lde_out, d_lde, ncols * P.m * sizeof(u64), hipMemcpyDeviceToHost) != hipSuccess) rc = fail(SBN_ERR_HIP, "D2H failed");
-  for (u64* b : {d_vals, d_coef, d_lde, P.d_tmp, P.d_tmp2, P.d_shift_odd, P.d_tw_f, P.d_tw_i, P.d_shift, P.tree_t.d, P.d_sponge}) if (b) (void)hipFree(b);
+  for (u64* b : {d_vals, d_coef, d_lde, P.d_tmp, P.d_tmp2, P.d_shift_odd, P.d_tw_f, P.d_tw_i, P.d_tw_i_n, P.d_shift, P.tree_t.d, P.d_sponge}) if (b) (void)hipFree(b);
   (void)hipStreamDestroy(P.stream);
   return rc;
 }
diff --git a/starky_bn254_amd/csrc/prover_ctx.hpp b/starky_bn254_amd/csrc/prover_ctx.hpp
--- a/starky_bn254_amd/csrc/prover_ctx.hpp
+++ b/starky_bn254_amd/csrc/prover_ctx.hpp
@@ -68,6 +68,7 @@
   DevTree tree_t, tree_z, tree_q;
   std::vector<DevTree> fri_trees;
   u64 *d_tw_f = nullptr, *d_tw_i = nullptr, *d_shift = nullptr, *d_shift_inv = nullptr;
+  u64 *d_tw_i_n = nullptr;
   u64 *d_shift_odd = nullptr;
   u64 *d_xs = nullptr, *d_lag_first = nullptr, *d_lag_last = nullptr;
   u64 *d_apow = nullptr;
```
